# IuvenisSapiens/Qwen3-TTS-Rust

Hardware: AMD Instinct MI355X
Metric: audio-seconds generated per second (aggregate over GPUs) = concurrent real-time streams; RTF and first-chunk latency from the single-utterance leg (higher is better)
Workload: dtype i8

## Files before the change

### include/q3tts.h

```cpp
#ifndef Q3TTS_H
#define Q3TTS_H
#include <stdint.h>
#include <stddef.h>
#ifdef __cplusplus
extern "C" {
#endif

#define Q3TTS_OK 0
#define Q3TTS_ERR -1

const char* q3tts_last_error(void);
int q3tts_version(void);
int q3tts_device_count(void);

typedef struct q3tts_sampler_config {
    float temperature;
    int32_t top_k;
    float top_p;
    int32_t has_seed;
    uint64_t seed;
} q3tts_sampler_config;
void q3tts_sampler_config_default(q3tts_sampler_config* c);

typedef struct q3tts_gen_options {
// ... 112 lines not shown
int32_t q3tts_group_device_of(q3tts_group* g, int64_t req_id);
int q3tts_group_poll(q3tts_group* g, int64_t req_id, q3tts_req_status* out);
int q3tts_group_fetch(q3tts_group* g, int64_t req_id, int32_t* codes_out, int32_t frame_off, int32_t max_frames, float* pcm_out,
                      int64_t pcm_off, int64_t pcm_cap, int32_t* got_frames, int64_t* got_pcm);
int q3tts_group_wait(q3tts_group* g, int64_t req_id, double timeout_ms);
int q3tts_group_release(q3tts_group* g, int64_t req_id);
int q3tts_group_start(q3tts_group* g);
int q3tts_group_stop(q3tts_group* g);
typedef struct q3tts_comm q3tts_comm;
int q3tts_comm_available(void);
int q3tts_comm_unique_id(uint8_t out_id[128]);
int q3tts_comm_create(const uint8_t id[128], int32_t rank, int32_t world, int32_t device, q3tts_comm** out);
void q3tts_comm_destroy(q3tts_comm* c);
int q3tts_comm_voice_register(q3tts_comm* c, q3tts_engine* e, int32_t root, const float* spk_emb2048, const int32_t* ref_codes,
                              int32_t n_ref_codes, const int32_t* ref_text_ids, int32_t n_ref_text, int32_t* voice_id);
int32_t q3tts_engine_device(q3tts_engine* e);

typedef struct q3tts_assets q3tts_assets;
int q3tts_assets_open(const char* gguf_path, q3tts_assets** out);
void q3tts_assets_close(q3tts_assets* a);
const q3tts_assets* q3tts_engine_assets(q3tts_engine* e);
int q3tts_assets_codec_embedding(const q3tts_assets* a, int32_t q, int32_t code, float* out2048);
int q3tts_assets_text_embedding(const q3tts_assets* a, int64_t token, float* out2048);
int q3tts_assets_tts_pad(const q3tts_assets* a, float* out2048);
int q3tts_prompt_build_core(const q3tts_assets* a, const int32_t* text_ids, int32_t n_text, int32_t lang_id, int32_t spk_id,
                            const float* spk_emb2048, const int32_t* instr_ids, int32_t n_instr, const float* mid_rows,
                            int32_t n_mid, float* out, int32_t max_rows);
int q3tts_prompt_build_clone(const q3tts_assets* a, const int32_t* text_ids, int32_t n_text, const int32_t* ref_codes,
                             int32_t n_ref_codes, const int32_t* ref_text_ids, int32_t n_ref_text, const float* spk_emb2048,
                             int32_t lang_id, const int32_t* instr_ids, int32_t n_instr, float* out, int32_t max_rows);
int q3tts_prompt_build_streaming(const q3tts_assets* a, const int32_t* text_ids, int32_t n_text, int32_t lang_id, int32_t spk_id,
                                 const float* spk_emb2048, const int32_t* instr_ids, int32_t n_instr, const int32_t* ref_codes,
                                 int32_t n_ref_codes, const int32_t* ref_text_ids, int32_t n_ref_text, float* out, int32_t max_rows,
                                 int32_t* trail_ids, int32_t trail_cap, int32_t* n_trail);

typedef struct q3tts_sampler q3tts_sampler;
q3tts_sampler* q3tts_sampler_new(float temperature, int32_t top_k, float top_p, uint64_t seed);
void q3tts_sampler_free(q3tts_sampler* s);
int32_t q3tts_sampler_sample(q3tts_sampler* s, const float* logits, int32_t n_vocab, int32_t start, int32_t end);

typedef void (*q3tts_decode_cb)(void* user, const int64_t* codes, int32_t n_codes, int32_t is_final);
typedef struct q3tts_chunker q3tts_chunker;
q3tts_chunker* q3tts_chunker_new(q3tts_decode_cb cb, void* user);
void q3tts_chunker_free(q3tts_chunker* c);
int q3tts_chunker_push(q3tts_chunker* c, const int64_t* codes, int32_t n, int32_t is_final);

typedef struct q3tts_decoder q3tts_decoder;
int q3tts_decoder_create(const char* codec_gguf, int32_t n_streams, q3tts_decoder** out);
void q3tts_decoder_destroy(q3tts_decoder* d);
int q3tts_decoder_create_ex(const char* codec_gguf, int32_t n_streams, int32_t max_frames_per_call, int32_t max_group, q3tts_decoder** out);
int q3tts_decoder_decode_group(q3tts_decoder* d, int32_t G, const int32_t* streams, const int64_t* codes, int32_t n_frames, float* wav_out);
int q3tts_decoder_samples_per_frame(q3tts_decoder* d);
int q3tts_decoder_reset(q3tts_decoder* d, int32_t stream);
int q3tts_decoder_decode(q3tts_decoder* d, int32_t stream, const int64_t* codes, int32_t n_frames, int32_t is_last,
                         float* final_wav, int64_t* valid_samples);

int64_t q3tts_decoder_state_floats(q3tts_decoder* d);
int q3tts_decoder_state_export(q3tts_decoder* d, int32_t stream, float* out, int64_t n_floats);
int q3tts_decoder_state_import(q3tts_decoder* d, int32_t stream, const float* in, int64_t n_floats);
int32_t q3tts_decoder_state_entry(q3tts_decoder* d, int32_t i, const char** name, int64_t* offset, int32_t* rows, int32_t* cols);

int q3tts_mel_frames(int32_t n_samples);
int q3tts_mel(const float* audio, int32_t n_samples, float* mel_out );

typedef struct q3tts_tf q3tts_tf;
int q3tts_tf_open(const char* gguf_path, int32_t n_ctx, int32_t max_tok, q3tts_tf** out);
void q3tts_tf_close(q3tts_tf* t);
int q3tts_tf_dims(q3tts_tf* t, int32_t* n_embd, int32_t* n_layer, int32_t* n_head, int32_t* n_vocab);
void q3tts_tf_clear(q3tts_tf* t);
int q3tts_tf_eval(q3tts_tf* t, const float* x, const int32_t* pos4, int32_t ntok, float* hidden_out, float* logits_out,
                  int32_t row0, int32_t row1);

typedef struct q3tts_tokenizer q3tts_tokenizer;
int q3tts_tokenizer_open(const char* tokenizer_json, q3tts_tokenizer** out);
void q3tts_tokenizer_close(q3tts_tokenizer* t);
int32_t q3tts_tokenizer_encode(q3tts_tokenizer* t, const char* text_utf8, int32_t* ids, int32_t cap);
int64_t q3tts_tokenizer_decode(q3tts_tokenizer* t, const int32_t* ids, int32_t n, char* buf, int64_t cap);
int32_t q3tts_tokenizer_vocab_size(q3tts_tokenizer* t);
int64_t q3tts_text_nfc(const char* utf8, char* out, int64_t cap);

typedef struct q3tts_onnx q3tts_onnx;
int q3tts_onnx_open(const char* path, q3tts_onnx** out);
void q3tts_onnx_close(q3tts_onnx* m);
int q3tts_onnx_counts(q3tts_onnx* m, int32_t* n_nodes, int32_t* n_initializers, int32_t* n_inputs, int32_t* n_outputs);
int64_t q3tts_onnx_summary(q3tts_onnx* m, char* buf, int64_t cap);
int q3tts_onnx_node(q3tts_onnx* m, int32_t i, const char** op_type, const char** name, int32_t* n_in, int32_t* n_out, int32_t* n_attr);
const char* q3tts_onnx_node_input(q3tts_onnx* m, int32_t i, int32_t j);
const char* q3tts_onnx_node_output(q3tts_onnx* m, int32_t i, int32_t j);
int32_t q3tts_onnx_node_attr_ints(q3tts_onnx* m, int32_t i, const char* attr, int64_t* out, int32_t cap);
int32_t q3tts_onnx_node_attr_float(q3tts_onnx* m, int32_t i, const char* attr, float* out);
int q3tts_onnx_initializer(q3tts_onnx* m, int32_t i, const char** name, int32_t* dtype, int64_t* dims8, int32_t* ndims, const void** data,
                           int64_t* nbytes);
const char* q3tts_onnx_op_kernel(const char* op_type);
int q3tts_onnx_decoder_contract(q3tts_onnx* m, char* buf, int64_t cap);

typedef struct q3tts_onnx_session q3tts_onnx_session;
int q3tts_onnx_session_open(const char* path, int32_t device, q3tts_onnx_session** out);
void q3tts_onnx_session_close(q3tts_onnx_session* s);
int32_t q3tts_onnx_session_unsupported(q3tts_onnx_session* s, char* buf, int64_t cap);
int q3tts_onnx_session_set_input(q3tts_onnx_session* s, const char* name, int32_t dtype, const void* data, const int64_t* shape, int32_t rank);
int q3tts_onnx_session_run(q3tts_onnx_session* s);
int q3tts_onnx_session_output_info(q3tts_onnx_session* s, const char* name, int32_t* dtype, int32_t* rank, int64_t* shape8);
int q3tts_onnx_session_output(q3tts_onnx_session* s, const char* name, void* dst, int64_t cap_bytes);
int64_t q3tts_onnx_session_launches(q3tts_onnx_session* s);
int q3tts_onnx_op_executable(const char* op_type);
typedef struct q3tts_onnx_decoder q3tts_onnx_decoder;
int q3tts_onnx_decoder_open(const char* path, int32_t device, q3tts_onnx_decoder** out);
void q3tts_onnx_decoder_close(q3tts_onnx_decoder* d);
int q3tts_onnx_decoder_reset(q3tts_onnx_decoder* d);
int q3tts_onnx_decoder_decode(q3tts_onnx_decoder* d, const int64_t* codes, int32_t n_frames, int32_t is_final, float* pcm, int64_t cap, int64_t* n_out);
int q3tts_onnx_decoder_fetch(q3tts_onnx_decoder* d, float* pcm, int64_t cap, int64_t* n_out);

int q3tts_op_gemv_q8(const void* w_q8_0 , int32_t n, int32_t k, const int8_t* xq,
                     const uint16_t* xd, int32_t ntok, float* y , int32_t lpr);
int q3tts_op_gemv_kq(const void* const* raws, const int32_t* types, const int32_t* rows, int32_t nparts, int32_t k, const int8_t* xq, const uint16_t* xd,
                     int32_t ntok, float* y, int32_t lpr);
int q3tts_op_gateup_kq(const void* gate_raw, const void* up_raw, int32_t type, int32_t ff, int32_t k, const int8_t* xq, const uint16_t* xd, int32_t ntok,
                       int8_t* aq, uint16_t* ad);
int q3tts_op_gateup_q8(const void* w_q8_0, int32_t ff, int32_t k, const int8_t* xq, const uint16_t* xd, int32_t ntok, int8_t* aq,
                       uint16_t* ad);
int q3tts_op_matmul_float(const void* w , int32_t type, int32_t n, int32_t k, int32_t row0, int32_t nrows,
                          const float* x , int32_t ntok, float* y );
int q3tts_op_rmsnorm_quant(const float* x, const float* g, int32_t d, int32_t ntok, float eps, int8_t* xq, uint16_t* xd,
                           float* xn);
int q3tts_op_swiglu_quant(const float* gu, int32_t ff, int32_t ntok, int8_t* aq, uint16_t* ad);
int q3tts_op_argmax(const float* logits, int32_t n, int32_t start, int32_t end, int32_t mask_idx, int32_t* out);
int q3tts_op_sample(const float* logits, int32_t n, float temperature, int32_t top_k, float top_p, uint64_t seed, int32_t mask_idx,
                    int32_t n_draws, int32_t* out);
int q3tts_op_sample_rows(int32_t kernel, const float* logits, int32_t B, int32_t n, const float* temperature, const int32_t* top_k,
                         const float* top_p, const float* penalty, const uint64_t* seed, const int32_t* hist, const int32_t* hist_len,
                         int32_t hist_cap, int32_t n_draws, int32_t* out);
int q3tts_op_project(const float* x, const float* w , const float* b, int32_t n_in, int32_t n_out, float* y);
enum { Q3TTS_GEMM_AUTO = 0, Q3TTS_GEMM_SKINNY4 = 1, Q3TTS_GEMM_SKINNY8 = 2, Q3TTS_GEMM_SKINNY16 = 3,
       Q3TTS_GEMM_F32_1 = 4, Q3TTS_GEMM_F32_2 = 5,
       Q3TTS_GEMM_H1 = 6, Q3TTS_GEMM_H1_EPL = 7, Q3TTS_GEMM_H2 = 8, Q3TTS_GEMM_H2_EPL = 9,
       Q3TTS_GEMM_H3 = 10, Q3TTS_GEMM_H3_EPL = 11 };
enum { Q3TTS_EPI_NONE = 0, Q3TTS_EPI_GELU = 1, Q3TTS_EPI_RES_SCALE = 2 , Q3TTS_EPI_RES = 3 ,
       Q3TTS_EPI_SNAKE = 4  };
typedef struct q3tts_codec_gemm_desc {
    int32_t M, N, cin, taps, dil;
    const float* A; int64_t a_rows; int32_t lda, a_segT, a_skip;
    int32_t a_split, o_split;
    const float* W; const float* bias;
    int32_t epi; const float* res; int64_t res_floats; int32_t ldr, r_segT; int64_t r_skip;
    const float* scale; const float* snake_ea; const float* snake_ib;
    float* out; int64_t out_floats, out_off; int32_t ldo, o_segT; int64_t o_skip;
    int64_t ws_floats;
    int32_t form, ksplit, reducer;
    int32_t form_ran, ksplit_ran, reducer_ran;
} q3tts_codec_gemm_desc;
int q3tts_op_codec_gemm(q3tts_codec_gemm_desc* d);
int q3tts_codec_gemm_plan(q3tts_codec_gemm_desc* d);

#ifdef __cplusplus
}
#endif
#endif
```

### qwen3-tts-rust_amd/csrc/capi_ops.cpp

```cpp
#include "../../include/q3tts.h"
#include "transformer.h"
#include "host_logic.h"
#include "kdev.h"
#include "codec.h"

using namespace q3;
#define Q3_API_BEGIN try {
#define Q3_API_END(failval) } catch (const std::exception& ex) { set_last_error(ex.what()); return failval; } catch (...) { set_last_error("unknown error"); return failval; }
static void require_gpu() {
    int n = 0;
    if (hipGetDeviceCount(&n) != hipSuccess || n <= 0) throw Error("no HIP device available: the HIP path is the only compute path (no CPU fallback)");
}

extern "C" {

int q3tts_op_gemv_q8(const void* w, int32_t n, int32_t k, const int8_t* xq, const uint16_t* xd, int32_t ntok, float* y, int32_t lpr) {
    Q3_API_BEGIN
    require_gpu();
    DevBuf<uint8_t> storage;
    Q8Mat m = q8mat_from_host(w, n, k, storage);
    DevBuf<int8_t> dxq((size_t)ntok * k); dxq.upload(xq, dxq.n);
    DevBuf<uint16_t> dxd((size_t)ntok * (k / 32)); dxd.upload(xd, dxd.n);
    const int nsseg = ((k >> 8) + 7) / 8;
    DevBuf<float> parts((size_t)nsseg * ntok * n);
// ... 65 lines not shown
    DevBuf<uint8_t> storage;
    Q8Mat m = kqmat_from_host(parts, 2, k, storage);
    DevBuf<int8_t> dxq((size_t)ntok * k); dxq.upload(xq, dxq.n);
    DevBuf<uint16_t> dxd((size_t)ntok * (k / 32)); dxd.upload(xd, dxd.n);
    DevBuf<int8_t> daq((size_t)ntok * ff); DevBuf<uint16_t> dad((size_t)ntok * (ff / 32));
    if (!launch_gateup_mfma(0, m, ff, dxq.p, dxd.p, daq.p, dad.p, ntok)) throw Error("shape not served by the fused gate/up matrix-core kernel");
    Q3_LAUNCH_CHECK();
    Q3_HIP(hipDeviceSynchronize());
    daq.download(aq, daq.n); dad.download(ad, dad.n);
    return Q3TTS_OK;
    Q3_API_END(Q3TTS_ERR)
}

int q3tts_op_matmul_float(const void* w, int32_t type, int32_t n, int32_t k, int32_t row0, int32_t nrows, const float* x, int32_t ntok, float* y) {
    Q3_API_BEGIN
    require_gpu();
    Q3_CHECK(type == Q3_T_F32 || type == Q3_T_F16 || type == Q3_T_BF16, "float type expected");
    Q3_CHECK(n > 0 && k > 0 && k % 256 == 0 && ntok > 0 && row0 >= 0 && nrows > 0 && row0 + nrows <= n, "bad matmul shape");
    const size_t esz = type == Q3_T_F32 ? 4 : 2;
    DevBuf<uint8_t> dw((size_t)n * k * esz); dw.upload((const uint8_t*)w, dw.n);
    DevBuf<uint8_t> dwt((size_t)((n + 63) / 64) * 64 * k * esz);
    launch_tile_float(0, dw.p, dwt.p, type, n, k);
    FMat m; m.w = dw.p; m.wt = dwt.p; m.type = type; m.N = n; m.K = k;
    DevBuf<float> dx((size_t)ntok * k); dx.upload(x, dx.n);
    DevBuf<float> dy((size_t)ntok * nrows);
    launch_gemv_float(0, m, row0, nrows, dx.p, k, dy.p, nrows, ntok);
    Q3_HIP(hipDeviceSynchronize());
    dy.download(y, dy.n);
    return Q3TTS_OK;
    Q3_API_END(Q3TTS_ERR)
}

int q3tts_op_rmsnorm_quant(const float* x, const float* g, int32_t d, int32_t ntok, float eps, int8_t* xq, uint16_t* xd, float* xn) {
    Q3_API_BEGIN
    require_gpu();
    Q3_CHECK(d % 256 == 0 && d <= 2048, "d must be a multiple of 256 and <= 2048");
    DevBuf<float> dx((size_t)ntok * d), dg(d), dxn((size_t)ntok * d);
    dx.upload(x, dx.n); dg.upload(g, d);
    DevBuf<int8_t> dq((size_t)ntok * d); DevBuf<uint16_t> dd((size_t)ntok * d / 32);
    NormArgs a{};
    a.h_in = dx.p; a.h_stride = d; a.g = dg.p; a.eps = eps; a.d = d; a.xq = dq.p; a.xd = dd.p; a.xn_out = dxn.p;
    launch_rmsnorm_quant(0, a, ntok);
    Q3_HIP(hipDeviceSynchronize());
    if (xq) dq.download(xq, dq.n);
    if (xd) dd.download(xd, dd.n);
    if (xn) dxn.download(xn, dxn.n);
    return Q3TTS_OK;
    Q3_API_END(Q3TTS_ERR)
}

int q3tts_op_swiglu_quant(const float* gu, int32_t ff, int32_t ntok, int8_t* aq, uint16_t* ad) {
    Q3_API_BEGIN
    require_gpu();
    DevBuf<float> dgu((size_t)ntok * 2 * ff); dgu.upload(gu, dgu.n);
    DevBuf<int8_t> dq((size_t)ntok * ff); DevBuf<uint16_t> dd((size_t)ntok * ff / 32);
    launch_swiglu_quant(0, dgu.p, ff, dq.p, dd.p, ntok);
    Q3_HIP(hipDeviceSynchronize());
    dq.download(aq, dq.n); dd.download(ad, dd.n);
    return Q3TTS_OK;
    Q3_API_END(Q3TTS_ERR)
}

int q3tts_op_argmax(const float* logits, int32_t n, int32_t start, int32_t end, int32_t mask_idx, int32_t* out) {
    Q3_API_BEGIN
    require_gpu();
    DevBuf<float> dl(n); dl.upload(logits, n);
    DevBuf<int32_t> dm(1), dout(1);
    dm.upload(&mask_idx, 1);
    launch_argmax(0, dl.p, n, start, end, dm.p, dout.p, 1, 0, 1);
    Q3_HIP(hipDeviceSynchronize());
    dout.download(out, 1);
    return Q3TTS_OK;
    Q3_API_END(Q3TTS_ERR)
}

int q3tts_op_sample(const float* logits, int32_t n, float temperature, int32_t top_k, float top_p, uint64_t seed, int32_t mask_idx,
                    int32_t n_draws, int32_t* out) {
    Q3_API_BEGIN
    require_gpu();
    Q3_CHECK(logits && out && n >= 1 && n_draws >= 1, "bad arguments");
    StdRng rng(seed);
    DevBuf<float> dl(n), dt(1), dp(1); DevBuf<int32_t> dk(1), dm(1); DevBuf<uint32_t> dkey(8), ddraw(1); DevBuf<q3_u64> dout(n_draws);
    const uint32_t zero = 0;
    dl.upload(logits, n); dt.upload(&temperature, 1); dp.upload(&top_p, 1); dk.upload(&top_k, 1); dm.upload(&mask_idx, 1);
    dkey.upload(rng.key(), 8); ddraw.upload(&zero, 1);
    for (int i = 0; i < n_draws; i++) {
        SampleArgs a{dl.p, n, n, dt.p, dk.p, dp.p, dm.p, dkey.p, ddraw.p, dout.p + i, 1};
        launch_sample(0, a, 1);
    }
    Q3_HIP(hipDeviceSynchronize());
    std::vector<q3_u64> keys(n_draws);
    dout.download(keys.data(), n_draws);
    for (int i = 0; i < n_draws; i++) out[i] = (int32_t)(~(uint32_t)(keys[i] & 0xFFFFFFFFull));
    return Q3TTS_OK;
    Q3_API_END(Q3TTS_ERR)
}

int q3tts_op_sample_rows(int32_t kernel, const float* logits, int32_t B, int32_t n, const float* temperature, const int32_t* top_k,
                         const float* top_p, const float* penalty, const uint64_t* seed, const int32_t* hist, const int32_t* hist_len,
                         int32_t hist_cap, int32_t n_draws, int32_t* out) {
    Q3_API_BEGIN
    require_gpu();
    Q3_CHECK(logits && temperature && top_k && top_p && seed && out && B >= 1 && n >= 1 && n_draws >= 1, "bad arguments");
    Q3_CHECK(kernel == 0 || kernel == 1, "kernel must be 0 (k_sample) or 1 (k_sample_pred)");
    Q3_CHECK(kernel == 0 || !penalty, "the predictor sampler takes no penalty");
    Q3_CHECK(!penalty || (hist && hist_len && hist_cap >= 1), "a penalty needs a history");
    DevBuf<float> dl((size_t)B * n), dt(B), dp(B), dpen(B); DevBuf<int32_t> dk(B); DevBuf<uint32_t> dkey((size_t)8 * B), ddraw(B);
    DevBuf<q3_u64> dout((size_t)n_draws * B);
    dl.upload(logits, dl.n); dt.upload(temperature, B); dp.upload(top_p, B); dk.upload(top_k, B);
    std::vector<uint32_t> keys((size_t)8 * B), zero(B, 0u);
    for (int b = 0; b < B; b++) { StdRng rng(seed[b]); std::copy(rng.key(), rng.key() + 8, keys.begin() + (size_t)b * 8); }
    dkey.upload(keys.data(), keys.size()); ddraw.upload(zero.data(), B);
    DevBuf<int32_t> dh, dlen; DevBuf<q3_u64> dcur;
    if (penalty) {
        const int stride = hist_cap * 16;
        std::vector<int32_t> hh((size_t)B * stride, -1), len(B);
        std::vector<q3_u64> cur(B, 0ull);
        for (int b = 0; b < B; b++) {
            Q3_CHECK(hist_len[b] >= 0 && hist_len[b] <= hist_cap, "hist_len out of range");
            const int nh = hist_len[b];
            for (int f = 0; f + 1 < nh; f++) hh[(size_t)b * stride + (size_t)f * 16] = hist[(size_t)b * hist_cap + f];
            len[b] = nh > 0 ? nh - 1 : 0;
            if (nh > 0) cur[b] = pack_key(0.0f, hist[(size_t)b * hist_cap + nh - 1]);
        }
        dh.alloc(hh.size()); dh.upload(hh.data(), hh.size()); dlen.alloc(B); dlen.upload(len.data(), B); dcur.alloc((size_t)16 * B);
        std::vector<q3_u64> cur16((size_t)16 * B, 0ull);
        for (int b = 0; b < B; b++) cur16[(size_t)b * 16] = cur[b];
        dcur.upload(cur16.data(), cur16.size());
        dpen.upload(penalty, B);
    }
    for (int i = 0; i < n_draws; i++) {
        SampleArgs a{dl.p, n, n, dt.p, dk.p, dp.p, nullptr, dkey.p, ddraw.p, dout.p + (size_t)i * B, 1};
        if (penalty) { a.penalty = dpen.p; a.hist = dh.p; a.hist_stride = hist_cap * 16; a.hist_len = dlen.p; a.cur_key = dcur.p; a.cur_stride = 16; }
        if (kernel == 0) launch_sample(0, a, B);
        else launch_sample_pred(0, a, B);
        Q3_LAUNCH_CHECK();
    }
    Q3_HIP(hipDeviceSynchronize());
    std::vector<q3_u64> res(dout.n);
    dout.download(res.data(), res.size());
    for (size_t i = 0; i < res.size(); i++) out[i] = key_code(res[i]);
    return Q3TTS_OK;
    Q3_API_END(Q3TTS_ERR)
}

int q3tts_op_codec_gemm(q3tts_codec_gemm_desc* d) {
    Q3_API_BEGIN
    require_gpu();
    codec_gemm_run(d);
    return Q3TTS_OK;
    Q3_API_END(Q3TTS_ERR)
}

int q3tts_codec_gemm_plan(q3tts_codec_gemm_desc* d) {
    Q3_API_BEGIN
    codec_gemm_plan_only(d);
    return Q3TTS_OK;
    Q3_API_END(Q3TTS_ERR)
}

int q3tts_op_project(const float* x, const float* w, const float* b, int32_t n_in, int32_t n_out, float* y) {
    Q3_API_BEGIN
    require_gpu();
    std::vector<float> wt((size_t)n_in * n_out);
    for (int o = 0; o < n_out; o++) for (int i = 0; i < n_in; i++) wt[(size_t)i * n_out + o] = w[(size_t)o * n_in + i];
    DevBuf<float> dx(n_in), dw(wt.size()), db(n_out), dy(n_out);
    dx.upload(x, n_in); dw.upload(wt.data(), wt.size()); db.upload(b, n_out);
    launch_project(0, dx.p, n_in, dw.p, db.p, n_in, n_out, dy.p, n_out, 1);
    Q3_HIP(hipDeviceSynchronize());
    dy.download(y, n_out);
    return Q3TTS_OK;
    Q3_API_END(Q3TTS_ERR)
}

int q3tts_mel_frames(int32_t n) { const int plen = n + 768; return (plen > 1024 ? plen - 1024 : 0) / 256 + 1; }

}

#include "onnx_reader.h"
#include "onnx_exec.h"
struct q3tts_onnx { std::unique_ptr<OnnxModel> m; std::string text; };
extern "C" {
int q3tts_onnx_open(const char* path, q3tts_onnx** out) {
    Q3_API_BEGIN
    Q3_CHECK(path && out, "null argument");
    auto* h = new q3tts_onnx();
    try { h->m.reset(new OnnxModel(path)); } catch (...) { delete h; throw; }
    *out = h;
    return Q3TTS_OK;
    Q3_API_END(Q3TTS_ERR)
}
void q3tts_onnx_close(q3tts_onnx* m) { delete m; }
int q3tts_onnx_counts(q3tts_onnx* m, int32_t* n_nodes, int32_t* n_init, int32_t* n_in, int32_t* n_out) {
    if (!m) return Q3TTS_ERR;
    if (n_nodes) *n_nodes = (int32_t)m->m->nodes.size();
    if (n_init) *n_init = (int32_t)m->m->initializers.size();
    if (n_in) *n_in = (int32_t)m->m->inputs.size();
    if (n_out) *n_out = (int32_t)m->m->outputs.size();
    return Q3TTS_OK;
}
int64_t q3tts_onnx_summary(q3tts_onnx* m, char* buf, int64_t cap) {
    if (!m) return -1;
    m->text = m->m->summary();
    if (buf && cap > 0) { const size_t n = std::min((size_t)cap - 1, m->text.size()); std::memcpy(buf, m->text.data(), n); buf[n] = 0; }
    return (int64_t)m->text.size() + 1;
}
int q3tts_onnx_node(q3tts_onnx* m, int32_t i, const char** op_type, const char** name, int32_t* n_in, int32_t* n_out, int32_t* n_attr) {
    Q3_API_BEGIN
    Q3_CHECK(m && i >= 0 && i < (int)m->m->nodes.size(), "node index out of range");
    const OnnxNode& n = m->m->nodes[i];
    if (op_type) *op_type = n.op_type.c_str();
    if (name) *name = n.name.c_str();
    if (n_in) *n_in = (int32_t)n.inputs.size();
    if (n_out) *n_out = (int32_t)n.outputs.size();
    if (n_attr) *n_attr = (int32_t)n.attrs.size();
    return Q3TTS_OK;
    Q3_API_END(Q3TTS_ERR)
}
const char* q3tts_onnx_node_input(q3tts_onnx* m, int32_t i, int32_t j) {
    return (m && i >= 0 && i < (int)m->m->nodes.size() && j >= 0 && j < (int)m->m->nodes[i].inputs.size()) ? m->m->nodes[i].inputs[j].c_str() : nullptr;
}
const char* q3tts_onnx_node_output(q3tts_onnx* m, int32_t i, int32_t j) {
    return (m && i >= 0 && i < (int)m->m->nodes.size() && j >= 0 && j < (int)m->m->nodes[i].outputs.size()) ? m->m->nodes[i].outputs[j].c_str() : nullptr;
}
int32_t q3tts_onnx_node_attr_ints(q3tts_onnx* m, int32_t i, const char* attr, int64_t* out, int32_t cap) {
    if (!m || i < 0 || i >= (int)m->m->nodes.size() || !attr) return -1;
    const OnnxAttr* a = m->m->nodes[i].attr(attr);
    if (!a) return -1;
    if (a->type == 2 || (a->ints.empty() && a->type == 0)) { if (out && cap > 0) out[0] = a->i; return 1; }
    for (int k = 0; k < (int)a->ints.size() && k < cap; k++) out[k] = a->ints[k];
    return (int32_t)a->ints.size();
}
int32_t q3tts_onnx_node_attr_float(q3tts_onnx* m, int32_t i, const char* attr, float* out) {
    if (!m || i < 0 || i >= (int)m->m->nodes.size() || !attr || !out) return -1;
    const OnnxAttr* a = m->m->nodes[i].attr(attr);
    if (!a) return -1;
    *out = a->f;
    return 1;
}
int q3tts_onnx_initializer(q3tts_onnx* m, int32_t i, const char** name, int32_t* dtype, int64_t* dims8, int32_t* ndims, const void** data, int64_t* nbytes) {
    Q3_API_BEGIN
    Q3_CHECK(m && i >= 0 && i < (int)m->m->initializers.size(), "initializer index out of range");
    const OnnxTensor& t = m->m->initializers[i];
    Q3_CHECK(t.dims.size() <= 8, "more than 8 dimensions");
    if (name) *name = t.name.c_str();
    if (dtype) *dtype = t.data_type;
    if (ndims) *ndims = (int32_t)t.dims.size();
    if (dims8) for (size_t d = 0; d < t.dims.size(); d++) dims8[d] = t.dims[d];
    const void* p = t.raw; int64_t nb = (int64_t)t.raw_bytes;
    if (!p && !t.float_data.empty()) { p = t.float_data.data(); nb = (int64_t)t.float_data.size() * 4; }
    else if (!p && !t.int64_data.empty()) { p = t.int64_data.data(); nb = (int64_t)t.int64_data.size() * 8; }
    else if (!p && !t.int32_data.empty()) { p = t.int32_data.data(); nb = (int64_t)t.int32_data.size() * 4; }
    if (data) *data = p;
    if (nbytes) *nbytes = nb;
    return Q3TTS_OK;
    Q3_API_END(Q3TTS_ERR)
}
const char* q3tts_onnx_op_kernel(const char* op_type) { return op_type ? onnx_op_kernel(op_type) : nullptr; }
int q3tts_onnx_decoder_contract(q3tts_onnx* m, char* buf, int64_t cap) {
    if (!m) return Q3TTS_ERR;
    const std::string miss = m->m->check_decoder_contract();
    if (buf && cap > 0) { const size_t n = std::min((size_t)cap - 1, miss.size()); std::memcpy(buf, miss.data(), n); buf[n] = 0; }
    return miss.empty() ? 0 : 1;
}
}

#include "tokenizer.h"
struct q3tts_tokenizer { std::unique_ptr<Tokenizer> t; std::string text; };
extern "C" {
int q3tts_tokenizer_open(const char* tokenizer_json, q3tts_tokenizer** out) {
    Q3_API_BEGIN
    Q3_CHECK(tokenizer_json && out, "null argument");
    auto* h = new q3tts_tokenizer();
    try { h->t.reset(new Tokenizer(tokenizer_json)); } catch (...) { delete h; throw; }
    *out = h;
    return Q3TTS_OK;
    Q3_API_END(Q3TTS_ERR)
}
void q3tts_tokenizer_close(q3tts_tokenizer* t) { delete t; }
int32_t q3tts_tokenizer_encode(q3tts_tokenizer* t, const char* text_utf8, int32_t* ids, int32_t cap) {
    Q3_API_BEGIN
    Q3_CHECK(t && text_utf8, "null argument");
    const std::vector<int32_t> v = t->t->encode(text_utf8);
    for (size_t i = 0; i < v.size() && (int32_t)i < cap; i++) ids[i] = v[i];
    return (int32_t)v.size();
    Q3_API_END(-1)
}
int64_t q3tts_tokenizer_decode(q3tts_tokenizer* t, const int32_t* ids, int32_t n, char* buf, int64_t cap) {
    Q3_API_BEGIN
    Q3_CHECK(t && (ids || n == 0) && n >= 0, "bad arguments");
    t->text = t->t->decode(std::vector<int32_t>(ids, ids + n));
    if (buf && cap > 0) { const size_t k = std::min((size_t)cap - 1, t->text.size()); std::memcpy(buf, t->text.data(), k); buf[k] = 0; }
    return (int64_t)t->text.size();
    Q3_API_END(-1)
}
int64_t q3tts_text_nfc(const char* utf8, char* out, int64_t cap) {
    try {
        if (!utf8) return 0;
        const std::string r = q3::nfc_utf8(utf8);
        if (out && cap > 0) { const size_t n = std::min<size_t>((size_t)cap - 1, r.size()); memcpy(out, r.data(), n); out[n] = 0; }
        return (int64_t)r.size() + 1;
    } catch (const std::exception& e) { q3::set_last_error(e.what()); return -1; }
}
int32_t q3tts_tokenizer_vocab_size(q3tts_tokenizer* t) { return t ? t->t->vocab_size() : 0; }
}

// ... 93 lines not shown
```

### qwen3-tts-rust_amd/csrc/kernels.h

```cpp
#pragma once
#include <hip/hip_runtime.h>
#include <cstdint>

namespace q3 {

struct Q8Mat {
    const uint8_t* qs = nullptr;
    const uint16_t* sc = nullptr;
    int N = 0;
    int Npad = 0;
    int K = 0;
    const uint8_t* rg_type = nullptr;
    const uint32_t* rg_off = nullptr;
    const uint8_t* meta = nullptr;
    size_t qbytes = 0;
    int nparts = 0; int p1_rg0 = 0x7fffffff, p2_rg0 = 0x7fffffff; int p0_type = 0, p1_type = 0, p2_type = 0; uint32_t p0_off = 0, p1_off = 0, p2_off = 0;
    size_t bytes() const { return (qbytes ? qbytes : (size_t)Npad * K) + (size_t)Npad * (K / 32) * 2 + (meta ? (size_t)Npad * (K / 256) * 16 : 0); }
};
inline size_t q3_rowgroup_bytes(int type, int K) { return type == 13 ? (size_t)(K / 256) * 5120 : type == 14 ? (size_t)(K / 256) * 6144 : (size_t)(K / 32) * 1024; }

struct TokMeta {
    const int32_t* seq;
    const int32_t* slot;
    const int32_t* pos;
    int uniform_pos = -1;
    __device__ __forceinline__ int seq_of(int tok) const { return uniform_pos >= 0 ? tok : seq[tok]; }
    __device__ __forceinline__ int slot_of(int tok) const { return uniform_pos >= 0 ? uniform_pos : slot[tok]; }
    __device__ __forceinline__ int pos_of(int tok, int stream) const { return uniform_pos >= 0 ? uniform_pos : pos[(size_t)tok * 4 + stream]; }
};

struct KvCache {
    uint16_t* k;
    uint16_t* v;
    const int32_t* page_table;
    int max_pages;
    int n_layer, n_kv;
    __host__ __device__ size_t page_stride() const { return (size_t)n_layer * n_kv * 8192; }
    __host__ __device__ size_t layer_stride() const { return (size_t)n_kv * 8192; }
    __device__ __forceinline__ int page_of(int seq, int logical) const { return page_table ? page_table[(size_t)seq * max_pages + logical] : seq; }
};

bool launch_gateup_mfma(hipStream_t st, const Q8Mat& wgu, int ff, const int8_t* xq, const uint16_t* xd, int8_t* aq, uint16_t* ad, int ntok);
void launch_gemv_q8(hipStream_t st, const Q8Mat& w, int row0, int nrows, const int8_t* xq, const uint16_t* xd,
                    float* out, int out_stride, int ntok, int lpr_hint = 0);

struct NormArgs {
    const float* h_in; int h_stride;
    const int32_t* idx; int idx_stride;
    const unsigned long long* idx_keys;
    const float* parts; int nparts; int parts_stride;
    float* h_out;
    const float* g; float eps; int d;
    int8_t* xq; uint16_t* xd;
    float* xn_out;
};
void launch_rmsnorm_quant(hipStream_t st, const NormArgs& a, int ntok);

void launch_qk_rope_append(hipStream_t st, const float* qkv, int qkv_stride, const float* parts_unused, int n_head, int n_kv,
                           const float* q_norm_w, const float* k_norm_w, float eps, const float* rope_cos,
                           const float* rope_sin, int n_ctx, const int32_t* mrope_sec , const TokMeta& tm,
                           const KvCache& kv, int layer, float* qrot, int ntok);

void launch_attention(hipStream_t st, const float* qrot, int n_head, int n_kv, const TokMeta& tm, const KvCache& kv,
                      int layer, float* att , int8_t* aq, uint16_t* ad, int ntok);

void launch_swiglu_quant(hipStream_t st, const float* gu, int ff, int8_t* aq, uint16_t* ad, int ntok);

void launch_argmax(hipStream_t st, const float* logits, int stride, int start, int end, const int32_t* mask_per_tok,
                   int32_t* out, int out_stride, int add, int ntok);

void launch_project(hipStream_t st, const float* x, int x_stride, const float* Wt, const float* b, int n_in, int n_out,
                    float* out, int out_stride, int ntok);
void launch_project_table(hipStream_t st, const float* table, int64_t rows, const float* Wt, const float* b, int n_in,
                          int n_out, float* out);

void launch_argmax_keys(hipStream_t st, const float* logits, int stride, int n, const int32_t* mask_per_tok, unsigned long long* keys,
                        int key_stride, int ntok);


void launch_copy_f32(hipStream_t st, const float* src, float* dst, size_t n);
void init_kernel_attributes();

struct FMat { const void* w = nullptr; const void* wt = nullptr; int type = 0; int N = 0, K = 0; size_t bytes() const { return (size_t)N * K * (type == 0 ? 4 : 2); } };
void launch_gemv_float(hipStream_t st, const FMat& w, int row0, int nrows, const float* x, int x_stride, float* out, int out_stride, int ntok);
bool launch_gateup_float(hipStream_t st, const FMat& wgu, int ff, const float* x, int x_stride, float* act, int ntok);
void launch_tile_float(hipStream_t st, const void* w, void* wt, int type, int N, int K);
void launch_swiglu_f32(hipStream_t st, const float* gu, int ff, float* out, int ntok);

typedef unsigned long long q3_u64;
struct NormPro {
    const float* h_in; int h_stride;
    const q3_u64* idx_keys; int idx_stride;
    const float* parts; int nparts; int parts_stride; size_t parts_slab;
    float* h_out;
    const float* g; float eps;
    float* xn_out;
};
struct ArgmaxEpi {
    q3_u64* keys; int key_stride;
    const int32_t* mask_per_tok;
    int idx_add;
};
void launch_gemv_q8_norm(hipStream_t st, const Q8Mat& w, int row0, int nrows, const NormPro& a, float* out, int out_stride,
                         int ntok, const ArgmaxEpi* am);
void launch_rmsnorm_quant_wg(hipStream_t st, const NormPro& a, int d, int8_t* xq, uint16_t* xd, int ntok);
void launch_gateup_swiglu(hipStream_t st, const Q8Mat& wgu, int ff, const NormPro& a, int8_t* aq, uint16_t* ad, int ntok);
void launch_attention_fused(hipStream_t st, const float* qkv, int qkv_stride, int n_head, int n_kv, const float* q_norm_w,
                            const float* k_norm_w, float eps, const float* rope_cos, const float* rope_sin, int n_ctx,
                            const int32_t* mrope_sec, const TokMeta& tm, const KvCache& kv, int layer, int8_t* aq, uint16_t* ad,
                            int ntok);
void launch_attention_short(hipStream_t st, const float* qkv, int qkv_stride, int n_head, int n_kv, const float* q_norm_w,
                            const float* k_norm_w, float eps, const float* rope_cos, const float* rope_sin, int n_ctx,
                            const int32_t* mrope_sec, const TokMeta& tm, const KvCache& kv, int layer, int8_t* aq, uint16_t* ad, int ntok,
                            float* att = nullptr );
void launch_project_blk(hipStream_t st, const float* x, int x_stride, const float* Wblk , const float* b,
                        int n_in, int n_out, float* out, int out_stride, int ntok);
struct TextTrail {
    const int32_t* n_frames = nullptr; const int32_t* n_trail = nullptr; const int32_t* ids = nullptr; int ids_stride = 0;
    const float* table = nullptr; int64_t rows = 0;
};
void launch_feedback_keys(hipStream_t st, const float* const* tables, const int64_t* table_rows, const q3_u64* keys, int key_stride,
                          const float* tts_pad, float* out, int ntok, const TextTrail* trail = nullptr);
void launch_gather_rows_keys(hipStream_t st, const float* table, int64_t rows, const q3_u64* keys, int key_stride, int row_len,
                             float* dst, int ntok);
struct AdvanceKeysArgs {
    int B; int32_t *finished, *n_frames; const int32_t* max_frames; q3_u64* keys; q3_u64* next_key0; int32_t* hist; int hist_stride;
    int32_t *t_slot, *t_pos;
};
void launch_advance_keys(hipStream_t st, const AdvanceKeysArgs& a);

struct SampleArgs {
    const float* logits; int stride; int n;
    const float* temperature; const int32_t* top_k; const float* top_p;
    const int32_t* mask_idx;
    const uint32_t* rng_key; uint32_t* draws;
    q3_u64* out_key; int out_stride;
    const float* penalty = nullptr;
    const int32_t* hist = nullptr; int hist_stride = 0; const int32_t* hist_len = nullptr;
    const q3_u64* cur_key = nullptr; int cur_stride = 0;
};
void launch_sample(hipStream_t st, const SampleArgs& a, int B);
void launch_sample_pred(hipStream_t st, const SampleArgs& a, int B);

}
```

### qwen3-tts-rust_amd/csrc/kernels_fused.hip

```cpp
#include "kernels.h"
#include "kdev.h"
#include "wslice.h"
#include <cstdlib>
#include "q3_common.h"

namespace q3 {
Q3_STAMP_SETTER(set_stamp_buffer_fused)

__device__ __forceinline__ void norm_quant_token(const NormPro& a, int d, int tok, int ntok, int lane, int8_t* xq_dst,
                                                 uint16_t* xd_dst, bool write_global) {
    const int nch = d >> 8;
    const float* hin = a.h_in;
    if (a.idx_keys) hin += (size_t)key_code(a.idx_keys[(size_t)tok * a.idx_stride]) * a.h_stride;
    else hin += (size_t)tok * a.h_stride;
    float4 x[8];
    float p = 0.0f;
#pragma unroll
    for (int c = 0; c < 8; c++) {
        if (c < nch) {
            float4 v = *reinterpret_cast<const float4*>(hin + 256 * c + 4 * lane);
            if (a.nparts > 0) {
                const float* pp = a.parts + (size_t)tok * a.parts_stride + 256 * c + 4 * lane;
                float4 y = *reinterpret_cast<const float4*>(pp);
                for (int s = 1; s < a.nparts; s++) {
// ... 136 lines not shown
            acc[m] = ws.chain(0.0f, &xq_s[mm][seg * 256], dxv, r, half, bil);
        }
        if (q == 0) {
#pragma unroll
            for (int m = 0; m < MT; m++) red[wave][m * R + r] = acc[m];
        }
    });
    wg_barrier_lds();
    for (int t = threadIdx.x; t < R * MT; t += blockDim.x) {
        const int m = t / R, rr = t % R;
        float v[8];
#pragma unroll
        for (int s = 0; s < 8; s++) v[s] = red[s][t];
        float S = v[0];
#pragma unroll
        for (int s = 1; s < 8; s++) S = (s < nseg) ? S + v[s] : S;
        const int orow = blockIdx.x * R + rr, tok = tok0 + m;
        const bool ok = orow < nrows && tok < ntok;
        if (EPI == 0) {
            if (ok) out[(size_t)tok * out_stride + orow] = S;
        } else {
            const int gi = orow + am.idx_add;
            const int mk = (ok && am.mask_per_tok) ? am.mask_per_tok[tok] : -1;
            u64 key = (ok && gi != mk && S > -INFINITY) ? pack_key(S, gi) : 0ull;
#pragma unroll
            for (int sft = R / 2; sft >= 1; sft >>= 1) {
                const u64 o = __shfl_xor(key, sft);
                key = o > key ? o : key;
            }
            if (rr == 0 && key != 0ull && tok < ntok) atomicMax(am.keys + (size_t)tok * am.key_stride, key);
        }
    }
}

template <int LPR, int MT, int EPI>
static void gemv_norm_launch(hipStream_t st, const Q8Mat& w, int row0, int nrows, const NormPro& a, float* out, int out_stride,
                             int ntok, const ArgmaxEpi& am) {
    constexpr int R = 64 / LPR;
    const int nseg = w.K >> 8;
    dim3 grid((nrows + R - 1) / R, 1, (ntok + MT - 1) / MT);
    Q3_TS_SWITCH(w, hipLaunchKernelGGL((k_gemv_q8_norm<LPR, MT, EPI, TS>), grid, dim3(64 * nseg), 0, st, w, row0, nrows, a, out, out_stride, ntok, am));
}
template <int LPR, int EPI>
static void gemv_norm_mt(hipStream_t st, const Q8Mat& w, int row0, int nrows, const NormPro& a, float* out, int out_stride, int ntok,
                         const ArgmaxEpi& am) {
    if (ntok == 1) gemv_norm_launch<LPR, 1, EPI>(st, w, row0, nrows, a, out, out_stride, ntok, am);
    else if (ntok == 2) gemv_norm_launch<LPR, 2, EPI>(st, w, row0, nrows, a, out, out_stride, ntok, am);
    else if (ntok <= 4) gemv_norm_launch<LPR, 4, EPI>(st, w, row0, nrows, a, out, out_stride, ntok, am);
    else gemv_norm_launch<LPR, 8, EPI>(st, w, row0, nrows, a, out, out_stride, ntok, am);
}
void launch_gemv_q8_norm(hipStream_t st, const Q8Mat& w, int row0, int nrows, const NormPro& a, float* out, int out_stride, int ntok,
                         const ArgmaxEpi* am) {
    ArgmaxEpi none{};
    if (am) { gemv_norm_mt<2, 1>(st, w, row0, nrows, a, out, out_stride, ntok, *am); return; }
    if (nrows / 32 >= 512) gemv_norm_mt<2, 0>(st, w, row0, nrows, a, out, out_stride, ntok, none);
    else if (nrows / 16 >= 256) gemv_norm_mt<4, 0>(st, w, row0, nrows, a, out, out_stride, ntok, none);
    else gemv_norm_mt<8, 0>(st, w, row0, nrows, a, out, out_stride, ntok, none);
}

template <int MT, int NSEG, int TS>
__global__ void __launch_bounds__(64 * NSEG) k_gateup_swiglu(Q8Mat w, int ff, NormPro a, int8_t* __restrict__ aq,
                                                             uint16_t* __restrict__ ad, int ntok) {
    __shared__ float red[8][2][32 * MT];
    __shared__ __attribute__((aligned(16))) int8_t xq_s[MT][2048];
    __shared__ __attribute__((aligned(16))) uint16_t xd_s[MT][64];
    __shared__ __attribute__((aligned(16))) float vbuf_s[2048];
    __shared__ float scal_s[1];
    const int lane = threadIdx.x & 63, wave = threadIdx.x >> 6;
    const int r = lane & 31, half = lane >> 5;
    const int nseg = w.K >> 8;
    const int seg = wave;
    const int tok0 = blockIdx.z * MT;
    const int rgG = blockIdx.x, rgU = (ff >> 5) + blockIdx.x;
    wslice_dispatch<TS>(w, rgG, [&](auto tag) {
        constexpr int WT = decltype(tag)::value;
        WSlice<2, WT> wsg, wsu;
        if (WT == 0) {
            const int nb = w.K >> 5;
            const uint8_t* baseG = w.qs + ((size_t)rgG * nb + (size_t)seg * 8) * 1024 + half * 512 + r * 16;
            const uint8_t* baseU = w.qs + ((size_t)rgU * nb + (size_t)seg * 8) * 1024 + half * 512 + r * 16;
#pragma unroll
            for (int i = 0; i < 8; i++) { wsg.wv[i] = *reinterpret_cast<const uint4*>(baseG + (size_t)i * 1024); wsu.wv[i] = *reinterpret_cast<const uint4*>(baseU + (size_t)i * 1024); }
            wsg.dwv = *reinterpret_cast<const uint4*>(w.sc + (((size_t)rgG * nseg + seg) * 32 + r) * 8);
            wsu.dwv = *reinterpret_cast<const uint4*>(w.sc + (((size_t)rgU * nseg + seg) * 32 + r) * 8);
        } else {
            wsg.load(w, rgG, r, seg, half, 0);
            wsu.load(w, rgU, r, seg, half, 0);
        }
        for (int m = 0; m < MT; m++) {
            const int tok = tok0 + m;
            norm_quant_wg(a, w.K, tok, tok < ntok, lane, wave, xq_s[m], xd_s[m], vbuf_s, scal_s, blockIdx.x == 0);
            if (m + 1 < MT) wg_barrier_lds();
        }
        wg_barrier_lds();
        wsg.finish(half); wsu.finish(half);
#pragma unroll
        for (int m = 0; m < MT; m++) {
            const int mm = (tok0 + m < ntok) ? m : 0;
            const uint4 dxv = *reinterpret_cast<const uint4*>(&xd_s[mm][seg * 8]);
            float ag = 0.0f, au = 0.0f;
            if (WT == 0) {
#pragma unroll
                for (int i = 0; i < 8; i++) {
                    const uint4 xv = *reinterpret_cast<const uint4*>(&xq_s[mm][seg * 256 + i * 32 + half * 16]);
                    int ig = dot16(wsg.wv[i], xv), iu = dot16(wsu.wv[i], xv);
                    ig += xor_lane<32>(ig); iu += xor_lane<32>(iu);
                    const float dx = h2f(half_of(dxv, i));
                    ag = q3_fmaf((float)ig, h2f(half_of(wsg.dwv, i)) * dx, ag);
                    au = q3_fmaf((float)iu, h2f(half_of(wsu.dwv, i)) * dx, au);
                }
            } else {
                ag = wsg.chain(0.0f, &xq_s[mm][seg * 256], dxv, r, half, 0);
                au = wsu.chain(0.0f, &xq_s[mm][seg * 256], dxv, r, half, 0);
            }
            if (half == 0) { red[wave][0][m * 32 + r] = ag; red[wave][1][m * 32 + r] = au; }
        }
    });
    wg_barrier_lds();
    for (int t = threadIdx.x; t < 32 * MT; t += blockDim.x) {
        const int m = t >> 5, rr = t & 31, tok = tok0 + m;
        float vg[8], vu[8];
#pragma unroll
        for (int s = 0; s < 8; s++) { vg[s] = red[s][0][t]; vu[s] = red[s][1][t]; }
        float G = vg[0], U = vu[0];
#pragma unroll
        for (int s = 1; s < 8; s++) { G = (s < nseg) ? G + vg[s] : G; U = (s < nseg) ? U + vu[s] : U; }
        const float y = q3_swiglu(G, U);
        float amax = q3_fabsf(y);
        amax = fmaxf(amax, xor_lane<16>(amax)); amax = fmaxf(amax, xor_lane<8>(amax)); amax = fmaxf(amax, xor_lane<4>(amax));
        amax = fmaxf(amax, xor_lane<2>(amax)); amax = fmaxf(amax, xor_lane<1>(amax));
        const float dd = amax / 127.0f;
        const float id = (dd != 0.0f) ? (1.0f / dd) : 0.0f;
        if (tok < ntok) {
            aq[(size_t)tok * ff + blockIdx.x * 32 + rr] = (int8_t)(int)q3_rintf(y * id);
            if (rr == 0) ad[(size_t)tok * (ff >> 5) + blockIdx.x] = f2h(dd);
        }
    }
}
void launch_gateup_swiglu(hipStream_t st, const Q8Mat& w, int ff, const NormPro& a, int8_t* aq, uint16_t* ad, int ntok) {
    const int nseg = w.K >> 8;
    const int mt = ntok == 1 ? 1 : ntok == 2 ? 2 : 4;
    dim3 grid(ff / 32, 1, (ntok + mt - 1) / mt);
#define Q3_GU(MTV, NS) Q3_TS_SWITCH(w, hipLaunchKernelGGL((k_gateup_swiglu<MTV, NS, TS>), grid, dim3(64 * NS), 0, st, w, ff, a, aq, ad, ntok))
#define Q3_GU_NS(NS) do { if (mt == 1) Q3_GU(1, NS); else if (mt == 2) Q3_GU(2, NS); else Q3_GU(4, NS); } while (0)
    switch (nseg) {
        case 1: Q3_GU_NS(1); break; case 2: Q3_GU_NS(2); break; case 3: Q3_GU_NS(3); break; case 4: Q3_GU_NS(4); break;
        case 5: Q3_GU_NS(5); break; case 6: Q3_GU_NS(6); break; case 7: Q3_GU_NS(7); break; case 8: Q3_GU_NS(8); break;
        default: throw Error("k_gateup_swiglu: K must be at most 2048");
    }
#undef Q3_GU_NS
#undef Q3_GU
}

__global__ void __launch_bounds__(256) k_attention_fused(const float* __restrict__ qkv, int qkv_stride, int n_head, int n_kv,
                                                         const float* __restrict__ q_norm_w, const float* __restrict__ k_norm_w,
                                                         float eps, const float* __restrict__ rope_cos,
                                                         const float* __restrict__ rope_sin, int n_ctx,
                                                         const int32_t* __restrict__ mrope_sec, TokMeta tm, KvCache kv, int layer,
                                                         int8_t* __restrict__ aq, uint16_t* __restrict__ ad) {
    __shared__ __attribute__((aligned(16))) float q_s[128];
    __shared__ __attribute__((aligned(16))) uint16_t kcur_s[128];
    __shared__ __attribute__((aligned(16))) uint16_t vcur_s[128];
    __shared__ float p_s[256];
    __shared__ float red_s[4][128];
    __shared__ float wmax_s[4];
    const int h = blockIdx.x, tok = blockIdx.y, tid = threadIdx.x, lane = tid & 63, wave = tid >> 6;
    const int seq = tm.seq_of(tok), slot = tm.slot_of(tok), n = slot + 1;
    const int grp = n_head / n_kv, kvh = h / grp;
    const size_t head_off = (size_t)layer * kv.layer_stride() + (size_t)kvh * 8192;
    const int jj = lane >> 4, dc = lane & 15;
    uint4 kreg[16], vreg[16];
    {
        const int jbase = wave * 64;
        if (jbase < n) {
            const int page = kv.page_of(seq, jbase >> 6);
            const uint16_t* Kb = kv.k + (size_t)page * kv.page_stride() + head_off;
#pragma unroll
            for (int d8 = 0; d8 < 16; d8++) kreg[d8] = *reinterpret_cast<const uint4*>(Kb + (d8 * 64 + lane) * 8);
        }
#pragma unroll
        for (int u = 0; u < 16; u++) {
            const int jg = 16 * u + 4 * wave + jj;
            vreg[u] = make_uint4(0, 0, 0, 0);
            if (jg < n && jg != slot) {
                const int page = kv.page_of(seq, jg >> 6);
                vreg[u] = *reinterpret_cast<const uint4*>(kv.v + (size_t)page * kv.page_stride() + head_off + (jg & 63) * 128 + dc * 8);
            }
        }
    }
    if (wave < 3) {
        const float* vec = qkv + (size_t)tok * qkv_stride + (wave == 0 ? (size_t)h * 128 : wave == 1 ? (size_t)(n_head + kvh) * 128 : (size_t)(n_head + n_kv + kvh) * 128);
        const float x1 = vec[lane], x2 = vec[lane + 64];
        const int page = kv.page_of(seq, slot >> 6), ps = slot & 63;
        if (wave < 2) {
            const float* wn = wave == 0 ? q_norm_w : k_norm_w;
            const float w1 = wn[lane], w2 = wn[lane + 64];
            int32_t sec[4] = { mrope_sec[0], mrope_sec[1], mrope_sec[2], mrope_sec[3] };
            int pp = tm.pos_of(tok, q3_mrope_stream(lane, sec));
            if (pp < 0) pp = 0;
            if (pp > n_ctx - 1) pp = n_ctx - 1;
            const float cs = rope_cos[(size_t)pp * 64 + lane], sn = rope_sin[(size_t)pp * 64 + lane];
            float p = x1 * x1;
            p = q3_fmaf(x2, x2, p);
            const float ss = wave_sum_bfly(p);
            const float mean = ss / 128.0f;
            const float scale = 1.0f / q3_sqrtf(mean + eps);
            const float y1 = (x1 * scale) * w1, y2 = (x2 * scale) * w2;
            float o1, o2;
            q3_rope_pair(y1, y2, cs, sn, &o1, &o2);
            if (wave == 0) { q_s[lane] = o1; q_s[lane + 64] = o2; }
            else {
                const uint16_t k1 = f2h(o1), k2 = f2h(o2);
                kcur_s[lane] = k1; kcur_s[lane + 64] = k2;
                if (h % grp == 0) {
                    uint16_t* Kb = kv.k + (size_t)page * kv.page_stride() + head_off;
                    Kb[((lane >> 3) * 64 + ps) * 8 + (lane & 7)] = k1;
                    Kb[(((lane + 64) >> 3) * 64 + ps) * 8 + (lane & 7)] = k2;
                }
            }
        } else {
            const uint16_t v1 = f2h(x1), v2 = f2h(x2);
            vcur_s[lane] = v1; vcur_s[lane + 64] = v2;
            if (h % grp == 0) {
                uint16_t* Vb = kv.v + (size_t)page * kv.page_stride() + head_off;
                Vb[ps * 128 + lane] = v1; Vb[ps * 128 + lane + 64] = v2;
            }
        }
    }
    wg_barrier_lds();
    const float scale = 0.08838834764831845f;
    float M = 0.0f, L = 0.0f, O[8];
#pragma unroll
    for (int i = 0; i < 8; i++) O[i] = 0.0f;
    for (int c0 = 0; c0 < n; c0 += 256) {
        const int jbase = c0 + wave * 64;
        const int jme = jbase + lane;
        const bool valid = jme < n;
        if (c0 > 0) {
            if (jbase < n) {
                const int page = kv.page_of(seq, jbase >> 6);
                const uint16_t* Kb = kv.k + (size_t)page * kv.page_stride() + head_off;
#pragma unroll
                for (int d8 = 0; d8 < 16; d8++) kreg[d8] = *reinterpret_cast<const uint4*>(Kb + (d8 * 64 + lane) * 8);
            }
#pragma unroll
            for (int u = 0; u < 16; u++) {
                const int jg = c0 + 16 * u + 4 * wave + jj;
                vreg[u] = make_uint4(0, 0, 0, 0);
                if (jg < n && jg != slot) {
                    const int page = kv.page_of(seq, jg >> 6);
                    vreg[u] = *reinterpret_cast<const uint4*>(kv.v + (size_t)page * kv.page_stride() + head_off + (jg & 63) * 128 + dc * 8);
                }
            }
        }
        float s = -INFINITY;
        if (jbase < n) {
            const bool cur = (jme == slot);
            float acc = 0.0f;
#pragma unroll
            for (int d8 = 0; d8 < 16; d8++) {
                uint4 kk = kreg[d8];
                if (cur) kk = *reinterpret_cast<const uint4*>(&kcur_s[8 * d8]);
                const float4 qa = *reinterpret_cast<const float4*>(&q_s[8 * d8]);
                const float4 qb = *reinterpret_cast<const float4*>(&q_s[8 * d8 + 4]);
                acc = q3_fmaf(qa.x, h2f(kk.x & 0xFFFFu), acc); acc = q3_fmaf(qa.y, h2f(kk.x >> 16), acc);
                acc = q3_fmaf(qa.z, h2f(kk.y & 0xFFFFu), acc); acc = q3_fmaf(qa.w, h2f(kk.y >> 16), acc);
                acc = q3_fmaf(qb.x, h2f(kk.z & 0xFFFFu), acc); acc = q3_fmaf(qb.y, h2f(kk.z >> 16), acc);
                acc = q3_fmaf(qb.z, h2f(kk.w & 0xFFFFu), acc); acc = q3_fmaf(qb.w, h2f(kk.w >> 16), acc);
            }
            if (valid) s = acc * scale;
        }
        const float wm = wave_max_bfly(s);
        if (lane == 0) wmax_s[wave] = wm;
        wg_barrier_lds();
        const float mc = fmaxf(fmaxf(wmax_s[0], wmax_s[1]), fmaxf(wmax_s[2], wmax_s[3]));
        const float p = valid ? q3_expf(s - mc) : 0.0f;
        p_s[wave * 64 + lane] = p;
        wg_barrier_lds();
        float S[8];
#pragma unroll
        for (int i = 0; i < 8; i++) S[i] = 0.0f;
        const int cn = (n - c0) < 256 ? (n - c0) : 256;
#pragma unroll
        for (int u = 0; u < 16; u++) {
            if (16 * u < cn) {
                const int jl = 16 * u + 4 * wave + jj;
                const int jg = c0 + jl;
                const float pj = p_s[jl];
                uint4 vv = vreg[u];
                if (jg == slot) vv = *reinterpret_cast<const uint4*>(&vcur_s[dc * 8]);
                S[0] = q3_fmaf(pj, h2f(vv.x & 0xFFFFu), S[0]); S[1] = q3_fmaf(pj, h2f(vv.x >> 16), S[1]);
                S[2] = q3_fmaf(pj, h2f(vv.y & 0xFFFFu), S[2]); S[3] = q3_fmaf(pj, h2f(vv.y >> 16), S[3]);
                S[4] = q3_fmaf(pj, h2f(vv.z & 0xFFFFu), S[4]); S[5] = q3_fmaf(pj, h2f(vv.z >> 16), S[5]);
                S[6] = q3_fmaf(pj, h2f(vv.w & 0xFFFFu), S[6]); S[7] = q3_fmaf(pj, h2f(vv.w >> 16), S[7]);
            }
        }
#pragma unroll
        for (int i = 0; i < 8; i++) {
            const float a2 = S[i] + xor_lane<16>(S[i]);
            const float T = a2 + xor_lane<32>(a2);
            if (jj == 0) red_s[wave][dc * 8 + i] = T;
        }
        wg_barrier_lds();
        if (wave == 0) {
            float a2 = p_s[lane];
            a2 = a2 + p_s[lane + 64]; a2 = a2 + p_s[lane + 128]; a2 = a2 + p_s[lane + 192];
            const float lc = wave_sum_bfly(a2);
            float oc[8];
#pragma unroll
            for (int i = 0; i < 8; i++) oc[i] = (red_s[0][dc * 8 + i] + red_s[1][dc * 8 + i]) + (red_s[2][dc * 8 + i] + red_s[3][dc * 8 + i]);
            if (c0 == 0) {
                M = mc; L = lc;
#pragma unroll
                for (int i = 0; i < 8; i++) O[i] = oc[i];
            } else {
                const float mn = fmaxf(M, mc);
                const float ea = q3_expf(M - mn), eb = q3_expf(mc - mn);
                const float t2 = lc * eb;
                L = q3_fmaf(L, ea, t2);
#pragma unroll
                for (int i = 0; i < 8; i++) { const float u2 = oc[i] * eb; O[i] = q3_fmaf(O[i], ea, u2); }
                M = mn;
            }
        }
        wg_barrier_lds();
    }
    if (wave == 0) {
        float y[8];
        float amax = 0.0f;
#pragma unroll
        for (int i = 0; i < 8; i++) { y[i] = O[i] / L; amax = fmaxf(amax, q3_fabsf(y[i])); }
        amax = fmaxf(amax, xor_lane<1>(amax));
        amax = fmaxf(amax, xor_lane<2>(amax));
        const float dd = amax / 127.0f;
        const float id = (dd != 0.0f) ? (1.0f / dd) : 0.0f;
        if (jj == 0) {
            const size_t o = ((size_t)tok * n_head + h) * 128 + dc * 8;
            uint32_t lo = 0, hi = 0;
#pragma unroll
            for (int i = 0; i < 4; i++) {
                lo |= (uint32_t)((int)q3_rintf(y[i] * id) & 0xFF) << (8 * i);
                hi |= (uint32_t)((int)q3_rintf(y[i + 4] * id) & 0xFF) << (8 * i);
            }
            *reinterpret_cast<uint2*>(aq + o) = make_uint2(lo, hi);
            if ((dc & 3) == 0) ad[o >> 5] = f2h(dd);
        }
    }
}
void launch_attention_fused(hipStream_t st, const float* qkv, int qkv_stride, int n_head, int n_kv, const float* q_norm_w,
                            const float* k_norm_w, float eps, const float* rope_cos, const float* rope_sin, int n_ctx,
                            const int32_t* mrope_sec, const TokMeta& tm, const KvCache& kv, int layer, int8_t* aq, uint16_t* ad,
                            int ntok) {
    hipLaunchKernelGGL(k_attention_fused, dim3(n_head, ntok), dim3(256), 0, st, qkv, qkv_stride, n_head, n_kv, q_norm_w, k_norm_w,
                       eps, rope_cos, rope_sin, n_ctx, mrope_sec, tm, kv, layer, aq, ad);
}

template <int HPW>
__global__ void __launch_bounds__(64) k_attention_short(const float* __restrict__ qkv, int qkv_stride, int n_head, int n_kv,
                                                        const float* __restrict__ q_norm_w, const float* __restrict__ k_norm_w, float eps,
                                                        const float* __restrict__ rope_cos, const float* __restrict__ rope_sin, int n_ctx,
                                                        const int32_t* __restrict__ mrope_sec, TokMeta tm, KvCache kv, int layer,
                                                        int8_t* __restrict__ aq, uint16_t* __restrict__ ad, float* __restrict__ att) {
    __shared__ __attribute__((aligned(16))) float q_s[HPW][128];
    __shared__ __attribute__((aligned(16))) uint16_t kcur_s[128];
    __shared__ __attribute__((aligned(16))) uint16_t vcur_s[128];
    __shared__ float p_s[HPW][64];
    const int kvh = HPW == 2 ? blockIdx.x : blockIdx.x >> 1, h0 = HPW == 2 ? 2 * blockIdx.x : blockIdx.x;
    Q3_STAMP_DECL;
    Q3_STAMP(0);
    const bool writer = HPW == 2 || (blockIdx.x & 1) == 0;
    const int tok = blockIdx.y, lane = threadIdx.x;
    const float scale = 0.08838834764831845f;
    const int jj = lane >> 4, dc = lane & 15;
    const int seq = tm.seq_of(tok), slot = tm.slot_of(tok), n = slot + 1;
    const size_t head_off = (size_t)layer * kv.layer_stride() + (size_t)kvh * 8192;
    const int page = kv.page_of(seq, 0);
    const uint16_t* Kb = kv.k + (size_t)page * kv.page_stride() + head_off;
    const uint16_t* Vb = kv.v + (size_t)page * kv.page_stride() + head_off;
    uint4 kreg[16], vreg[4][4];
#pragma unroll
    for (int d8 = 0; d8 < 16; d8++) kreg[d8] = (lane < slot) ? *reinterpret_cast<const uint4*>(Kb + (d8 * 64 + lane) * 8) : make_uint4(0, 0, 0, 0);
#pragma unroll
    for (int ww = 0; ww < 4; ww++)
#pragma unroll
        for (int u = 0; u < 4; u++) {
            const int jl = 16 * u + 4 * ww + jj;
            vreg[ww][u] = (jl < slot) ? *reinterpret_cast<const uint4*>(Vb + jl * 128 + dc * 8) : make_uint4(0, 0, 0, 0);
        }
    int32_t sec[4] = { mrope_sec[0], mrope_sec[1], mrope_sec[2], mrope_sec[3] };
    int pp = tm.pos_of(tok, q3_mrope_stream(lane, sec));
    if (pp < 0) pp = 0;
    if (pp > n_ctx - 1) pp = n_ctx - 1;
    const float cs = rope_cos[(size_t)pp * 64 + lane], sn = rope_sin[(size_t)pp * 64 + lane];
    const float* tv = qkv + (size_t)tok * qkv_stride;
#pragma unroll
    for (int which = 0; which < HPW + 1; which++) {
        const float* vec = tv + (which < HPW ? (size_t)(h0 + which) * 128 : (size_t)(n_head + kvh) * 128);
        const float* wn = which < HPW ? q_norm_w : k_norm_w;
        const float x1 = vec[lane], x2 = vec[lane + 64];
        float p = x1 * x1;
        p = q3_fmaf(x2, x2, p);
        const float ss = wave_sum_bfly(p);
        const float mean = ss / 128.0f;
        const float sc2 = 1.0f / q3_sqrtf(mean + eps);
        const float y1 = (x1 * sc2) * wn[lane], y2 = (x2 * sc2) * wn[lane + 64];
        float o1, o2;
        q3_rope_pair(y1, y2, cs, sn, &o1, &o2);
        if (which < HPW) { q_s[which][lane] = o1; q_s[which][lane + 64] = o2; }
        else {
            const uint16_t k1 = f2h(o1), k2 = f2h(o2);
            kcur_s[lane] = k1; kcur_s[lane + 64] = k2;
            if (writer) {
                uint16_t* Kw = kv.k + (size_t)page * kv.page_stride() + head_off;
                Kw[((lane >> 3) * 64 + slot) * 8 + (lane & 7)] = k1;
                Kw[(((lane + 64) >> 3) * 64 + slot) * 8 + (lane & 7)] = k2;
            }
        }
    }
    {
        const float* vec = tv + (size_t)(n_head + n_kv + kvh) * 128;
        const uint16_t v1 = f2h(vec[lane]), v2 = f2h(vec[lane + 64]);
        vcur_s[lane] = v1; vcur_s[lane + 64] = v2;
        if (writer) {
            uint16_t* Vw = kv.v + (size_t)page * kv.page_stride() + head_off;
            Vw[slot * 128 + lane] = v1; Vw[slot * 128 + lane + 64] = v2;
        }
    }
    wg_barrier_lds();
    Q3_STAMP(1);
    const bool valid = lane < n, cur = lane == slot;
    float a[HPW];
#pragma unroll
    for (int hh = 0; hh < HPW; hh++) a[hh] = 0.0f;
#pragma unroll
    for (int d8 = 0; d8 < 16; d8++) {
        uint4 kk = kreg[d8];
        if (cur) kk = *reinterpret_cast<const uint4*>(&kcur_s[8 * d8]);
        const float kf[8] = { h2f(kk.x & 0xFFFFu), h2f(kk.x >> 16), h2f(kk.y & 0xFFFFu), h2f(kk.y >> 16),
                              h2f(kk.z & 0xFFFFu), h2f(kk.z >> 16), h2f(kk.w & 0xFFFFu), h2f(kk.w >> 16) };
#pragma unroll
        for (int e = 0; e < 8; e++)
#pragma unroll
            for (int hh = 0; hh < HPW; hh++) a[hh] = q3_fmaf(q_s[hh][8 * d8 + e], kf[e], a[hh]);
    }
    Q3_STAMP_AFTER(2, a[0]);
    float L[HPW];
#pragma unroll
    for (int hh = 0; hh < HPW; hh++) {
        const float sc = valid ? a[hh] * scale : -INFINITY;
        const float m = wave_max_bfly(sc);
        const float pv = valid ? q3_expf(sc - m) : 0.0f;
        p_s[hh][lane] = pv;
        L[hh] = wave_sum_bfly(pv);
    }
    wg_barrier_lds();
    Q3_STAMP(3);
    const int dq = n_head * 128;
#pragma unroll
    for (int hh = 0; hh < HPW; hh++) {
        float s01[8], s23[8], y[8];
#pragma unroll
        for (int ww = 0; ww < 4; ww++) {
            float S[8];
#pragma unroll
            for (int i = 0; i < 8; i++) S[i] = 0.0f;
#pragma unroll
            for (int u = 0; u < 4; u++) {
                if (16 * u < n) {
                    const int jl = 16 * u + 4 * ww + jj;
                    const float pj = p_s[hh][jl];
                    uint4 vv = vreg[ww][u];
                    if (jl == slot) vv = *reinterpret_cast<const uint4*>(&vcur_s[dc * 8]);
                    S[0] = q3_fmaf(pj, h2f(vv.x & 0xFFFFu), S[0]); S[1] = q3_fmaf(pj, h2f(vv.x >> 16), S[1]);
                    S[2] = q3_fmaf(pj, h2f(vv.y & 0xFFFFu), S[2]); S[3] = q3_fmaf(pj, h2f(vv.y >> 16), S[3]);
                    S[4] = q3_fmaf(pj, h2f(vv.z & 0xFFFFu), S[4]); S[5] = q3_fmaf(pj, h2f(vv.z >> 16), S[5]);
                    S[6] = q3_fmaf(pj, h2f(vv.w & 0xFFFFu), S[6]); S[7] = q3_fmaf(pj, h2f(vv.w >> 16), S[7]);
                }
            }
#pragma unroll
            for (int i = 0; i < 8; i++) {
                const float a2 = S[i] + xor_lane<16>(S[i]);
                const float T = a2 + xor_lane<32>(a2);
                if (ww == 0) s01[i] = T; else if (ww == 1) s01[i] = s01[i] + T; else if (ww == 2) s23[i] = T; else s23[i] = s23[i] + T;
            }
        }
#pragma unroll
        for (int i = 0; i < 8; i++) y[i] = (s01[i] + s23[i]) / L[hh];
        const int hq = h0 + hh;
        if (att && jj == 0) {
            float* o = att + (size_t)tok * dq + (size_t)hq * 128 + dc * 8;
            *reinterpret_cast<float4*>(o) = make_float4(y[0], y[1], y[2], y[3]);
            *reinterpret_cast<float4*>(o + 4) = make_float4(y[4], y[5], y[6], y[7]);
        }
        float amax = 0.0f;
#pragma unroll
        for (int i = 0; i < 8; i++) amax = fmaxf(amax, q3_fabsf(y[i]));
        amax = fmaxf(amax, xor_lane<1>(amax));
        amax = fmaxf(amax, xor_lane<2>(amax));
        const float dd = amax / 127.0f;
        const float id = (dd != 0.0f) ? (1.0f / dd) : 0.0f;
        if (jj == 0) {
            uint32_t lo = 0, hi = 0;
#pragma unroll
            for (int i = 0; i < 4; i++) {
                lo |= (uint32_t)((int)q3_rintf(y[i] * id) & 0xFF) << (8 * i);
                hi |= (uint32_t)((int)q3_rintf(y[i + 4] * id) & 0xFF) << (8 * i);
            }
            *reinterpret_cast<uint2*>(aq + (size_t)tok * dq + (size_t)hq * 128 + dc * 8) = make_uint2(lo, hi);
            if ((dc & 3) == 0) ad[(size_t)tok * (dq >> 5) + hq * 4 + (dc >> 2)] = f2h(dd);
        }
    }
    Q3_STAMP(6);
    Q3_STAMP_FLUSH();
}
void launch_attention_short(hipStream_t st, const float* qkv, int qkv_stride, int n_head, int n_kv, const float* q_norm_w,
                            const float* k_norm_w, float eps, const float* rope_cos, const float* rope_sin, int n_ctx,
                            const int32_t* mrope_sec, const TokMeta& tm, const KvCache& kv, int layer, int8_t* aq, uint16_t* ad, int ntok, float* att) {
    static const int hpw1_max = [] { const char* e = std::getenv("Q3_SHORT_ATTN_HPW1_MAX"); return e ? atoi(e) : 128; }();
    if (ntok <= hpw1_max)
        hipLaunchKernelGGL(k_attention_short<1>, dim3(n_head, ntok), dim3(64), 0, st, qkv, qkv_stride, n_head, n_kv, q_norm_w, k_norm_w, eps, rope_cos,
                           rope_sin, n_ctx, mrope_sec, tm, kv, layer, aq, ad, att);
    else
        hipLaunchKernelGGL(k_attention_short<2>, dim3(n_kv, ntok), dim3(64), 0, st, qkv, qkv_stride, n_head, n_kv, q_norm_w, k_norm_w, eps, rope_cos,
                           rope_sin, n_ctx, mrope_sec, tm, kv, layer, aq, ad, att);
}

__global__ void __launch_bounds__(256) k_project_mt(const float* __restrict__ x, int x_stride, const float* __restrict__ Wblk,
                                                    const float* __restrict__ b, int n_in, int n_out, float* __restrict__ out,
                                                    int out_stride, int ntok) {
    constexpr int KC = 512, LDP = KC + 4;
    __shared__ __attribute__((aligned(16))) float xs[16][LDP];
    __shared__ __attribute__((aligned(16))) float ws[16][LDP];
    const int ob = blockIdx.x, t0 = blockIdx.y * 16, tid = threadIdx.x;
    const int o16 = tid & 15, tl = tid >> 4;
    const float* wslab = Wblk + (size_t)ob * n_in * 16;
    float4 rx[8], rw[8];
    auto fetch = [&](int k0) {
#pragma unroll
        for (int j = 0; j < 8; j++) {
            const int e = tid + 256 * j;
            const int t = e >> 7, i4 = e & 127;
            rx[j] = (t0 + t < ntok) ? *reinterpret_cast<const float4*>(x + (size_t)(t0 + t) * x_stride + k0 + 4 * i4) : make_float4(0.f, 0.f, 0.f, 0.f);
            rw[j] = *reinterpret_cast<const float4*>(wslab + (size_t)k0 * 16 + 4 * (size_t)e);
        }
    };
    auto stash = [&]() {
#pragma unroll
        for (int j = 0; j < 8; j++) {
            const int e = tid + 256 * j;
            *reinterpret_cast<float4*>(&xs[e >> 7][4 * (e & 127)]) = rx[j];
            const int i = e >> 2, q = (e & 3) * 4;
            ws[q + 0][i] = rw[j].x; ws[q + 1][i] = rw[j].y; ws[q + 2][i] = rw[j].z; ws[q + 3][i] = rw[j].w;
        }
    };
    const int o = ob * 16 + o16;
    float sum = b[o];
    fetch(0);
    for (int k0 = 0; k0 < n_in; k0 += KC) {
        stash();
        __syncthreads();
        if (k0 + KC < n_in) fetch(k0 + KC);
#pragma unroll 8
        for (int i = 0; i < KC; i += 4) {
            const float4 xv = *reinterpret_cast<const float4*>(&xs[tl][i]), wv = *reinterpret_cast<const float4*>(&ws[o16][i]);
            float t = xv.x * wv.x; sum = sum + t;
            t = xv.y * wv.y; sum = sum + t;
            t = xv.z * wv.z; sum = sum + t;
            t = xv.w * wv.w; sum = sum + t;
        }
        __syncthreads();
    }
    if (t0 + tl < ntok) out[(size_t)(t0 + tl) * out_stride + o] = sum;
}
void init_fused_kernel_attributes() {}
void launch_project_blk(hipStream_t st, const float* x, int x_stride, const float* Wblk, const float* b, int n_in, int n_out,
                        float* out, int out_stride, int ntok) {
    if (n_in % 512 != 0 || x_stride % 4 != 0 || (reinterpret_cast<uintptr_t>(x) & 15) != 0) throw Error("k_project_mt: n_in must be a multiple of 512 and the rows 16-byte aligned");
    hipLaunchKernelGGL(k_project_mt, dim3(n_out / 16, (ntok + 15) / 16), dim3(256), 0, st, x, x_stride, Wblk, b, n_in, n_out, out, out_stride, ntok);
}

template <bool TRAIL>
__global__ void __launch_bounds__(256) k_feedback_keys(const float* const* __restrict__ tables, const int64_t* __restrict__ table_rows,
                                                       const u64* __restrict__ keys, int key_stride,
                                                       const float* __restrict__ tts_pad, float* __restrict__ out, TextTrail tt) {
    const int tok = blockIdx.y, i = blockIdx.x * 256 + threadIdx.x;
    float acc = 0.0f;
#pragma unroll
    for (int q = 0; q < 16; q++) {
        int c = key_code(keys[(size_t)tok * key_stride + q]);
        if (c < 0) c = 0;
        const float v = ((int64_t)c < table_rows[q]) ? tables[q][(size_t)c * 2048 + i] : 0.0f;
        acc = acc + v;
    }
    float last;
    if constexpr (TRAIL) {
        const int f = tt.n_frames[tok];
        if (f < tt.n_trail[tok]) {
            const int32_t id = tt.ids[(size_t)tok * tt.ids_stride + f];
            if (id >= 0 && (int64_t)id < tt.rows) last = tt.table[(size_t)id * 2048 + i];
            else {
                const float x = (float)((unsigned long long)(long long)id * 17ull + (unsigned long long)i);
                last = (x < 16777216.0f ? (float)((uint32_t)x & 1u) : 0.0f) - 1.0f;
            }
        } else {
            last = tts_pad[i];
        }
    } else {
        last = tts_pad[i];
    }
    acc = acc + last;
    out[(size_t)tok * 2048 + i] = acc;
}
void launch_feedback_keys(hipStream_t st, const float* const* tables, const int64_t* table_rows, const u64* keys, int key_stride,
                          const float* tts_pad, float* out, int ntok, const TextTrail* trail) {
    if (trail) hipLaunchKernelGGL(k_feedback_keys<true>, dim3(8, ntok), dim3(256), 0, st, tables, table_rows, keys, key_stride, tts_pad, out, *trail);
    else hipLaunchKernelGGL(k_feedback_keys<false>, dim3(8, ntok), dim3(256), 0, st, tables, table_rows, keys, key_stride, tts_pad, out, TextTrail());
}

__global__ void __launch_bounds__(256) k_gather_rows_keys(const float* __restrict__ table, int64_t rows, const u64* __restrict__ keys,
                                                          int key_stride, int row_len, float* __restrict__ dst) {
    const int tok = blockIdx.y, i = blockIdx.x * 256 + threadIdx.x;
    if (i >= row_len) return;
    int c = key_code(keys[(size_t)tok * key_stride]);
    if (c < 0) c = 0;
    dst[(size_t)tok * row_len + i] = ((int64_t)c < rows) ? table[(size_t)c * row_len + i] : 0.0f;
}
void launch_gather_rows_keys(hipStream_t st, const float* table, int64_t rows, const u64* keys, int key_stride, int row_len,
                             float* dst, int ntok) {
    hipLaunchKernelGGL(k_gather_rows_keys, dim3((row_len + 255) / 256, ntok), dim3(256), 0, st, table, rows, keys, key_stride, row_len, dst);
}

__global__ void k_advance_keys(AdvanceKeysArgs a) {
    const int b = blockIdx.x * 64 + threadIdx.x;
    if (b >= a.B) return;
    u64* k = a.keys + (size_t)b * 16;
    const bool live = !a.finished[b] && a.n_frames[b] < a.max_frames[b];
    if (live) {
        const int c0 = key_code(k[0]);
        if (c0 == Q3_CODEC_EOS || c0 == Q3_TEXT_EOS) a.finished[b] = 1;
        else {
            int32_t* dst = a.hist + (size_t)b * a.hist_stride + (size_t)a.n_frames[b] * 16;
            for (int q = 0; q < 16; q++) dst[q] = key_code(k[q]);
            a.n_frames[b] = a.n_frames[b] + 1;
            a.t_slot[b] = a.t_slot[b] + 1;
            a.t_pos[b * 4 + 0] += 1; a.t_pos[b * 4 + 1] += 1; a.t_pos[b * 4 + 2] += 1;
        }
    }
    k[0] = a.next_key0[b];
    a.next_key0[b] = pack_key(-INFINITY, 0);
    for (int q = 1; q < 16; q++) k[q] = pack_key(-INFINITY, 0);
}
void launch_advance_keys(hipStream_t st, const AdvanceKeysArgs& a) {
    hipLaunchKernelGGL(k_advance_keys, dim3((a.B + 63) / 64), dim3(64), 0, st, a);
}

}
```

### qwen3-tts-rust_amd/csrc/transformer.cpp

```cpp
#include "transformer.h"
#include <cstdlib>
#include <cmath>

namespace q3 {

__global__ void k_repack_q8(const uint8_t* __restrict__ raw, int n, int K, int row_off, uint8_t* __restrict__ qs,
                            uint16_t* __restrict__ sc, int sc_row_extra) {
    const int nb = K >> 5, nseg = K >> 8;
    const size_t id = (size_t)blockIdx.x * 256 + threadIdx.x;
    if (id >= (size_t)n * nb) return;
    const int r = (int)(id / nb), b = (int)(id % nb);
    const uint8_t* src = raw + id * 34;
    const int row = row_off + r, rg = row >> 5, r32 = row & 31;
    uint16_t d;
    memcpy(&d, src, 2);
    const int srow = row + sc_row_extra;
    sc[(((size_t)(srow >> 5) * nseg + (b >> 3)) * 32 + (srow & 31)) * 8 + (b & 7)] = d;
    uint8_t* dst = qs + ((size_t)rg * nb + b) * 1024 + r32 * 16;
    for (int i = 0; i < 16; i++) { dst[i] = src[2 + i]; dst[512 + i] = src[18 + i]; }
}

__global__ void k_repack_q5k(const uint8_t* __restrict__ raw, int n, int K, int row_off, uint8_t* __restrict__ qs, const uint32_t* __restrict__ rg_off,
                             uint16_t* __restrict__ sc, uint8_t* __restrict__ meta) {
    const int nseg = K >> 8;
// ... 95 lines not shown
    std::vector<uint8_t> types((size_t)nrg);
    std::vector<uint32_t> off((size_t)nrg);
    size_t qs_bytes = 0;
    { int rg = 0; for (int i = 0; i < nparts; i++) for (int j = 0; j < parts[i].rows / 32; j++, rg++) { types[(size_t)rg] = (uint8_t)parts[i].type; off[(size_t)rg] = (uint32_t)(qs_bytes / 16); qs_bytes += q3_rowgroup_bytes(parts[i].type, k); } }
    const size_t sc_bytes = (size_t)n * (k / 32) * 2, meta_bytes = (size_t)n * (k / 256) * 16, ty_bytes = (size_t)((nrg + 15) & ~15), off_bytes = (size_t)((nrg * 4 + 15) & ~15);
    storage.alloc(qs_bytes + sc_bytes + meta_bytes + ty_bytes + off_bytes);
    storage.zero();
    uint8_t* base = storage.p;
    uint16_t* sc = reinterpret_cast<uint16_t*>(base + qs_bytes);
    uint8_t* meta = base + qs_bytes + sc_bytes;
    uint8_t* ty = meta + meta_bytes;
    uint32_t* offd = reinterpret_cast<uint32_t*>(ty + ty_bytes);
    Q3_HIP(hipMemcpy(ty, types.data(), types.size(), hipMemcpyHostToDevice));
    Q3_HIP(hipMemcpy(offd, off.data(), off.size() * 4, hipMemcpyHostToDevice));
    m.qs = base; m.sc = sc; m.meta = meta; m.rg_type = ty; m.rg_off = offd; m.qbytes = qs_bytes;
    int last = -1, row_off = 0;
    for (int i = 0; i < nparts; i++) {
        const int t = parts[i].type, rows = parts[i].rows;
        Q3_CHECK(t == Q3_T_Q8_0 || t == Q3_T_Q5_K || t == Q3_T_Q6_K, "unsupported weight type");
        if (t != last) {
            const int rg0 = row_off / 32;
            if (m.nparts == 0) { m.p0_type = t; m.p0_off = off[(size_t)rg0]; }
            else if (m.nparts == 1) { m.p1_rg0 = rg0; m.p1_type = t; m.p1_off = off[(size_t)rg0]; }
            else { m.p2_rg0 = rg0; m.p2_type = t; m.p2_off = off[(size_t)rg0]; }
            m.nparts++; last = t;
        }
        const size_t raw_bytes = t == Q3_T_Q8_0 ? (size_t)rows * (k / 32) * 34 : (size_t)rows * (k / 256) * (t == Q3_T_Q5_K ? 176 : 210);
        DevBuf<uint8_t> raw(raw_bytes);
        raw.upload((const uint8_t*)parts[i].raw, raw_bytes);
        if (t == Q3_T_Q8_0) {
            const size_t nblk = (size_t)rows * (k / 32);
            hipLaunchKernelGGL(k_repack_q8, dim3((unsigned)((nblk + 255) / 256)), dim3(256), 0, 0, raw.p, rows, k, 0, base + (size_t)off[(size_t)(row_off / 32)] * 16, sc, row_off);
        } else {
            const size_t nsb = (size_t)rows * (k / 256);
            if (t == Q3_T_Q5_K) hipLaunchKernelGGL(k_repack_q5k, dim3((unsigned)((nsb + 255) / 256)), dim3(256), 0, 0, raw.p, rows, k, row_off, base, offd, sc, meta);
            else hipLaunchKernelGGL(k_repack_q6k, dim3((unsigned)((nsb + 255) / 256)), dim3(256), 0, 0, raw.p, rows, k, row_off, base, offd, sc, meta);
        }
        Q3_HIP(hipDeviceSynchronize());
        row_off += rows;
    }
    return m;
}

Q8Mat Transformer::make_mat(const Gguf& g, const std::vector<std::pair<std::string, int>>& rows, int N, int K) {
    Q3_CHECK(K % 256 == 0, "K must be a multiple of 256");
    Q8Mat m;
    m.N = N; m.Npad = (N + 31) & ~31; m.K = K;
    const int nrg = m.Npad / 32;
    std::vector<uint8_t> types((size_t)nrg, (uint8_t)Q3_T_Q8_0);
    bool kq = false;
    for (auto& r : rows) {
        const GgufTensor& t = g.need(r.first);
        if (t.type != Q3_T_Q8_0 && t.type != Q3_T_Q5_K && t.type != Q3_T_Q6_K)
            throw Error("tensor " + r.first + ": ggml type " + std::to_string(t.type) + " is not supported by the HIP path (Q8_0, Q5_K, Q6_K)");
        Q3_CHECK(r.second % 32 == 0 && t.ne[1] % 32 == 0 && r.second + t.ne[1] <= m.Npad, "bad row range for " + r.first);
        for (int64_t i = 0; i < t.ne[1] / 32; i++) types[(size_t)(r.second / 32 + i)] = (uint8_t)t.type;
        kq = kq || t.type != Q3_T_Q8_0;
    }
    std::vector<uint32_t> off((size_t)nrg);
    size_t qs_bytes = 0;
    for (int i = 0; i < nrg; i++) { off[(size_t)i] = (uint32_t)(qs_bytes / 16); qs_bytes += q3_rowgroup_bytes(kq ? types[(size_t)i] : Q3_T_Q8_0, K); }
    Q3_CHECK(qs_bytes / 16 < (1ull << 32), "matrix too large for 32-bit row-group offsets");
    const size_t sc_bytes = (size_t)m.Npad * (K / 32) * 2;
    const size_t meta_bytes = kq ? (size_t)m.Npad * (K / 256) * 16 : 0, ty_bytes = (size_t)((nrg + 15) & ~15), off_bytes = kq ? (size_t)((nrg * 4 + 15) & ~15) : 0;
    blobs_.emplace_back(qs_bytes + sc_bytes + meta_bytes + ty_bytes + off_bytes);
    blobs_.back().zero();
    uint8_t* base = blobs_.back().p;
    m.qs = base;
    m.sc = reinterpret_cast<const uint16_t*>(base + qs_bytes);
    mat_meta_[m.qs] = base + qs_bytes + sc_bytes;
    mat_types_[m.qs] = base + qs_bytes + sc_bytes + meta_bytes;
    mat_off_[m.qs] = reinterpret_cast<uint32_t*>(base + qs_bytes + sc_bytes + meta_bytes + ty_bytes);
    if (kq) {
        Q3_HIP(hipMemcpy(mat_types_[m.qs], types.data(), types.size(), hipMemcpyHostToDevice));
        Q3_HIP(hipMemcpy(mat_off_[m.qs], off.data(), off.size() * 4, hipMemcpyHostToDevice));
        m.meta = mat_meta_[m.qs]; m.rg_type = mat_types_[m.qs]; m.rg_off = mat_off_[m.qs]; m.qbytes = qs_bytes;
        all_q8_ = false;
        int last = -1;
        for (int i = 0; i < nrg; i++) {
            if (last == types[(size_t)i]) continue;
            last = types[(size_t)i];
            Q3_CHECK(m.nparts < 3, "more than 3 runs of weight types in one fused matrix");
            if (m.nparts == 0) { m.p0_type = last; m.p0_off = off[(size_t)i]; }
            else if (m.nparts == 1) { m.p1_rg0 = i; m.p1_type = last; m.p1_off = off[(size_t)i]; }
            else { m.p2_rg0 = i; m.p2_type = last; m.p2_off = off[(size_t)i]; }
            m.nparts++;
        }
    }
    for (auto& r : rows) load_into(g, r.first, m, r.second, K);
    return m;
}

void Transformer::load_into(const Gguf& g, const std::string& name, Q8Mat& dst, int row_off, int K_expect) {
    const GgufTensor& t = g.need(name);
    Q3_CHECK(t.ne[0] == K_expect, "unexpected K for " + name);
    DevBuf<uint8_t> raw(t.nbytes);
    raw.upload(t.data, t.nbytes);
    uint8_t* qs = const_cast<uint8_t*>(dst.qs);
    uint16_t* sc = const_cast<uint16_t*>(dst.sc);
    if (t.type == Q3_T_Q8_0) {
        const size_t nblk = (size_t)t.ne[1] * (t.ne[0] / 32);
        uint8_t* q0 = qs;
        int ro = row_off;
        if (dst.rg_off) {
            uint32_t o = 0;
            Q3_HIP(hipMemcpy(&o, dst.rg_off + row_off / 32, 4, hipMemcpyDeviceToHost));
            q0 = qs + (size_t)o * 16; ro = 0;
        }
        hipLaunchKernelGGL(k_repack_q8, dim3((unsigned)((nblk + 255) / 256)), dim3(256), 0, 0, raw.p, (int)t.ne[1], (int)t.ne[0], ro, q0, sc, row_off - ro);
    } else {
        const size_t nsb = (size_t)t.ne[1] * (t.ne[0] / 256);
        uint8_t* meta = mat_meta_.at(dst.qs);
        if (t.type == Q3_T_Q5_K) hipLaunchKernelGGL(k_repack_q5k, dim3((unsigned)((nsb + 255) / 256)), dim3(256), 0, 0, raw.p, (int)t.ne[1], (int)t.ne[0], row_off, qs, dst.rg_off, sc, meta);
        else hipLaunchKernelGGL(k_repack_q6k, dim3((unsigned)((nsb + 255) / 256)), dim3(256), 0, 0, raw.p, (int)t.ne[1], (int)t.ne[0], row_off, qs, dst.rg_off, sc, meta);
    }
    Q3_HIP(hipDeviceSynchronize());
}

FMat Transformer::make_fmat(const Gguf& g, const std::vector<std::string>& names, int K_expect) {
    FMat m;
    size_t total = 0;
    for (auto& n : names) {
        const GgufTensor& t = g.need(n);
        Q3_CHECK(t.ne[0] == K_expect && (t.type == Q3_T_F32 || t.type == Q3_T_F16 || t.type == Q3_T_BF16), "bad float tensor " + n);
        if (m.N == 0) m.type = t.type;
        Q3_CHECK(t.type == m.type, "mixed float types in one fused matrix: " + n);
        m.N += (int)t.ne[1]; total += t.nbytes;
    }
    m.K = K_expect;
    blobs_.emplace_back(total);
    size_t off = 0;
    for (auto& n : names) { const GgufTensor& t = g.need(n); Q3_HIP(hipMemcpy(blobs_.back().p + off, t.data, t.nbytes, hipMemcpyHostToDevice)); off += t.nbytes; }
    m.w = blobs_.back().p;
    if (K_expect % 256 == 0) {
        const size_t esz = m.type == Q3_T_F32 ? 4 : 2;
        blobs_.emplace_back((size_t)((m.N + 63) / 64) * 64 * K_expect * esz);
        launch_tile_float(nullptr, m.w, blobs_.back().p, m.type, m.N, K_expect);
        Q3_HIP(hipDeviceSynchronize());
        m.wt = blobs_.back().p;
    }
    return m;
}

float* Transformer::load_f32(const Gguf& g, const std::string& name, int64_t n_expect) {
    const GgufTensor& t = g.need(name);
    Q3_CHECK(t.type == Q3_T_F32 && t.ne[0] * t.rows() == n_expect, "bad f32 tensor " + name);
    blobs_.emplace_back((size_t)n_expect * 4);
    blobs_.back().upload(t.data, (size_t)n_expect * 4);
    return reinterpret_cast<float*>(blobs_.back().p);
}

Transformer::Transformer(const std::string& path, int n_ctx, int max_tok) : n_ctx_(n_ctx), max_tok_(max_tok) {
    init_kernel_attributes();
    if (const char* e = std::getenv("Q3_UNFUSED")) fused = !(e[0] == '1');
    Gguf g(path);
    hp_.arch = g.kv_str("general.architecture", "qwen3");
    auto K = [&](const char* s) { return hp_.arch + "." + s; };
    hp_.n_embd = (int)g.kv_int(K("embedding_length"), 0);
    hp_.n_layer = (int)g.kv_int(K("block_count"), 0);
    hp_.n_head = (int)g.kv_int(K("attention.head_count"), 0);
    hp_.n_kv = (int)g.kv_int(K("attention.head_count_kv"), hp_.n_head);
    const int head_dim = (int)g.kv_int(K("attention.key_length"), hp_.n_head ? hp_.n_embd / hp_.n_head : 0);
    hp_.n_ff = (int)g.kv_int(K("feed_forward_length"), 0);
    hp_.eps = (float)g.kv_float(K("attention.layer_norm_rms_epsilon"), 1e-6);
    hp_.rope_base = (float)g.kv_float(K("rope.freq_base"), 1e6);
    if (auto* s = g.kv(K("rope.dimension_sections")))
        for (size_t i = 0; i < s->arr_i.size() && i < 4; i++) hp_.mrope_sec[i] = (int32_t)s->arr_i[i];
    Q3_CHECK(hp_.n_embd > 0 && hp_.n_layer > 0 && hp_.n_head > 0 && head_dim == Q3_HEAD_DIM, "unsupported hparams");
    Q3_CHECK(hp_.n_embd % 256 == 0 && hp_.n_embd <= 2048 && hp_.n_ff % 256 == 0 && hp_.n_head % hp_.n_kv == 0, "unsupported dims");
    Q3_CHECK(hp_.n_head * 128 <= 2048, "n_head*128 must be <= 2048 (single super-segment o-proj)");
    const int d = hp_.n_embd, dq = hp_.n_head * 128, dkv = hp_.n_kv * 128, ff = hp_.n_ff;
    layers_.resize(hp_.n_layer);
    {
        const int t0 = g.need("blk.0.attn_q.weight").type;
        float_mode_ = (t0 == Q3_T_F32 || t0 == Q3_T_F16 || t0 == Q3_T_BF16);
    }
    for (int l = 0; l < hp_.n_layer; l++) {
        Layer& L = layers_[l];
        const std::string p = "blk." + std::to_string(l) + ".";
        if (float_mode_) {
            L.fqkv = make_fmat(g, {p + "attn_q.weight", p + "attn_k.weight", p + "attn_v.weight"}, d);
            L.fo = make_fmat(g, {p + "attn_output.weight"}, dq);
            L.fgu = make_fmat(g, {p + "ffn_gate.weight", p + "ffn_up.weight"}, d);
            L.fdown = make_fmat(g, {p + "ffn_down.weight"}, ff);
            L.attn_norm = load_f32(g, p + "attn_norm.weight", d);
            L.q_norm = load_f32(g, p + "attn_q_norm.weight", 128);
            L.k_norm = load_f32(g, p + "attn_k_norm.weight", 128);
            L.ffn_norm = load_f32(g, p + "ffn_norm.weight", d);
            const size_t lb = L.fqkv.bytes() + L.fo.bytes() + L.fgu.bytes() + L.fdown.bytes();
            if (l == 0) layer_weight_bytes_ = lb;
            weight_bytes_ += lb;
            continue;
        }
        L.wqkv = make_mat(g, {{p + "attn_q.weight", 0}, {p + "attn_k.weight", dq}, {p + "attn_v.weight", dq + dkv}}, dq + 2 * dkv, d);
        L.wo = make_mat(g, {{p + "attn_output.weight", 0}}, d, dq);
        L.wgu = make_mat(g, {{p + "ffn_gate.weight", 0}, {p + "ffn_up.weight", ff}}, 2 * ff, d);
        L.wdown = make_mat(g, {{p + "ffn_down.weight", 0}}, d, ff);
        if (L.wgu.nparts > 1) fused = false;
        L.attn_norm = load_f32(g, p + "attn_norm.weight", d);
        L.q_norm = load_f32(g, p + "attn_q_norm.weight", 128);
        L.k_norm = load_f32(g, p + "attn_k_norm.weight", 128);
        L.ffn_norm = load_f32(g, p + "ffn_norm.weight", d);
        if (l == 0) layer_weight_bytes_ = L.wqkv.bytes() + L.wo.bytes() + L.wgu.bytes() + L.wdown.bytes();
        weight_bytes_ += L.wqkv.bytes() + L.wo.bytes() + L.wgu.bytes() + L.wdown.bytes();
    }
    if (const char* e = std::getenv("Q3_SPEC")) ggml_mode_ = std::string(e) == "ggml";
    if (ggml_mode_) {
        Q3_CHECK(!float_mode_, "Q3_SPEC=ggml serves Q8_0 / Q5_K_M files (float-weight files have no ggml-mode kernels)");
        gg_layers_.resize(hp_.n_layer);
        for (int l = 0; l < hp_.n_layer; l++) {
            const std::string p = "blk." + std::to_string(l) + ".";
            GgLayer& G = gg_layers_[l];
            G.wq = gg_load(g, p + "attn_q.weight", dq, d); G.wk = gg_load(g, p + "attn_k.weight", dkv, d); G.wv = gg_load(g, p + "attn_v.weight", dkv, d);
            G.wo = gg_load(g, p + "attn_output.weight", d, dq);
            G.gate = gg_load(g, p + "ffn_gate.weight", ff, d); G.up = gg_load(g, p + "ffn_up.weight", ff, d); G.down = gg_load(g, p + "ffn_down.weight", d, ff);
        }
    }
    output_norm_ = load_f32(g, "output_norm.weight", d);
    const GgufTensor& ot = g.need("output.weight");
    hp_.n_vocab = (int)ot.ne[1];
    if (float_mode_) { foutput_ = make_fmat(g, {"output.weight"}, d); fused = false; }
    else output_ = make_mat(g, {{"output.weight", 0}}, hp_.n_vocab, d);
    if (ggml_mode_) gg_output_ = gg_load(g, "output.weight", hp_.n_vocab, d);
    std::vector<float> c((size_t)n_ctx * 64), s((size_t)n_ctx * 64);
    for (int p = 0; p < n_ctx; p++)
        for (int i = 0; i < 64; i++) {
            const double inv = std::pow((double)hp_.rope_base, -(double)i / 64.0);
            const double ang = (double)p * inv;
            c[(size_t)p * 64 + i] = (float)std::cos(ang);
            s[(size_t)p * 64 + i] = (float)std::sin(ang);
        }
    rope_cos_.alloc(c.size()); rope_cos_.upload(c.data(), c.size());
    rope_sin_.alloc(s.size()); rope_sin_.upload(s.data(), s.size());
    d_mrope_.alloc(4); d_mrope_.upload(hp_.mrope_sec, 4);
    alloc_workspace();
}

Transformer::Transformer(const Transformer& o, int max_tok)
    : fused(o.fused), float_mode_(o.float_mode_), foutput_(o.foutput_), hp_(o.hp_), n_ctx_(o.n_ctx_), max_tok_(max_tok), layers_(o.layers_), output_(o.output_),
      output_norm_(o.output_norm_), ws_(o.ws_), weight_bytes_(o.weight_bytes_), layer_weight_bytes_(o.layer_weight_bytes_), all_q8_(o.all_q8_),
      ggml_mode_(o.ggml_mode_), gg_layers_(o.gg_layers_), gg_output_(o.gg_output_) {
    alloc_workspace();
}

void Transformer::alloc_workspace() {
    const int d = hp_.n_embd, dq = hp_.n_head * 128, dkv = hp_.n_kv * 128, ff = hp_.n_ff;
    nparts_d_ = ((ff >> 8) + 7) / 8;
    const size_t T = (size_t)max_tok_;
    scratch_.alloc(T * 32); hid_.alloc(T * d); big_logits_.alloc(T * 2176);
    if (float_mode_) { xnf_.alloc(T * d); attf_.alloc(T * dq); actf_.alloc(T * ff); }
    h_.alloc(T * d); h2_.alloc(T * d); parts_o_.alloc(T * d); parts_d_.alloc((size_t)nparts_d_ * T * d);
    qkv_.alloc(T * (dq + 2 * dkv)); qrot_.alloc(T * dq); gu_.alloc(T * 2 * ff);
    const size_t mx = (size_t)(d > dq ? d : dq);
    xq_.alloc(T * mx); xd_.alloc(T * mx / 32); aq_.alloc(T * dq); ad_.alloc(T * dq / 32); fq_.alloc(T * ff); fd_.alloc(T * ff / 32);
    if (ggml_mode_) {
        const size_t kmax = (size_t)std::max(std::max(d, dq), ff);
        gg_q8_.alloc(T * kmax); gg_qk_.alloc(T * kmax); gg_d8_.alloc(T * kmax / 32); gg_dk_.alloc(T * kmax / 256); gg_bs_.alloc(T * kmax / 16);
        gg_xn_.alloc(T * kmax); gg_att_.alloc(T * dq); gg_act_f_.alloc(T * ff); gg_scores_.alloc(T * hp_.n_head * (size_t)n_ctx_);
        gg_act_ = GgAct{gg_q8_.p, gg_d8_.p, gg_qk_.p, gg_dk_.p, gg_bs_.p};
    }
}

GgMat Transformer::gg_load(const Gguf& g, const std::string& name, int n_expect, int k_expect) {
    const GgufTensor& t = g.need(name);
    Q3_CHECK((int)t.ne[0] == k_expect && (int)t.ne[1] == n_expect, "ggml mode: shape of " + name);
    Q3_CHECK(t.type == Q3_T_Q8_0 || t.type == Q3_T_Q5_K || t.type == Q3_T_Q6_K, "ggml mode: type of " + name);
    GgMat m; m.type = t.type; m.n = n_expect; m.k = k_expect;
    m.row_bytes = t.type == Q3_T_Q8_0 ? (size_t)(k_expect / 32) * 34 : t.type == Q3_T_Q5_K ? (size_t)(k_expect / 256) * 176 : (size_t)(k_expect / 256) * 210;
    blobs_.emplace_back(m.row_bytes * (size_t)n_expect);
    blobs_.back().upload(reinterpret_cast<const uint8_t*>(t.data), m.row_bytes * (size_t)n_expect);
    m.p = blobs_.back().p;
    return m;
}
void Transformer::gg_linear(hipStream_t st, const GgMat& w, int row0, int nrows, const float* x, float* out, int out_stride, int ntok) {
    gg_quant(st, x, w.k, gg_act_, ntok);
    gg_matvec(st, w, row0, nrows, gg_act_, out, out_stride, ntok);
}
void Transformer::forward_ggml(hipStream_t st, const Input& in, int ntok, const TokMeta& tm, const KvCache& kv, float* hidden_out) {
    const int d = hp_.n_embd, dq = hp_.n_head * 128, dkv = hp_.n_kv * 128, ff = hp_.n_ff, qs = dq + 2 * dkv;
    gg_load_rows(st, in.x, in.x_stride, in.idx, in.idx_stride, in.idx_keys, d, h_.p, ntok);
    for (int l = 0; l < hp_.n_layer; l++) {
        const Layer& L = layers_[l];
        const GgLayer& G = gg_layers_[l];
        gg_rmsnorm(st, h_.p, L.attn_norm, d, hp_.eps, gg_xn_.p, ntok);
        gg_quant(st, gg_xn_.p, d, gg_act_, ntok);
        gg_matvec(st, G.wq, 0, dq, gg_act_, qkv_.p, qs, ntok);
        gg_matvec(st, G.wk, 0, dkv, gg_act_, qkv_.p + dq, qs, ntok);
        gg_matvec(st, G.wv, 0, dkv, gg_act_, qkv_.p + dq + dkv, qs, ntok);
        gg_qk_rope_append(st, qkv_.p, qs, hp_.n_head, hp_.n_kv, L.q_norm, L.k_norm, hp_.eps, rope_cos_.p, rope_sin_.p, n_ctx_, d_mrope_.p, tm, kv, l, ntok);
        gg_attention(st, qkv_.p, qs, hp_.n_head, hp_.n_kv, tm, kv, l, gg_att_.p, gg_scores_.p, n_ctx_, ntok);
        gg_linear(st, G.wo, 0, d, gg_att_.p, parts_o_.p, d, ntok);
        gg_add(st, h_.p, parts_o_.p, (size_t)ntok * d);
        gg_rmsnorm(st, h_.p, L.ffn_norm, d, hp_.eps, gg_xn_.p, ntok);
        gg_quant(st, gg_xn_.p, d, gg_act_, ntok);
        gg_matvec(st, G.gate, 0, ff, gg_act_, gu_.p, ff, ntok);
        gg_matvec(st, G.up, 0, ff, gg_act_, gu_.p + (size_t)ntok * ff, ff, ntok);
        gg_swiglu(st, gu_.p, gu_.p + (size_t)ntok * ff, gg_act_f_.p, (size_t)ntok * ff);
        gg_linear(st, G.down, 0, d, gg_act_f_.p, parts_o_.p, d, ntok);
        gg_add(st, h_.p, parts_o_.p, (size_t)ntok * d);
    }
    gg_rmsnorm(st, h_.p, output_norm_, d, hp_.eps, hid_.p, ntok);
    if (hidden_out) launch_copy_f32(st, hid_.p, hidden_out, (size_t)ntok * d);
    Q3_LAUNCH_CHECK();
}


void Transformer::gemv(hipStream_t st, const Q8Mat& w, int row0, int nrows, const int8_t* xq, const uint16_t* xd, float* out,
                       int out_stride, int ntok) {
    if (timer) timer->begin(st);
    launch_gemv_q8(st, w, row0, nrows, xq, xd, out, out_stride, ntok);
    if (timer) timer->end(st, (double)nrows * ((double)w.K + (double)(w.K / 32) * 2.0));
}

void Transformer::forward(hipStream_t st, const Input& in, int ntok, const TokMeta& tm, const KvCache& kv, float* hidden_out) {
    Q3_CHECK(ntok >= 1 && ntok <= max_tok_, "ntok out of range");
    const int d = hp_.n_embd, dq = hp_.n_head * 128, dkv = hp_.n_kv * 128, ff = hp_.n_ff;
    if (ggml_mode_) { last_fused_ = false; last_ntok_ = ntok; forward_ggml(st, in, ntok, tm, kv, hidden_out); return; }
    if (float_mode_) { last_fused_ = false; last_ntok_ = ntok; forward_float(st, in, ntok, tm, kv, hidden_out); return; }
    const bool use_fused = fused && ntok <= fused_max_tok_;
    last_fused_ = use_fused; last_ntok_ = ntok;
    if (use_fused) {
        for (int l = 0; l < hp_.n_layer; l++) {
            const Layer& L = layers_[l];
            NormPro a{};
            if (l == 0) { a.h_in = in.x; a.h_stride = in.x_stride; a.idx_keys = in.idx_keys; a.idx_stride = in.idx_stride; a.nparts = 0; }
            else { a.h_in = h2_.p; a.h_stride = d; a.parts = parts_d_.p; a.nparts = nparts_d_; a.parts_stride = d; a.parts_slab = (size_t)ntok * d; }
            a.h_out = h_.p; a.g = L.attn_norm; a.eps = hp_.eps;
            if (timer) timer->begin(st);
            launch_gemv_q8_norm(st, L.wqkv, 0, dq + 2 * dkv, a, qkv_.p, dq + 2 * dkv, ntok, nullptr);
            if (timer) timer->end(st, (double)L.wqkv.bytes());
            if (same_seq_) {
                launch_qk_rope_append(st, qkv_.p, dq + 2 * dkv, nullptr, hp_.n_head, hp_.n_kv, L.q_norm, L.k_norm, hp_.eps, rope_cos_.p,
                                      rope_sin_.p, n_ctx_, d_mrope_.p, tm, kv, l, qrot_.p, ntok);
                launch_attention(st, qrot_.p, hp_.n_head, hp_.n_kv, tm, kv, l, nullptr, aq_.p, ad_.p, ntok);
            } else {
                if (short_attn_min_ > 0 && ntok >= short_attn_min_ && hp_.n_head == 2 * hp_.n_kv)
                    launch_attention_short(st, qkv_.p, dq + 2 * dkv, hp_.n_head, hp_.n_kv, L.q_norm, L.k_norm, hp_.eps, rope_cos_.p,
                                           rope_sin_.p, n_ctx_, d_mrope_.p, tm, kv, l, aq_.p, ad_.p, ntok);
                else
                launch_attention_fused(st, qkv_.p, dq + 2 * dkv, hp_.n_head, hp_.n_kv, L.q_norm, L.k_norm, hp_.eps, rope_cos_.p,
                                       rope_sin_.p, n_ctx_, d_mrope_.p, tm, kv, l, aq_.p, ad_.p, ntok);
            }
            gemv(st, L.wo, 0, d, aq_.p, ad_.p, parts_o_.p, d, ntok);
            NormPro b{};
            b.h_in = h_.p; b.h_stride = d; b.parts = parts_o_.p; b.nparts = 1; b.parts_stride = d; b.parts_slab = (size_t)ntok * d; b.h_out = h2_.p;
            b.g = L.ffn_norm; b.eps = hp_.eps;
            LaunchTimer* tg = timer_gu ? timer_gu : timer;
            if (tg) tg->begin(st);
            launch_gateup_swiglu(st, L.wgu, ff, b, fq_.p, fd_.p, ntok);
            if (tg) tg->end(st, (double)L.wgu.bytes());
            gemv(st, L.wdown, 0, d, fq_.p, fd_.p, parts_d_.p, d, ntok);
        }
        if (hidden_out) head(st, 0, ntok, 0, 0, nullptr, 0, nullptr, -1, hidden_out);
        Q3_LAUNCH_CHECK();
        return;
    }
    const bool wgnorm = ntok > 8;
    auto norm = [&](const NormArgs& a) {
        if (!wgnorm) { launch_rmsnorm_quant(st, a, ntok); return; }
        NormPro p{};
        p.h_in = a.h_in; p.h_stride = a.h_stride; p.idx_keys = a.idx_keys; p.idx_stride = a.idx_stride; p.parts = a.parts; p.nparts = a.nparts;
        p.parts_stride = a.parts_stride; p.parts_slab = (size_t)ntok * a.parts_stride; p.h_out = a.h_out; p.g = a.g; p.eps = a.eps; p.xn_out = a.xn_out;
        Q3_CHECK(a.idx == nullptr, "int32 row indices are not supported on the batched path");
        launch_rmsnorm_quant_wg(st, p, a.d, a.xq, a.xd, ntok);
    };
    for (int l = 0; l < hp_.n_layer; l++) {
        const Layer& L = layers_[l];
        NormArgs a{};
        if (l == 0) { a.h_in = in.x; a.h_stride = in.x_stride; a.idx = in.idx; a.idx_keys = in.idx_keys; a.idx_stride = in.idx_stride; a.nparts = 0; }
        else { a.h_in = h_.p; a.h_stride = d; a.parts = parts_d_.p; a.nparts = nparts_d_; a.parts_stride = d; }
        a.h_out = h_.p; a.g = L.attn_norm; a.eps = hp_.eps; a.d = d; a.xq = xq_.p; a.xd = xd_.p;
        norm(a);
        gemv(st, L.wqkv, 0, dq + 2 * dkv, xq_.p, xd_.p, qkv_.p, dq + 2 * dkv, ntok);
        if (short_attn_min_ > 0 && ntok >= short_attn_min_ && !same_seq_ && hp_.n_head == 2 * hp_.n_kv)
            launch_attention_short(st, qkv_.p, dq + 2 * dkv, hp_.n_head, hp_.n_kv, L.q_norm, L.k_norm, hp_.eps, rope_cos_.p, rope_sin_.p,
                                   n_ctx_, d_mrope_.p, tm, kv, l, aq_.p, ad_.p, ntok);
        else {
            launch_qk_rope_append(st, qkv_.p, dq + 2 * dkv, nullptr, hp_.n_head, hp_.n_kv, L.q_norm, L.k_norm, hp_.eps, rope_cos_.p,
                                  rope_sin_.p, n_ctx_, d_mrope_.p, tm, kv, l, qrot_.p, ntok);
            launch_attention(st, qrot_.p, hp_.n_head, hp_.n_kv, tm, kv, l, nullptr, aq_.p, ad_.p, ntok);
        }
        NormArgs b{};
        b.h_in = h_.p; b.h_stride = d; b.parts = parts_o_.p; b.nparts = 1; b.parts_stride = d; b.h_out = h_.p;
        b.g = L.ffn_norm; b.eps = hp_.eps; b.d = d; b.xq = xq_.p; b.xd = xd_.p;
        gemv(st, L.wo, 0, d, aq_.p, ad_.p, parts_o_.p, d, ntok);
        norm(b);
        bool gu_done = false;
        LaunchTimer* tg = timer_gu ? timer_gu : timer;
        if (fused) {
            if (tg) tg->begin(st);
            gu_done = launch_gateup_mfma(st, L.wgu, ff, xq_.p, xd_.p, fq_.p, fd_.p, ntok);
            if (tg && gu_done) tg->end(st, (double)L.wgu.bytes());
        }
        if (!gu_done) {
            if (tg) { tg->begin(st); launch_gemv_q8(st, L.wgu, 0, 2 * ff, xq_.p, xd_.p, gu_.p, 2 * ff, ntok); tg->end(st, (double)L.wgu.bytes()); }
            else
            gemv(st, L.wgu, 0, 2 * ff, xq_.p, xd_.p, gu_.p, 2 * ff, ntok);
            launch_swiglu_quant(st, gu_.p, ff, fq_.p, fd_.p, ntok);
        }
        gemv(st, L.wdown, 0, d, fq_.p, fd_.p, parts_d_.p, d, ntok);
        if (l + 1 == hp_.n_layer) {
            NormArgs nx{};
            nx.h_in = h_.p; nx.h_stride = d; nx.parts = parts_d_.p; nx.nparts = nparts_d_; nx.parts_stride = d; nx.eps = hp_.eps; nx.d = d; nx.xq = xq_.p; nx.xd = xd_.p;
            nx.h_out = nullptr; nx.g = output_norm_; nx.xn_out = hidden_out ? hidden_out : hid_.p;
            norm(nx);
        }
    }
    Q3_LAUNCH_CHECK();
}

void Transformer::forward_float(hipStream_t st, const Input& in, int ntok, const TokMeta& tm, const KvCache& kv, float* hidden_out) {
    const int d = hp_.n_embd, dq = hp_.n_head * 128, dkv = hp_.n_kv * 128, ff = hp_.n_ff;
    auto norm = [&](const float* h_in, int h_stride, const unsigned long long* idx_keys, int idx_stride, const float* parts, const float* g, float* xn) {
        NormArgs a{};
        a.h_in = h_in; a.h_stride = h_stride; a.idx_keys = idx_keys; a.idx_stride = idx_stride; a.parts = parts; a.nparts = parts ? 1 : 0; a.parts_stride = d;
        a.h_out = h_.p; a.g = g; a.eps = hp_.eps; a.d = d; a.xq = xq_.p; a.xd = xd_.p; a.xn_out = xn;
        if (ntok <= 8) { launch_rmsnorm_quant(st, a, ntok); return; }
        NormPro p{};
        p.h_in = a.h_in; p.h_stride = a.h_stride; p.idx_keys = a.idx_keys; p.idx_stride = a.idx_stride; p.parts = a.parts; p.nparts = a.nparts;
        p.parts_stride = a.parts_stride; p.parts_slab = (size_t)ntok * a.parts_stride; p.h_out = a.h_out; p.g = a.g; p.eps = a.eps; p.xn_out = a.xn_out;
        launch_rmsnorm_quant_wg(st, p, a.d, a.xq, a.xd, ntok);
    };
    auto fgemv = [&](const FMat& w, const float* x, int xs, float* out, int os) {
        if (timer) timer->begin(st);
        launch_gemv_float(st, w, 0, w.N, x, xs, out, os, ntok);
        if (timer) timer->end(st, (double)w.bytes());
    };
    for (int l = 0; l < hp_.n_layer; l++) {
        const Layer& L = layers_[l];
        if (l == 0) norm(in.x, in.x_stride, in.idx_keys, in.idx_stride, nullptr, L.attn_norm, xnf_.p);
        else norm(h_.p, d, nullptr, 0, parts_d_.p, L.attn_norm, xnf_.p);
        fgemv(L.fqkv, xnf_.p, d, qkv_.p, dq + 2 * dkv);
        if (short_attn_min_ > 0 && ntok >= short_attn_min_ && !same_seq_ && hp_.n_head == 2 * hp_.n_kv)
            launch_attention_short(st, qkv_.p, dq + 2 * dkv, hp_.n_head, hp_.n_kv, L.q_norm, L.k_norm, hp_.eps, rope_cos_.p, rope_sin_.p,
                                   n_ctx_, d_mrope_.p, tm, kv, l, aq_.p, ad_.p, ntok, attf_.p);
        else {
            launch_qk_rope_append(st, qkv_.p, dq + 2 * dkv, nullptr, hp_.n_head, hp_.n_kv, L.q_norm, L.k_norm, hp_.eps, rope_cos_.p, rope_sin_.p,
                                  n_ctx_, d_mrope_.p, tm, kv, l, qrot_.p, ntok);
            launch_attention(st, qrot_.p, hp_.n_head, hp_.n_kv, tm, kv, l, attf_.p, aq_.p, ad_.p, ntok);
        }
        fgemv(L.fo, attf_.p, dq, parts_o_.p, d);
        norm(h_.p, d, nullptr, 0, parts_o_.p, L.ffn_norm, xnf_.p);
        LaunchTimer* tg = timer_gu ? timer_gu : timer;
        if (tg) tg->begin(st);
        const bool gu_fused = launch_gateup_float(st, L.fgu, ff, xnf_.p, d, actf_.p, ntok);
        if (tg && gu_fused) tg->end(st, (double)L.fgu.bytes());
        if (!gu_fused) {
            if (tg) { tg->begin(st); launch_gemv_float(st, L.fgu, 0, L.fgu.N, xnf_.p, d, gu_.p, 2 * ff, ntok); tg->end(st, (double)L.fgu.bytes()); }
            else
            fgemv(L.fgu, xnf_.p, d, gu_.p, 2 * ff);
            launch_swiglu_f32(st, gu_.p, ff, actf_.p, ntok);
        }
        fgemv(L.fdown, actf_.p, ff, parts_d_.p, d);
    }
    norm(h_.p, d, nullptr, 0, parts_d_.p, output_norm_, hidden_out ? hidden_out : hid_.p);
    if (hidden_out) launch_copy_f32(st, hidden_out, hid_.p, (size_t)ntok * d);
    Q3_LAUNCH_CHECK();
}

void Transformer::head(hipStream_t st, int tok0, int tok_count, int row0, int nrows, float* logits, int logits_stride,
                       const ArgmaxEpi* am, int nrows_valid, float* hidden_out) {
    head_impl(st, tok0, tok_count, row0, nrows, logits, logits_stride, am, nrows_valid, hidden_out);
    Q3_LAUNCH_CHECK();
}
void Transformer::head_impl(hipStream_t st, int tok0, int tok_count, int row0, int nrows, float* logits, int logits_stride,
                            const ArgmaxEpi* am, int nrows_valid, float* hidden_out) {
    const int d = hp_.n_embd;
    Q3_CHECK(row0 % 32 == 0 && (float_mode_ || row0 + nrows <= output_.Npad), "head row range");
    if (ggml_mode_) {
        if (hidden_out) launch_copy_f32(st, hid_.p + (size_t)tok0 * d, hidden_out, (size_t)tok_count * d);
        if (nrows <= 0) return;
        int nr = nrows;
        if (row0 + nr > gg_output_.n) nr = gg_output_.n - row0;
        float* dst = am ? big_logits_.p : logits;
        const int ls = am ? nrows : logits_stride;
        if (am && big_logits_.n < (size_t)tok_count * nrows) throw Error("head scratch too small");
        gg_linear(st, gg_output_, row0, nr, hid_.p + (size_t)tok0 * d, dst, ls, tok_count);
        if (am) launch_argmax_keys(st, big_logits_.p, nrows, std::min(nrows_valid > 0 ? nrows_valid : nrows, nr), am->mask_per_tok, am->keys, am->key_stride, tok_count);
        return;
    }
    if (last_fused_) {
        NormPro f{};
        f.h_in = h2_.p + (size_t)tok0 * d; f.h_stride = d;
        f.parts = parts_d_.p + (size_t)tok0 * d; f.nparts = nparts_d_; f.parts_stride = d;
        f.parts_slab = (size_t)last_ntok_ * d;
        f.g = output_norm_; f.eps = hp_.eps; f.xn_out = hidden_out;
        if (nrows <= 0) {
            if (timer) timer->begin(st);
            launch_gemv_q8_norm(st, output_, 0, 32, f, scratch_logits(tok_count), 32, tok_count, nullptr);
            if (timer) timer->end(st, 32.0 * ((double)d * 1.0625));
            return;
        }
        if (timer) timer->begin(st);
        if (am) launch_gemv_q8_norm(st, output_, row0, nrows_valid > 0 ? nrows_valid : nrows, f, nullptr, 0, tok_count, am);
        else launch_gemv_q8_norm(st, output_, row0, nrows, f, logits, logits_stride, tok_count, nullptr);
        if (timer) timer->end(st, (double)nrows * ((double)d * 1.0625));
        return;
    }
    if (hidden_out) launch_copy_f32(st, hid_.p + (size_t)tok0 * d, hidden_out, (size_t)tok_count * d);
    if (nrows <= 0) return;
    if (float_mode_) {
        float* dst = am ? big_logits_.p : logits;
        const int ls = am ? nrows : logits_stride;
        if (timer) timer->begin(st);
        launch_gemv_float(st, foutput_, row0, nrows, hid_.p + (size_t)tok0 * d, d, dst, ls, tok_count);
        if (timer) timer->end(st, (double)nrows * d * (foutput_.type == Q3_T_F32 ? 4 : 2));
        if (am) launch_argmax_keys(st, big_logits_.p, nrows, nrows_valid > 0 ? nrows_valid : nrows, am->mask_per_tok, am->keys, am->key_stride, tok_count);
        return;
    }
    if (am) {
        const int nv = nrows_valid > 0 ? nrows_valid : nrows;
        if (big_logits_.n < (size_t)tok_count * nrows) throw Error("head scratch too small");
        gemv(st, output_, row0, nrows, xq_.p + (size_t)tok0 * d, xd_.p + (size_t)tok0 * (d / 32), big_logits_.p, nrows, tok_count);
        launch_argmax_keys(st, big_logits_.p, nrows, nv, am->mask_per_tok, am->keys, am->key_stride, tok_count);
        return;
    }
    gemv(st, output_, row0, nrows, xq_.p + (size_t)tok0 * d, xd_.p + (size_t)tok0 * (d / 32), logits, logits_stride, tok_count);
}

KvPool::KvPool(int n_layer, int n_kv, int n_pages, int n_seq, int max_pages_per_seq)
    : n_layer_(n_layer), n_kv_(n_kv), n_pages_(n_pages), n_seq_(n_seq), max_pages_(max_pages_per_seq) {
    const size_t per_page = (size_t)n_layer * n_kv * 8192;
    k_.alloc(per_page * n_pages); v_.alloc(per_page * n_pages);
    k_.zero(); v_.zero();
    const size_t nt = (size_t)n_seq * max_pages_per_seq;
    Q3_HIP(hipHostMalloc((void**)&table_, nt * sizeof(int32_t)));
    std::fill(table_, table_ + nt, 0);
    d_table_.alloc(nt);
    d_table_.upload(table_, nt);
    for (int p = n_pages - 1; p >= 0; p--) free_.push_back(p);
    used_pages_.assign(n_seq, 0);
}
KvCache KvPool::view() const {
    KvCache c;
    c.k = k_.p; c.v = v_.p; c.page_table = d_table_.p; c.max_pages = max_pages_; c.n_layer = n_layer_; c.n_kv = n_kv_;
    return c;
}
int KvPool::alloc_page() { Q3_CHECK(!free_.empty(), "KV pool exhausted"); int p = free_.back(); free_.pop_back(); return p; }
void KvPool::free_page(int p) { free_.push_back(p); }
void KvPool::assign(int seq, int lp, int pp) {
    table_[(size_t)seq * max_pages_ + lp] = pp;
    Q3_HIP(hipMemcpy(d_table_.p + (size_t)seq * max_pages_ + lp, &pp, 4, hipMemcpyHostToDevice));
}
void KvPool::ensure(int seq, int n_positions) {
    const int need = (n_positions + 63) / 64;
    Q3_CHECK(seq >= 0 && seq < n_seq_, "KV sequence index out of range");
    Q3_CHECK(need <= max_pages_ && need <= n_pages_, "sequence exceeds max pages");
    while (used_pages_[seq] < need) { assign(seq, used_pages_[seq], alloc_page()); used_pages_[seq]++; }
}
void KvPool::ensure(int seq, int n_positions, hipStream_t st) {
    const int need = (n_positions + 63) / 64;
    Q3_CHECK(seq >= 0 && seq < n_seq_, "KV sequence index out of range");
    Q3_CHECK(need <= max_pages_ && need <= n_pages_, "sequence exceeds max pages");
    const int first = used_pages_[seq];
    while (used_pages_[seq] < need) { table_[(size_t)seq * max_pages_ + used_pages_[seq]] = alloc_page(); used_pages_[seq]++; }
    if (need > first)
        Q3_HIP(hipMemcpyAsync(d_table_.p + (size_t)seq * max_pages_ + first, table_ + (size_t)seq * max_pages_ + first, (size_t)(need - first) * 4,
                              hipMemcpyHostToDevice, st));
}
KvPool::~KvPool() { if (table_) (void)hipHostFree(table_); }
void KvPool::release(int seq) {
    Q3_CHECK(seq >= 0 && seq < n_seq_, "KV sequence index out of range");
    for (int i = 0; i < used_pages_[seq]; i++) free_page(table_[(size_t)seq * max_pages_ + i]);
    used_pages_[seq] = 0;
}

}
```

### qwen3-tts-rust_amd/csrc/transformer.h

```cpp
#pragma once
#include "q3_common.h"
#include "gguf.h"
#include "kernels.h"
#include "ggml_mode.h"
#include <map>
#include <memory>

namespace q3 {

struct TfHparams {
    std::string arch;
    int n_embd = 0, n_layer = 0, n_head = 0, n_kv = 0, n_ff = 0, n_vocab = 0;
    float eps = 1e-6f, rope_base = 1e6f;
    int32_t mrope_sec[4] = {0, 0, 0, 0};
};

class Transformer {
public:
    Transformer(const std::string& gguf_path, int n_ctx, int max_tok);
    Transformer(const Transformer& weights_of, int max_tok);
    const TfHparams& hp() const { return hp_; }
    int n_ctx() const { return n_ctx_; }
    int max_tok() const { return max_tok_; }
    size_t weight_bytes() const { return weight_bytes_; }
    size_t layer_weight_bytes() const { return layer_weight_bytes_; }
    size_t head_bytes_per_row() const { return (size_t)hp_.n_embd + (size_t)(hp_.n_embd / 32) * 2; }

    struct Input {
        const float* x = nullptr; int x_stride = 0;
        const int32_t* idx = nullptr; int idx_stride = 0;
        const q3_u64* idx_keys = nullptr;
    };
    bool fused = true;
    void forward(hipStream_t st, const Input& in, int ntok, const TokMeta& tm, const KvCache& kv, float* hidden_out);
    void head(hipStream_t st, int tok0, int tok_count, int row0, int nrows, float* logits, int logits_stride,
              const ArgmaxEpi* am = nullptr, int nrows_valid = -1, float* hidden_out = nullptr);
    void set_same_seq_tokens(bool v) { same_seq_ = v; }
    void set_short_attention(int min_tok) { short_attn_min_ = min_tok; }
    void set_fused_max_tokens(int n) { fused_max_tok_ = n; }

    bool ggml_mode() const { return ggml_mode_; }

    LaunchTimer* timer = nullptr;
    LaunchTimer* timer_gu = nullptr;
    const Q8Mat& mat_qkv(int l) const { return layers_[l].wqkv; }
    const Q8Mat& mat_out() const { return output_; }

private:
    void head_impl(hipStream_t st, int tok0, int tok_count, int row0, int nrows, float* logits, int logits_stride, const ArgmaxEpi* am,
                   int nrows_valid, float* hidden_out);
    struct Layer { Q8Mat wqkv, wo, wgu, wdown; FMat fqkv, fo, fgu, fdown; float *attn_norm, *q_norm, *k_norm, *ffn_norm; };
    FMat make_fmat(const Gguf& g, const std::vector<std::string>& names, int K_expect);
    void forward_float(hipStream_t st, const Input& in, int ntok, const TokMeta& tm, const KvCache& kv, float* hidden_out);
    bool float_mode_ = false; FMat foutput_; DevBuf<float> xnf_, attf_, actf_;
    float* scratch_logits(int) { return scratch_.p; }
    DevBuf<float> scratch_, hid_, big_logits_;
    void gemv(hipStream_t st, const Q8Mat& w, int row0, int nrows, const int8_t* xq, const uint16_t* xd, float* out,
              int out_stride, int ntok);
    Q8Mat make_mat(const Gguf& g, const std::vector<std::pair<std::string, int>>& rows , int N, int K);
    void load_into(const Gguf& g, const std::string& name, Q8Mat& dst, int row_off, int K_expect);
    float* load_f32(const Gguf& g, const std::string& name, int64_t n_expect);
    TfHparams hp_;
    int n_ctx_ = 0, max_tok_ = 0;
    std::vector<Layer> layers_;
    Q8Mat output_;
    float* output_norm_ = nullptr;
    struct WeightStore {
        std::vector<DevBuf<uint8_t>> blobs; DevBuf<float> rope_cos, rope_sin; DevBuf<int32_t> d_mrope;
        std::map<const uint8_t*, uint8_t*> mat_meta, mat_types; std::map<const uint8_t*, uint32_t*> mat_off;
    };
    std::shared_ptr<WeightStore> ws_;
    std::vector<DevBuf<uint8_t>>& blobs_ = ws_init()->blobs;
    size_t weight_bytes_ = 0, layer_weight_bytes_ = 0;
    DevBuf<float>& rope_cos_ = ws_->rope_cos; DevBuf<float>& rope_sin_ = ws_->rope_sin;
    DevBuf<int32_t>& d_mrope_ = ws_->d_mrope;
    WeightStore* ws_init() { if (!ws_) ws_ = std::make_shared<WeightStore>(); return ws_.get(); }
    void alloc_workspace();
    DevBuf<float> h_, h2_, parts_o_, parts_d_, qkv_, qrot_, gu_;
    bool same_seq_ = false; int short_attn_min_ = 0; int fused_max_tok_ = 8; bool last_fused_ = false; int last_ntok_ = 0; bool all_q8_ = true;
    std::map<const uint8_t*, uint8_t*>& mat_meta_ = ws_->mat_meta; std::map<const uint8_t*, uint8_t*>& mat_types_ = ws_->mat_types; std::map<const uint8_t*, uint32_t*>& mat_off_ = ws_->mat_off;
    DevBuf<int8_t> xq_, aq_, fq_;
    DevBuf<uint16_t> xd_, ad_, fd_;
    int nparts_d_ = 1;
    struct GgLayer { GgMat wq, wk, wv, wo, gate, up, down; };
    bool ggml_mode_ = false;
    std::vector<GgLayer> gg_layers_;
    GgMat gg_output_;
    GgMat gg_load(const Gguf& g, const std::string& name, int n_expect, int k_expect);
    void forward_ggml(hipStream_t st, const Input& in, int ntok, const TokMeta& tm, const KvCache& kv, float* hidden_out);
    void gg_linear(hipStream_t st, const GgMat& w, int row0, int nrows, const float* x, float* out, int out_stride, int ntok);
    GgAct gg_act_{};
    DevBuf<int8_t> gg_q8_, gg_qk_; DevBuf<uint16_t> gg_d8_; DevBuf<float> gg_dk_, gg_xn_, gg_att_, gg_scores_, gg_act_f_; DevBuf<int16_t> gg_bs_;
};

Q8Mat q8mat_from_host(const void* raw_q8_0, int n, int k, DevBuf<uint8_t>& storage);
struct KqPart { const void* raw; int type; int rows; };
Q8Mat kqmat_from_host(const KqPart* parts, int nparts, int k, DevBuf<uint8_t>& storage);

class KvPool {
public:
    KvPool(int n_layer, int n_kv, int n_pages, int n_seq, int max_pages_per_seq);
    ~KvPool();
    KvPool(const KvPool&) = delete; KvPool& operator=(const KvPool&) = delete;
    KvCache view() const;
    int alloc_page();
    void free_page(int p);
    void assign(int seq, int logical_page, int physical_page);
    void ensure(int seq, int n_positions);
    void ensure(int seq, int n_positions, hipStream_t st);
    void release(int seq);
    int pages_free() const { return (int)free_.size(); }
    int page(int seq, int logical_page) const { return table_[(size_t)seq * max_pages_ + logical_page]; }
    size_t bytes() const { return (k_.n + v_.n) * 2; }
private:
    int n_layer_, n_kv_, n_pages_, n_seq_, max_pages_;
    DevBuf<uint16_t> k_, v_;
    DevBuf<int32_t> d_table_;
    int32_t* table_ = nullptr;
    std::vector<int> free_;
    std::vector<int> used_pages_;
};

}
```

### qwen3-tts-rust_amd/python/q3tts/__init__.py

```python
import ctypes as C
import os
import numpy as np

_HERE = os.path.dirname(os.path.abspath(__file__))
PKG_ROOT = os.path.dirname(os.path.dirname(_HERE))
LIB_PATH = os.path.join(PKG_ROOT, "libq3tts.so")
_lib = None


class Q3Error(RuntimeError):
    pass


class SamplerConfig(C.Structure):
    _fields_ = [("temperature", C.c_float), ("top_k", C.c_int32), ("top_p", C.c_float), ("has_seed", C.c_int32),
                ("seed", C.c_uint64)]


class GenOptions(C.Structure):
    _fields_ = [("repetition_penalty", C.c_float), ("predictor_temperature", C.c_float), ("predictor_top_k", C.c_int32),
                ("predictor_top_p", C.c_float)]


GEN_DEFAULTS = {"repetition_penalty": 1.0, "predictor_temperature": 0.0, "predictor_top_k": 0, "predictor_top_p": 1.0}


class EngineParams(C.Structure):
    _fields_ = [("model_dir", C.c_char_p), ("quant", C.c_char_p), ("device", C.c_int32), ("max_batch", C.c_int32),
                ("max_prompt", C.c_int32), ("max_steps", C.c_int32), ("load_codec", C.c_int32), ("use_graph", C.c_int32)]


class Request(C.Structure):
    _fields_ = [("prompt", C.c_void_p), ("n_prompt", C.c_int32), ("sampler", SamplerConfig), ("max_steps", C.c_int32),
                ("mask_eos", C.c_int32), ("codes_out", C.c_void_p), ("pcm_out", C.c_void_p), ("pcm_capacity", C.c_int64),
                ("n_frames", C.c_int32), ("n_pcm", C.c_int64), ("prefill_ms", C.c_double), ("first_chunk_ms", C.c_double),
                ("total_ms", C.c_double)]


class Stats(C.Structure):
    _fields_ = [("frame_loop_ms", C.c_double), ("frames", C.c_int64), ("prefill_ms", C.c_double), ("gemv_ms", C.c_double),
                ("gemv_launches", C.c_int64), ("gemv_bytes", C.c_double), ("codec_ms", C.c_double), ("codec_calls", C.c_int64),
                ("talker_weight_bytes", C.c_double), ("predictor_weight_bytes", C.c_double), ("kv_bytes_per_token", C.c_double),
                ("gu_ms", C.c_double), ("gu_launches", C.c_int64), ("gu_bytes", C.c_double),
                ("sched_steps", C.c_int64), ("slot_frames", C.c_double), ("graph_frames", C.c_int64)]


class ReqStatus(C.Structure):
    _fields_ = [("state", C.c_int32), ("n_frames", C.c_int32), ("n_pcm", C.c_int64), ("queue_ms", C.c_double),
                ("prefill_ms", C.c_double), ("first_chunk_ms", C.c_double), ("total_ms", C.c_double)]


REQ_QUEUED, REQ_RUNNING, REQ_DRAINING, REQ_DONE, REQ_FAILED = 0, 1, 2, 3, -1


DECODE_CB = C.CFUNCTYPE(None, C.c_void_p, C.POINTER(C.c_int64), C.c_int32, C.c_int32)

SYMBOLS = [
    "q3tts_last_error", "q3tts_version", "q3tts_device_count", "q3tts_sampler_config_default", "q3tts_engine_params_default",
    "q3tts_engine_create", "q3tts_engine_destroy", "q3tts_generate_batch", "q3tts_engine_stats", "q3tts_engine_reset_stats",
    "q3tts_engine_set_instrument", "q3tts_engine_bytes_per_step", "q3tts_assets_open", "q3tts_assets_close", "q3tts_engine_assets",
    "q3tts_assets_codec_embedding", "q3tts_assets_text_embedding", "q3tts_assets_tts_pad", "q3tts_prompt_build_core",
    "q3tts_prompt_build_clone", "q3tts_sampler_new", "q3tts_sampler_free", "q3tts_sampler_sample", "q3tts_chunker_new",
    "q3tts_chunker_free", "q3tts_chunker_push", "q3tts_decoder_create", "q3tts_decoder_destroy", "q3tts_decoder_samples_per_frame",
    "q3tts_decoder_reset", "q3tts_decoder_decode", "q3tts_mel_frames", "q3tts_mel", "q3tts_tf_open", "q3tts_tf_close",
    "q3tts_tf_dims", "q3tts_tf_clear", "q3tts_tf_eval", "q3tts_op_gemv_q8", "q3tts_op_gateup_q8", "q3tts_op_matmul_float", "q3tts_op_rmsnorm_quant", "q3tts_op_swiglu_quant",
    "q3tts_op_argmax", "q3tts_op_project", "q3tts_op_sample", "q3tts_submit", "q3tts_poll", "q3tts_fetch", "q3tts_wait",
    "q3tts_release", "q3tts_decoder_create_ex", "q3tts_decoder_decode_group", "q3tts_sched_start", "q3tts_sched_stop", "q3tts_sched_step", "q3tts_voice_register", "q3tts_submit_text",
    "q3tts_group_create", "q3tts_group_destroy", "q3tts_group_size", "q3tts_group_engine", "q3tts_group_uses_rccl", "q3tts_group_voice_register",
    "q3tts_group_submit", "q3tts_group_submit_text", "q3tts_group_device_of", "q3tts_group_poll", "q3tts_group_fetch", "q3tts_group_wait",
    "q3tts_group_release", "q3tts_group_start", "q3tts_group_stop", "q3tts_comm_available", "q3tts_comm_unique_id", "q3tts_comm_create",
    "q3tts_comm_destroy", "q3tts_comm_voice_register", "q3tts_engine_device",
    "q3tts_onnx_open", "q3tts_onnx_close", "q3tts_onnx_counts", "q3tts_onnx_summary", "q3tts_onnx_node", "q3tts_onnx_node_input", "q3tts_onnx_node_output",
    "q3tts_onnx_node_attr_ints", "q3tts_onnx_node_attr_float", "q3tts_onnx_initializer", "q3tts_onnx_op_kernel", "q3tts_onnx_decoder_contract",
    "q3tts_onnx_session_open", "q3tts_onnx_session_close", "q3tts_onnx_session_unsupported", "q3tts_onnx_session_set_input", "q3tts_onnx_session_run",
    "q3tts_onnx_session_output_info", "q3tts_onnx_session_output", "q3tts_onnx_session_launches", "q3tts_onnx_op_executable",
    "q3tts_text_nfc", "q3tts_op_gemv_kq", "q3tts_op_gateup_kq", "q3tts_onnx_decoder_open", "q3tts_onnx_decoder_close", "q3tts_onnx_decoder_reset", "q3tts_onnx_decoder_fetch", "q3tts_group_info", "q3tts_onnx_decoder_decode",
    "q3tts_decoder_state_floats", "q3tts_decoder_state_export", "q3tts_decoder_state_import", "q3tts_decoder_state_entry",
    "q3tts_tokenizer_open", "q3tts_tokenizer_close", "q3tts_tokenizer_encode", "q3tts_tokenizer_decode", "q3tts_tokenizer_vocab_size",
    "q3tts_gen_options_default", "q3tts_submit_ex", "q3tts_submit_text_ex", "q3tts_generate_batch_ex", "q3tts_group_submit_ex",
    "q3tts_group_submit_text_ex", "q3tts_op_sample_rows",
    "q3tts_prompt_build_streaming", "q3tts_submit_trailing", "q3tts_submit_text_streaming", "q3tts_generate_batch_trailing",
    "q3tts_group_submit_text_streaming", "q3tts_op_codec_gemm", "q3tts_codec_gemm_plan",
]


def lib():
    global _lib
    if _lib is None:
        if not os.path.exists(LIB_PATH):
            raise Q3Error("libq3tts.so not built (run qwen3-tts-rust_amd/build.sh); there is no CPU fallback")
        L = C.CDLL(LIB_PATH)
        L.q3tts_last_error.restype = C.c_char_p
        L.q3tts_engine_create.argtypes = [C.POINTER(EngineParams), C.POINTER(C.c_void_p)]
        L.q3tts_engine_destroy.argtypes = [C.c_void_p]
        L.q3tts_generate_batch.argtypes = [C.c_void_p, C.POINTER(Request), C.c_int32, C.c_int32]
        L.q3tts_engine_stats.argtypes = [C.c_void_p, C.POINTER(Stats)]
        L.q3tts_submit.argtypes = [C.c_void_p, C.POINTER(Request), C.c_int32, C.POINTER(C.c_int64)]
        L.q3tts_poll.argtypes = [C.c_void_p, C.c_int64, C.POINTER(ReqStatus)]
        L.q3tts_fetch.argtypes = [C.c_void_p, C.c_int64, C.c_void_p, C.c_int32, C.c_int32, C.c_void_p, C.c_int64, C.c_int64,
                                  C.POINTER(C.c_int32), C.POINTER(C.c_int64)]
        L.q3tts_wait.argtypes = [C.c_void_p, C.c_int64, C.c_double]
        L.q3tts_release.argtypes = [C.c_void_p, C.c_int64]
        L.q3tts_sched_start.argtypes = [C.c_void_p]
        L.q3tts_sched_stop.argtypes = [C.c_void_p]
        L.q3tts_sched_step.argtypes = [C.c_void_p, C.POINTER(C.c_int32)]
        L.q3tts_voice_register.argtypes = [C.c_void_p, C.c_void_p, C.c_void_p, C.c_int32, C.c_void_p, C.c_int32, C.POINTER(C.c_int32)]
        L.q3tts_submit_text.argtypes = [C.c_void_p, C.c_int32, C.c_void_p, C.c_int32, C.c_int32, C.c_void_p, C.c_int32,
                                        C.POINTER(SamplerConfig), C.c_int32, C.c_int32, C.c_int32, C.POINTER(C.c_int64)]
        L.q3tts_engine_reset_stats.argtypes = [C.c_void_p]
        L.q3tts_engine_set_instrument.argtypes = [C.c_void_p, C.c_int32]
        L.q3tts_engine_bytes_per_step.restype = C.c_double
        L.q3tts_engine_bytes_per_step.argtypes = [C.c_void_p, C.c_int32, C.c_double]
        L.q3tts_assets_open.argtypes = [C.c_char_p, C.POINTER(C.c_void_p)]
        L.q3tts_assets_close.argtypes = [C.c_void_p]
        L.q3tts_engine_assets.restype = C.c_void_p
        L.q3tts_engine_assets.argtypes = [C.c_void_p]
        L.q3tts_assets_codec_embedding.argtypes = [C.c_void_p, C.c_int32, C.c_int32, C.c_void_p]
        L.q3tts_assets_text_embedding.argtypes = [C.c_void_p, C.c_int64, C.c_void_p]
        L.q3tts_assets_tts_pad.argtypes = [C.c_void_p, C.c_void_p]
        L.q3tts_prompt_build_core.argtypes = [C.c_void_p, C.c_void_p, C.c_int32, C.c_int32, C.c_int32, C.c_void_p, C.c_void_p,
                                              C.c_int32, C.c_void_p, C.c_int32, C.c_void_p, C.c_int32]
        L.q3tts_prompt_build_clone.argtypes = [C.c_void_p, C.c_void_p, C.c_int32, C.c_void_p, C.c_int32, C.c_void_p, C.c_int32,
                                               C.c_void_p, C.c_int32, C.c_void_p, C.c_int32, C.c_void_p, C.c_int32]
        L.q3tts_sampler_new.restype = C.c_void_p
        L.q3tts_sampler_new.argtypes = [C.c_float, C.c_int32, C.c_float, C.c_uint64]
        L.q3tts_sampler_free.argtypes = [C.c_void_p]
        L.q3tts_sampler_sample.restype = C.c_int32
        L.q3tts_sampler_sample.argtypes = [C.c_void_p, C.c_void_p, C.c_int32, C.c_int32, C.c_int32]
        L.q3tts_chunker_new.restype = C.c_void_p
        L.q3tts_chunker_new.argtypes = [DECODE_CB, C.c_void_p]
        L.q3tts_chunker_free.argtypes = [C.c_void_p]
        L.q3tts_chunker_push.argtypes = [C.c_void_p, C.c_void_p, C.c_int32, C.c_int32]
        L.q3tts_decoder_create.argtypes = [C.c_char_p, C.c_int32, C.POINTER(C.c_void_p)]
        L.q3tts_decoder_destroy.argtypes = [C.c_void_p]
        L.q3tts_decoder_create_ex.argtypes = [C.c_char_p, C.c_int32, C.c_int32, C.c_int32, C.POINTER(C.c_void_p)]
        L.q3tts_decoder_decode_group.argtypes = [C.c_void_p, C.c_int32, C.c_void_p, C.c_void_p, C.c_int32, C.c_void_p]
        L.q3tts_decoder_samples_per_frame.argtypes = [C.c_void_p]
        L.q3tts_decoder_reset.argtypes = [C.c_void_p, C.c_int32]
        L.q3tts_decoder_decode.argtypes = [C.c_void_p, C.c_int32, C.c_void_p, C.c_int32, C.c_int32, C.c_void_p, C.POINTER(C.c_int64)]
        L.q3tts_mel_frames.argtypes = [C.c_int32]
        L.q3tts_mel.argtypes = [C.c_void_p, C.c_int32, C.c_void_p]
        L.q3tts_tf_open.argtypes = [C.c_char_p, C.c_int32, C.c_int32, C.POINTER(C.c_void_p)]
        L.q3tts_tf_close.argtypes = [C.c_void_p]
        L.q3tts_tf_dims.argtypes = [C.c_void_p] + [C.POINTER(C.c_int32)] * 4
        L.q3tts_tf_clear.argtypes = [C.c_void_p]
        L.q3tts_tf_eval.argtypes = [C.c_void_p, C.c_void_p, C.c_void_p, C.c_int32, C.c_void_p, C.c_void_p, C.c_int32, C.c_int32]
        L.q3tts_op_gemv_q8.argtypes = [C.c_void_p, C.c_int32, C.c_int32, C.c_void_p, C.c_void_p, C.c_int32, C.c_void_p, C.c_int32]
        L.q3tts_op_gateup_q8.argtypes = [C.c_void_p, C.c_int32, C.c_int32, C.c_void_p, C.c_void_p, C.c_int32, C.c_void_p, C.c_void_p]
        L.q3tts_op_matmul_float.argtypes = [C.c_void_p, C.c_int32, C.c_int32, C.c_int32, C.c_int32, C.c_int32, C.c_void_p, C.c_int32, C.c_void_p]
        L.q3tts_op_rmsnorm_quant.argtypes = [C.c_void_p, C.c_void_p, C.c_int32, C.c_int32, C.c_float, C.c_void_p, C.c_void_p, C.c_void_p]
        L.q3tts_op_swiglu_quant.argtypes = [C.c_void_p, C.c_int32, C.c_int32, C.c_void_p, C.c_void_p]
        L.q3tts_op_argmax.argtypes = [C.c_void_p, C.c_int32, C.c_int32, C.c_int32, C.c_int32, C.c_void_p]
        L.q3tts_op_sample.argtypes = [C.c_void_p, C.c_int32, C.c_float, C.c_int32, C.c_float, C.c_uint64, C.c_int32, C.c_int32, C.c_void_p]
        L.q3tts_op_project.argtypes = [C.c_void_p, C.c_void_p, C.c_void_p, C.c_int32, C.c_int32, C.c_void_p]
        L.q3tts_gen_options_default.argtypes = [C.POINTER(GenOptions)]
        L.q3tts_submit_ex.argtypes = [C.c_void_p, C.POINTER(Request), C.c_int32, C.POINTER(GenOptions), C.POINTER(C.c_int64)]
        L.q3tts_submit_text_ex.argtypes = [C.c_void_p, C.c_int32, C.c_void_p, C.c_int32, C.c_int32, C.c_void_p, C.c_int32,
                                           C.POINTER(SamplerConfig), C.c_int32, C.c_int32, C.c_int32, C.POINTER(GenOptions),
                                           C.POINTER(C.c_int64)]
        L.q3tts_generate_batch_ex.argtypes = [C.c_void_p, C.POINTER(Request), C.c_int32, C.c_int32, C.POINTER(GenOptions)]
        L.q3tts_group_submit_ex.argtypes = [C.c_void_p, C.POINTER(Request), C.c_int32, C.POINTER(GenOptions), C.POINTER(C.c_int64)]
        L.q3tts_group_submit_text_ex.argtypes = [C.c_void_p, C.c_int32, C.c_void_p, C.c_int32, C.c_int32, C.c_void_p, C.c_int32,
                                                 C.POINTER(SamplerConfig), C.c_int32, C.c_int32, C.c_int32, C.POINTER(GenOptions),
                                                 C.POINTER(C.c_int64)]
        L.q3tts_op_sample_rows.argtypes = [C.c_int32, C.c_void_p, C.c_int32, C.c_int32, C.c_void_p, C.c_void_p, C.c_void_p, C.c_void_p,
                                           C.c_void_p, C.c_void_p, C.c_void_p, C.c_int32, C.c_int32, C.c_void_p]
        L.q3tts_prompt_build_streaming.argtypes = [C.c_void_p, C.c_void_p, C.c_int32, C.c_int32, C.c_int32, C.c_void_p, C.c_void_p, C.c_int32,
                                                   C.c_void_p, C.c_int32, C.c_void_p, C.c_int32, C.c_void_p, C.c_int32, C.c_void_p, C.c_int32,
                                                   C.POINTER(C.c_int32)]
        L.q3tts_submit_trailing.argtypes = [C.c_void_p, C.POINTER(Request), C.c_int32, C.POINTER(GenOptions), C.c_void_p, C.c_int32,
                                            C.POINTER(C.c_int64)]
        L.q3tts_submit_text_streaming.argtypes = L.q3tts_submit_text_ex.argtypes
        L.q3tts_generate_batch_trailing.argtypes = [C.c_void_p, C.POINTER(Request), C.c_int32, C.c_int32, C.POINTER(GenOptions),
                                                    C.POINTER(C.c_void_p), C.c_void_p]
        L.q3tts_group_submit_text_streaming.argtypes = L.q3tts_group_submit_text_ex.argtypes
        _lib = L
    return _lib


def _p(a):
    return a.ctypes.data_as(C.c_void_p) if a is not None else None


def _chk(rc):
    if rc != 0:
        raise Q3Error(lib().q3tts_last_error().decode())


def device_count():
    return lib().q3tts_device_count()


class Assets:
    def __init__(self, path=None, handle=None):
        self._own = handle is None
        if handle is None:
            h = C.c_void_p()
            _chk(lib().q3tts_assets_open(path.encode(), C.byref(h)))
            handle = h.value
        self.h = handle

    def close(self):
        if self._own and self.h:
            lib().q3tts_assets_close(self.h)
        self.h = None

    def codec_embedding(self, q, code):
        out = np.zeros(2048, np.float32)
        _chk(lib().q3tts_assets_codec_embedding(self.h, q, code, _p(out)))
        return out

    def text_embedding(self, tok):
        out = np.zeros(2048, np.float32)
        _chk(lib().q3tts_assets_text_embedding(self.h, tok, _p(out)))
        return out

    def tts_pad(self):
        out = np.zeros(2048, np.float32)
        _chk(lib().q3tts_assets_tts_pad(self.h, _p(out)))
        return out

    def build_core(self, text_ids, lang_id=2055, spk_id=None, spk_emb=None, instr_ids=None, mid=None, max_rows=4096):
        t = np.ascontiguousarray(text_ids, np.int32)
        ins = np.ascontiguousarray(instr_ids, np.int32) if instr_ids is not None else None
        se = np.ascontiguousarray(spk_emb, np.float32) if spk_emb is not None else None
        md = np.ascontiguousarray(mid, np.float32) if mid is not None else None
        out = np.zeros((max_rows, 2048), np.float32)
        n = lib().q3tts_prompt_build_core(self.h, _p(t), t.size, -1 if lang_id is None else lang_id,
                                          -1 if spk_id is None else spk_id, _p(se), _p(ins), ins.size if ins is not None else 0,
                                          _p(md), md.shape[0] if md is not None else 0, _p(out), max_rows)
        if n < 0:
            raise Q3Error(lib().q3tts_last_error().decode())
        return out[:n].copy()

    def build_clone(self, text_ids, ref_codes, ref_text_ids, spk_emb, lang_id=2055, instr_ids=None, max_rows=4096):
# ... 327 lines not shown
        return wav


def op_gemv_q8(w_raw, n, k, xq, xd, lpr=0):
    xq = np.ascontiguousarray(xq, np.int8).reshape(-1, k)
    xd = np.ascontiguousarray(xd, np.uint16).reshape(-1, k // 32)
    w_raw = np.ascontiguousarray(w_raw, np.uint8)
    y = np.zeros((xq.shape[0], n), np.float32)
    _chk(lib().q3tts_op_gemv_q8(_p(w_raw), n, k, _p(xq), _p(xd), xq.shape[0], _p(y), lpr))
    return y


def op_gateup_q8(w_raw, ff, k, xq, xd):
    xq = np.ascontiguousarray(xq, np.int8).reshape(-1, k)
    xd = np.ascontiguousarray(xd, np.uint16).reshape(-1, k // 32)
    w_raw = np.ascontiguousarray(w_raw, np.uint8)
    aq = np.zeros((xq.shape[0], ff), np.int8)
    ad = np.zeros((xq.shape[0], ff // 32), np.uint16)
    _chk(lib().q3tts_op_gateup_q8(_p(w_raw), ff, k, _p(xq), _p(xd), xq.shape[0], _p(aq), _p(ad)))
    return aq, ad


def op_matmul_float(w_raw, ggml_type, n, k, x, row0=0, nrows=None):
    nrows = n - row0 if nrows is None else nrows
    w_raw = np.ascontiguousarray(w_raw)
    x = np.ascontiguousarray(x, np.float32)
    y = np.zeros((x.shape[0], nrows), np.float32)
    _chk(lib().q3tts_op_matmul_float(_p(w_raw), ggml_type, n, k, row0, nrows, _p(x), x.shape[0], _p(y)))
    return y


def op_rmsnorm_quant(x, g, eps=1e-6):
    x = np.ascontiguousarray(x, np.float32)
    x2 = x.reshape(-1, x.shape[-1])
    d = x2.shape[1]
    g = np.ascontiguousarray(g, np.float32)
    xq = np.zeros(x2.shape, np.int8)
    xd = np.zeros((x2.shape[0], d // 32), np.uint16)
    xn = np.zeros(x2.shape, np.float32)
    _chk(lib().q3tts_op_rmsnorm_quant(_p(x2), _p(g), d, x2.shape[0], eps, _p(xq), _p(xd), _p(xn)))
    return xq, xd, xn


def op_swiglu_quant(gu, ff):
    gu = np.ascontiguousarray(gu, np.float32).reshape(-1, 2 * ff)
    aq = np.zeros((gu.shape[0], ff), np.int8)
    ad = np.zeros((gu.shape[0], ff // 32), np.uint16)
    _chk(lib().q3tts_op_swiglu_quant(_p(gu), ff, gu.shape[0], _p(aq), _p(ad)))
    return aq, ad


def op_argmax(logits, start, end, mask_idx=-1):
    logits = np.ascontiguousarray(logits, np.float32)
    out = np.zeros(1, np.int32)
    _chk(lib().q3tts_op_argmax(_p(logits), logits.size, start, end, mask_idx, _p(out)))
    return int(out[0])


def op_sample(logits, temperature, top_k, top_p, seed, n_draws=1, mask_idx=-1):
    logits = np.ascontiguousarray(logits, dtype=np.float32)
    out = np.zeros(n_draws, dtype=np.int32)
    _chk(lib().q3tts_op_sample(_p(logits), logits.size, temperature, top_k, top_p, seed, mask_idx, n_draws, _p(out)))
    return out


def op_sample_rows(logits, temperature, top_k, top_p, seed, n_draws=1, kernel=0, penalty=None, history=None):
    lg = np.ascontiguousarray(logits, np.float32)
    B, n = lg.shape
    t = np.ascontiguousarray(np.broadcast_to(np.asarray(temperature, np.float32), (B,)))
    k = np.ascontiguousarray(np.broadcast_to(np.asarray(top_k, np.int32), (B,)))
    p = np.ascontiguousarray(np.broadcast_to(np.asarray(top_p, np.float32), (B,)))
    s = np.ascontiguousarray(np.broadcast_to(np.asarray(seed, np.uint64), (B,)))
    pen = hist = hlen = None
    cap = 1
    if penalty is not None:
        pen = np.ascontiguousarray(np.broadcast_to(np.asarray(penalty, np.float32), (B,)))
        history = history if history is not None else [[] for _ in range(B)]
        cap = max(1, max(len(h) for h in history))
        hist = np.full((B, cap), -1, np.int32)
        hlen = np.array([len(h) for h in history], np.int32)
        for b, h in enumerate(history):
            hist[b, : len(h)] = h
    out = np.zeros((n_draws, B), np.int32)
    _chk(lib().q3tts_op_sample_rows(kernel, _p(lg), B, n, _p(t), _p(k), _p(p), _p(pen), _p(s), _p(hist), _p(hlen), cap, n_draws, _p(out)))
    return out


def op_project(x, w, b):
    x = np.ascontiguousarray(x, np.float32)
    w = np.ascontiguousarray(w, np.float32)
    b = np.ascontiguousarray(b, np.float32)
    y = np.zeros(b.size, np.float32)
    _chk(lib().q3tts_op_project(_p(x), _p(w), _p(b), x.size, b.size, _p(y)))
    return y


GEMM_FORMS = {"AUTO": 0, "SKINNY4": 1, "SKINNY8": 2, "SKINNY16": 3, "F32_1": 4, "F32_2": 5, "H1": 6, "H1_EPL": 7, "H2": 8, "H2_EPL": 9,
              "H3": 10, "H3_EPL": 11}
GEMM_FORM_NAMES = {v: k for k, v in GEMM_FORMS.items()}
EPI_NONE, EPI_GELU, EPI_RES_SCALE, EPI_RES, EPI_SNAKE = range(5)


class CodecGemmDesc(C.Structure):
    _fields_ = [("M", C.c_int32), ("N", C.c_int32), ("cin", C.c_int32), ("taps", C.c_int32), ("dil", C.c_int32),
                ("A", C.c_void_p), ("a_rows", C.c_int64), ("lda", C.c_int32), ("a_segT", C.c_int32), ("a_skip", C.c_int32),
                ("a_split", C.c_int32), ("o_split", C.c_int32),
                ("W", C.c_void_p), ("bias", C.c_void_p),
                ("epi", C.c_int32), ("res", C.c_void_p), ("res_floats", C.c_int64), ("ldr", C.c_int32), ("r_segT", C.c_int32), ("r_skip", C.c_int64),
                ("scale", C.c_void_p), ("snake_ea", C.c_void_p), ("snake_ib", C.c_void_p),
                ("out", C.c_void_p), ("out_floats", C.c_int64), ("out_off", C.c_int64), ("ldo", C.c_int32), ("o_segT", C.c_int32), ("o_skip", C.c_int64),
                ("ws_floats", C.c_int64),
                ("form", C.c_int32), ("ksplit", C.c_int32), ("reducer", C.c_int32),
                ("form_ran", C.c_int32), ("ksplit_ran", C.c_int32), ("reducer_ran", C.c_int32)]


def _codec_gemm_desc(M, N, cin, taps, dil, lda, a_rows, a_segT, a_skip, epi, ldr, res_floats, r_segT, r_skip, ldo, out_floats, out_off,
                     o_segT, o_skip, a_split, o_split, ws_floats, form, ksplit, reducer):
    d = CodecGemmDesc()
    d.M, d.N, d.cin, d.taps, d.dil = M, N, cin, taps, dil
    d.lda, d.a_rows, d.a_segT, d.a_skip = lda, a_rows, a_segT, a_skip
    d.epi, d.ldr, d.res_floats, d.r_segT, d.r_skip = epi, ldr, res_floats, r_segT, r_skip
    d.ldo, d.out_floats, d.out_off, d.o_segT, d.o_skip = ldo, out_floats, out_off, o_segT, o_skip
    d.a_split, d.o_split, d.ws_floats = int(bool(a_split)), int(bool(o_split)), ws_floats
    d.form = GEMM_FORMS[form] if isinstance(form, str) else form
    d.ksplit, d.reducer = ksplit, reducer
    return d


def op_codec_gemm(A, W, M, cin, taps=1, dil=1, out=None, ldo=None, out_off=0, o_segT=0, o_skip=0, a_segT=0, a_skip=0, bias=None,
                  epi=EPI_NONE, res=None, ldr=0, r_segT=0, r_skip=0, scale=None, ea=None, ib=None, a_split=False, o_split=False,
                  ws_floats=1 << 22, form="AUTO", ksplit=1, reducer=-1):
    A = np.ascontiguousarray(A)
    assert A.ndim == 2 and A.dtype.itemsize == 4
    W = np.ascontiguousarray(W, np.float32)
    N = W.shape[0]
    ldo = N if ldo is None else ldo
    if out is None:
        out = np.zeros(out_off + M * ldo, np.float32)
    out = np.array(out, copy=True).reshape(-1)
    assert out.dtype.itemsize == 4
    vecs = [None if v is None else np.ascontiguousarray(v, np.float32) for v in (bias, scale, ea, ib)]
    for v in vecs:
        assert v is None or v.size == N
    res = None if res is None else np.ascontiguousarray(res, np.float32).reshape(-1)
    d = _codec_gemm_desc(M, N, cin, taps, dil, A.shape[1], A.shape[0], a_segT, a_skip, epi, ldr, 0 if res is None else res.size, r_segT, r_skip,
                         ldo, out.size, out_off, o_segT, o_skip, a_split, o_split, ws_floats, form, ksplit, reducer)
    d.A, d.W, d.out, d.res = _p(A), _p(W), _p(out), _p(res)
    d.bias, d.scale, d.snake_ea, d.snake_ib = (_p(v) for v in vecs)
    lib().q3tts_op_codec_gemm.argtypes = [C.POINTER(CodecGemmDesc)]
    _chk(lib().q3tts_op_codec_gemm(C.byref(d)))
    return out, (GEMM_FORM_NAMES[d.form_ran], d.ksplit_ran, d.reducer_ran)


def codec_gemm_plan(M, N, cin, taps=1, dil=1, lda=None, ldo=None, out_off=0, o_segT=0, o_skip=0, a_segT=0, a_skip=0, epi=EPI_NONE, ldr=0,
                    r_segT=0, r_skip=0, a_split=False, o_split=False, ws_floats=1 << 22):
    d = _codec_gemm_desc(M, N, cin, taps, dil, cin if lda is None else lda, 0, a_segT, a_skip, epi, ldr, 0, r_segT, r_skip,
                         N if ldo is None else ldo, 0, out_off, o_segT, o_skip, a_split, o_split, ws_floats, 0, 1, -1)
    lib().q3tts_codec_gemm_plan.argtypes = [C.POINTER(CodecGemmDesc)]
    _chk(lib().q3tts_codec_gemm_plan(C.byref(d)))
    return GEMM_FORM_NAMES[d.form_ran], d.ksplit_ran, d.reducer_ran


def mel(audio):
    audio = np.ascontiguousarray(audio, np.float32)
    n = lib().q3tts_mel_frames(audio.size)
    out = np.zeros((n, 128), np.float32)
    _chk(lib().q3tts_mel(_p(audio), audio.size, _p(out)))
    return out


class OnnxSession:

    def __init__(self, path, device=0):
        L = lib()
        L.q3tts_onnx_session_open.argtypes = [C.c_char_p, C.c_int32, C.POINTER(C.c_void_p)]
        L.q3tts_onnx_session_close.argtypes = [C.c_void_p]
        L.q3tts_onnx_session_unsupported.argtypes = [C.c_void_p, C.c_char_p, C.c_int64]
        L.q3tts_onnx_session_set_input.argtypes = [C.c_void_p, C.c_char_p, C.c_int32, C.c_void_p, C.c_void_p, C.c_int32]
        L.q3tts_onnx_session_run.argtypes = [C.c_void_p]
        L.q3tts_onnx_session_output_info.argtypes = [C.c_void_p, C.c_char_p, C.POINTER(C.c_int32), C.POINTER(C.c_int32), C.c_void_p]
        L.q3tts_onnx_session_output.argtypes = [C.c_void_p, C.c_char_p, C.c_void_p, C.c_int64]
        L.q3tts_onnx_session_launches.restype = C.c_int64
        L.q3tts_onnx_session_launches.argtypes = [C.c_void_p]
        h = C.c_void_p()
        _chk(L.q3tts_onnx_session_open(path.encode(), device, C.byref(h)))
        self.h = h.value

    def close(self):
        if self.h:
            lib().q3tts_onnx_session_close(self.h)
        self.h = None

    def unsupported(self):
        buf = C.create_string_buffer(4096)
        n = lib().q3tts_onnx_session_unsupported(self.h, buf, 4096)
        return [x for x in buf.value.decode().split(",") if x] if n else []

    def run(self, feeds, outputs):
        keep = []
        for name, arr in feeds.items():
            a = np.ascontiguousarray(arr, dtype=np.int64 if np.issubdtype(np.asarray(arr).dtype, np.integer) else np.float32)
            keep.append(a)
            shape = (C.c_int64 * max(a.ndim, 1))(*a.shape)
            _chk(lib().q3tts_onnx_session_set_input(self.h, name.encode(), 7 if a.dtype == np.int64 else 1, a.ctypes.data, shape, a.ndim))
        _chk(lib().q3tts_onnx_session_run(self.h))
        res = {}
        for name in outputs:
            dt, rk = C.c_int32(), C.c_int32()
            shape = (C.c_int64 * 8)()
            _chk(lib().q3tts_onnx_session_output_info(self.h, name.encode(), C.byref(dt), C.byref(rk), shape))
            shp = tuple(shape[i] for i in range(rk.value))
            out = np.empty(shp, dtype=np.int64 if dt.value == 7 else np.float32)
            _chk(lib().q3tts_onnx_session_output(self.h, name.encode(), out.ctypes.data, out.nbytes))
            res[name] = out.astype(bool) if dt.value == 9 else out
        return res

    def launches(self):
        return lib().q3tts_onnx_session_launches(self.h)


class OnnxDecoder:

    def __init__(self, path, device=0):
        L = lib()
        L.q3tts_onnx_decoder_open.argtypes = [C.c_char_p, C.c_int32, C.POINTER(C.c_void_p)]
        L.q3tts_onnx_decoder_close.argtypes = [C.c_void_p]
        L.q3tts_onnx_decoder_reset.argtypes = [C.c_void_p]
        L.q3tts_onnx_decoder_decode.argtypes = [C.c_void_p, C.c_void_p, C.c_int32, C.c_int32, C.c_void_p, C.c_int64, C.POINTER(C.c_int64)]
        h = C.c_void_p()
        _chk(L.q3tts_onnx_decoder_open(path.encode(), device, C.byref(h)))
        self.h = h.value

    def close(self):
        if self.h:
            lib().q3tts_onnx_decoder_close(self.h)
        self.h = None

    def reset(self):
        _chk(lib().q3tts_onnx_decoder_reset(self.h))

    def decode(self, codes, is_final=False, max_samples_per_frame=1920):
        codes = np.ascontiguousarray(codes, np.int64).reshape(-1, 16)
        out = np.zeros(max(codes.shape[0], 1) * max_samples_per_frame, np.float32)
        n = C.c_int64()
        rc = lib().q3tts_onnx_decoder_decode(self.h, codes.ctypes.data, codes.shape[0], 1 if is_final else 0, out.ctypes.data, out.size, C.byref(n))
        if rc == 2:
            out = np.zeros(n.value, np.float32)
            lib().q3tts_onnx_decoder_fetch.argtypes = [C.c_void_p, C.c_void_p, C.c_int64, C.POINTER(C.c_int64)]
            rc = lib().q3tts_onnx_decoder_fetch(self.h, out.ctypes.data, out.size, C.byref(n))
        _chk(rc)
        return out[: n.value].copy()


def op_gemv_kq(parts, k, xq, xd, lpr=0):
    L = lib()
    L.q3tts_op_gemv_kq.argtypes = [C.c_void_p, C.c_void_p, C.c_void_p, C.c_int32, C.c_int32, C.c_void_p, C.c_void_p, C.c_int32, C.c_void_p, C.c_int32]
    raws = [np.ascontiguousarray(p[0]) for p in parts]
    ptrs = (C.c_void_p * len(parts))(*[r.ctypes.data for r in raws])
    types = np.asarray([p[1] for p in parts], np.int32); rows = np.asarray([p[2] for p in parts], np.int32)
    xq = np.ascontiguousarray(xq, np.int8); xd = np.ascontiguousarray(xd, np.uint16)
    ntok = xq.shape[0]
    y = np.zeros((ntok, int(rows.sum())), np.float32)
    _chk(L.q3tts_op_gemv_kq(ptrs, types.ctypes.data, rows.ctypes.data, len(parts), k, xq.ctypes.data, xd.ctypes.data, ntok, y.ctypes.data, lpr))
    return y


def op_gateup_kq(gate_raw, up_raw, qtype, ff, k, xq, xd):
    L = lib()
    L.q3tts_op_gateup_kq.argtypes = [C.c_void_p, C.c_void_p, C.c_int32, C.c_int32, C.c_int32, C.c_void_p, C.c_void_p, C.c_int32, C.c_void_p, C.c_void_p]
    g = np.ascontiguousarray(gate_raw); u = np.ascontiguousarray(up_raw)
    xq = np.ascontiguousarray(xq, np.int8); xd = np.ascontiguousarray(xd, np.uint16)
    ntok = xq.shape[0]
    aq = np.zeros((ntok, ff), np.int8); ad = np.zeros((ntok, ff // 32), np.uint16)
    _chk(L.q3tts_op_gateup_kq(g.ctypes.data, u.ctypes.data, qtype, ff, k, xq.ctypes.data, xd.ctypes.data, ntok, aq.ctypes.data, ad.ctypes.data))
    return aq, ad


def text_nfc(text):
    L = lib()
    L.q3tts_text_nfc.restype = C.c_int64
    L.q3tts_text_nfc.argtypes = [C.c_char_p, C.c_char_p, C.c_int64]
    raw = text.encode("utf-8", "surrogatepass")
    n = L.q3tts_text_nfc(raw, None, 0)
    buf = C.create_string_buffer(int(n))
    L.q3tts_text_nfc(raw, buf, n)
    return buf.raw[: n - 1].decode("utf-8", "surrogatepass")


def onnx_op_executable(op_type):
    L = lib()
    L.q3tts_onnx_op_executable.argtypes = [C.c_char_p]
    return bool(L.q3tts_onnx_op_executable(op_type.encode()))


class OnnxModel:

    def __init__(self, path):
        L = lib()
        L.q3tts_onnx_open.argtypes = [C.c_char_p, C.POINTER(C.c_void_p)]
        L.q3tts_onnx_close.argtypes = [C.c_void_p]
        L.q3tts_onnx_counts.argtypes = [C.c_void_p] + [C.POINTER(C.c_int32)] * 4
        L.q3tts_onnx_summary.restype = C.c_int64
        L.q3tts_onnx_summary.argtypes = [C.c_void_p, C.c_char_p, C.c_int64]
        L.q3tts_onnx_node.argtypes = [C.c_void_p, C.c_int32, C.POINTER(C.c_char_p), C.POINTER(C.c_char_p)] + [C.POINTER(C.c_int32)] * 3
        L.q3tts_onnx_node_input.restype = C.c_char_p
        L.q3tts_onnx_node_input.argtypes = [C.c_void_p, C.c_int32, C.c_int32]
# ... 100 lines not shown
```

Measured before the change: 701.2.

## Route decode attention through fused kernel serving two q heads per kv head

Enables the fused QK-norm/RoPE/KV-append/attention kernel by default in the decode path, replacing the separate rope-append plus attention launches when the short kernel does not apply. The fused kernel gains a template option that processes both query heads sharing a kv head in one workgroup, so each K/V chunk is loaded once for two heads. It also uses scalar loads for routing metadata, packed FMAs, and a shared KV-chunk loader. A test C API and Python binding for the attention variants are added. The cost is more LDS and registers per workgroup and fewer workgroups when HPW=2.

```diff
diff --git a/include/q3tts.h b/include/q3tts.h
--- a/include/q3tts.h
+++ b/include/q3tts.h
@@ -288,6 +288,28 @@
 int q3tts_op_codec_gemm(q3tts_codec_gemm_desc* d);
 int q3tts_codec_gemm_plan(q3tts_codec_gemm_desc* d);
 
+enum { Q3TTS_ATTN_PAIR = 0,
+       Q3TTS_ATTN_FUSED1 = 1,
+       Q3TTS_ATTN_FUSED2 = 2,
+       Q3TTS_ATTN_SHORT1 = 3,
+       Q3TTS_ATTN_SHORT2 = 4 };
+typedef struct q3tts_decode_attn_desc {
+    int32_t kernel;
+    int32_t n_head, n_kv, ntok, n_ctx;
+    int32_t n_layer, layer, n_pages;
+    const float* qkv;
+    const float* q_norm; const float* k_norm; float eps;
+    const float* rope_cos; const float* rope_sin;
+    const int32_t* mrope_sec;
+    const int32_t* seq; const int32_t* slot; const int32_t* pos;
+    int32_t uniform_pos;
+    const int32_t* page_table; int32_t max_pages;
+    uint16_t* k_cache; uint16_t* v_cache;
+    int8_t* aq; uint16_t* ad;
+    float* att;
+} q3tts_decode_attn_desc;
+int q3tts_op_decode_attention(q3tts_decode_attn_desc* d);
+
 #ifdef __cplusplus
 }
 #endif
diff --git a/qwen3-tts-rust_amd/csrc/capi_ops.cpp b/qwen3-tts-rust_amd/csrc/capi_ops.cpp
--- a/qwen3-tts-rust_amd/csrc/capi_ops.cpp
+++ b/qwen3-tts-rust_amd/csrc/capi_ops.cpp
@@ -241,6 +241,67 @@
     Q3_API_END(Q3TTS_ERR)
 }
 
+int q3tts_op_decode_attention(q3tts_decode_attn_desc* d) {
+    Q3_API_BEGIN
+    require_gpu();
+    Q3_CHECK(d && d->qkv && d->q_norm && d->k_norm && d->rope_cos && d->rope_sin && d->mrope_sec && d->k_cache && d->v_cache && d->aq && d->ad,
+             "null argument");
+    const int nh = d->n_head, nkv = d->n_kv, ntok = d->ntok, kern = d->kernel;
+    Q3_CHECK(nh >= 1 && nkv >= 1 && nh % nkv == 0 && ntok >= 1 && d->n_ctx >= 1 && d->n_layer >= 1 && d->layer >= 0 && d->layer < d->n_layer &&
+             d->n_pages >= 1 && kern >= Q3TTS_ATTN_PAIR && kern <= Q3TTS_ATTN_SHORT2, "bad decode-attention shape");
+    Q3_CHECK(kern == Q3TTS_ATTN_PAIR || kern == Q3TTS_ATTN_FUSED1 || nh == 2 * nkv, "this kernel serves exactly two q heads per kv head");
+    Q3_CHECK(d->uniform_pos >= 0 || (d->seq && d->slot && d->pos), "per-token routing needs seq, slot and pos");
+    Q3_CHECK(!d->page_table || d->max_pages >= 1, "bad page table");
+    const int n_seq = d->uniform_pos >= 0 ? ntok : [&] { int m = 0; for (int t = 0; t < ntok; t++) m = std::max(m, d->seq[t] + 1); return m; }();
+    for (int t = 0; t < ntok; t++) {
+        const int seq = d->uniform_pos >= 0 ? t : d->seq[t], slot = d->uniform_pos >= 0 ? d->uniform_pos : d->slot[t];
+        Q3_CHECK(seq >= 0 && slot >= 0, "negative sequence or slot");
+        Q3_CHECK(kern < Q3TTS_ATTN_SHORT1 || slot < 64, "the single-wave kernel serves contexts of one page");
+        for (int lp = 0; lp <= slot >> 6; lp++) {
+            Q3_CHECK(!d->page_table || lp < d->max_pages, "slot beyond the page table row");
+            const int pg = d->page_table ? d->page_table[(size_t)seq * d->max_pages + lp] : seq;
+            Q3_CHECK(pg >= 0 && pg < d->n_pages, "page outside the cache");
+        }
+    }
+    const int dq = nh * 128, dqkv = (nh + 2 * nkv) * 128;
+    const size_t cache_halfs = (size_t)d->n_pages * d->n_layer * nkv * 8192;
+    DevBuf<float> dqkv_((size_t)ntok * dqkv), dqn(128), dkn(128), dcos((size_t)d->n_ctx * 64), dsin((size_t)d->n_ctx * 64), dqrot((size_t)ntok * dq);
+    DevBuf<int32_t> dsec(4), dseq(ntok), dslot(ntok), dpos((size_t)ntok * 4), dpt(d->page_table ? (size_t)n_seq * d->max_pages : 1);
+    DevBuf<uint16_t> dk(cache_halfs), dv(cache_halfs), dad((size_t)ntok * (dq / 32));
+    DevBuf<int8_t> daq((size_t)ntok * dq);
+    DevBuf<float> datt(d->att ? (size_t)ntok * dq : 1);
+    dqkv_.upload(d->qkv, dqkv_.n); dqn.upload(d->q_norm, 128); dkn.upload(d->k_norm, 128);
+    dcos.upload(d->rope_cos, dcos.n); dsin.upload(d->rope_sin, dsin.n); dsec.upload(d->mrope_sec, 4);
+    dk.upload(d->k_cache, cache_halfs); dv.upload(d->v_cache, cache_halfs);
+    TokMeta tm{};
+    tm.uniform_pos = d->uniform_pos >= 0 ? d->uniform_pos : -1;
+    if (tm.uniform_pos < 0) {
+        dseq.upload(d->seq, ntok); dslot.upload(d->slot, ntok); dpos.upload(d->pos, dpos.n);
+        tm.seq = dseq.p; tm.slot = dslot.p; tm.pos = dpos.p;
+    }
+    KvCache kv{};
+    kv.k = dk.p; kv.v = dv.p; kv.n_layer = d->n_layer; kv.n_kv = nkv; kv.max_pages = d->page_table ? d->max_pages : 1;
+    if (d->page_table) { dpt.upload(d->page_table, dpt.n); kv.page_table = dpt.p; }
+    float* att = d->att ? datt.p : nullptr;
+    if (kern == Q3TTS_ATTN_PAIR) {
+        launch_qk_rope_append(0, dqkv_.p, dqkv, nullptr, nh, nkv, dqn.p, dkn.p, d->eps, dcos.p, dsin.p, d->n_ctx, dsec.p, tm, kv, d->layer, dqrot.p, ntok);
+        launch_attention(0, dqrot.p, nh, nkv, tm, kv, d->layer, att, daq.p, dad.p, ntok);
+    } else if (kern == Q3TTS_ATTN_FUSED1 || kern == Q3TTS_ATTN_FUSED2) {
+        launch_attention_fused(0, dqkv_.p, dqkv, nh, nkv, dqn.p, dkn.p, d->eps, dcos.p, dsin.p, d->n_ctx, dsec.p, tm, kv, d->layer, daq.p, dad.p,
+                               ntok, kern == Q3TTS_ATTN_FUSED2 ? 2 : 1, att);
+    } else {
+        launch_attention_short(0, dqkv_.p, dqkv, nh, nkv, dqn.p, dkn.p, d->eps, dcos.p, dsin.p, d->n_ctx, dsec.p, tm, kv, d->layer, daq.p, dad.p,
+                               ntok, att, kern == Q3TTS_ATTN_SHORT2 ? 2 : 1);
+    }
+    Q3_LAUNCH_CHECK();
+    Q3_HIP(hipDeviceSynchronize());
+    dk.download(d->k_cache, cache_halfs); dv.download(d->v_cache, cache_halfs);
+    daq.download(d->aq, daq.n); dad.download(d->ad, dad.n);
+    if (d->att) datt.download(d->att, datt.n);
+    return Q3TTS_OK;
+    Q3_API_END(Q3TTS_ERR)
+}
+
 int q3tts_codec_gemm_plan(q3tts_codec_gemm_desc* d) {
     Q3_API_BEGIN
     codec_gemm_plan_only(d);
diff --git a/qwen3-tts-rust_amd/csrc/kernels.h b/qwen3-tts-rust_amd/csrc/kernels.h
--- a/qwen3-tts-rust_amd/csrc/kernels.h
+++ b/qwen3-tts-rust_amd/csrc/kernels.h
@@ -108,11 +108,12 @@
 void launch_attention_fused(hipStream_t st, const float* qkv, int qkv_stride, int n_head, int n_kv, const float* q_norm_w,
                             const float* k_norm_w, float eps, const float* rope_cos, const float* rope_sin, int n_ctx,
                             const int32_t* mrope_sec, const TokMeta& tm, const KvCache& kv, int layer, int8_t* aq, uint16_t* ad,
-                            int ntok);
+                            int ntok, int hpw = 1 ,
+                            float* att = nullptr );
 void launch_attention_short(hipStream_t st, const float* qkv, int qkv_stride, int n_head, int n_kv, const float* q_norm_w,
                             const float* k_norm_w, float eps, const float* rope_cos, const float* rope_sin, int n_ctx,
                             const int32_t* mrope_sec, const TokMeta& tm, const KvCache& kv, int layer, int8_t* aq, uint16_t* ad, int ntok,
-                            float* att = nullptr );
+                            float* att = nullptr , int hpw = 0 );
 void launch_project_blk(hipStream_t st, const float* x, int x_stride, const float* Wblk , const float* b,
                         int n_in, int n_out, float* out, int out_stride, int ntok);
 struct TextTrail {
diff --git a/qwen3-tts-rust_amd/csrc/kernels_fused.hip b/qwen3-tts-rust_amd/csrc/kernels_fused.hip
--- a/qwen3-tts-rust_amd/csrc/kernels_fused.hip
+++ b/qwen3-tts-rust_amd/csrc/kernels_fused.hip
@@ -312,79 +312,108 @@
 #undef Q3_GU
 }
 
+typedef __attribute__((address_space(4))) const int32_t q3_cint;
+__device__ __forceinline__ int sload(const int32_t* p, size_t i) { return ((q3_cint*)p)[i]; }
+struct TokRoute { int seq, slot, pos[4]; };
+__device__ __forceinline__ TokRoute tok_route(const TokMeta& tm, int tok) {
+    TokRoute r;
+    if (tm.uniform_pos >= 0) { r.seq = tok; r.slot = tm.uniform_pos; for (int i = 0; i < 4; i++) r.pos[i] = tm.uniform_pos; }
+    else {
+        r.seq = sload(tm.seq, tok); r.slot = sload(tm.slot, tok);
+        for (int i = 0; i < 4; i++) r.pos[i] = sload(tm.pos, (size_t)tok * 4 + i);
+    }
+    return r;
+}
+__device__ __forceinline__ int rope_row(const TokRoute& r, const int32_t* mrope_sec, int lane, int n_ctx) {
+    const int32_t sec[4] = { sload(mrope_sec, 0), sload(mrope_sec, 1), sload(mrope_sec, 2), sload(mrope_sec, 3) };
+    const int s = q3_mrope_stream(lane, sec);
+    int pp = s == 0 ? r.pos[0] : s == 1 ? r.pos[1] : s == 2 ? r.pos[2] : r.pos[3];
+    if (pp < 0) pp = 0;
+    if (pp > n_ctx - 1) pp = n_ctx - 1;
+    return pp;
+}
+__device__ __forceinline__ int page_at(const KvCache& kv, int seq, int logical) {
+    return kv.page_table ? sload(kv.page_table, (size_t)seq * kv.max_pages + logical) : seq;
+}
+__device__ __forceinline__ void load_kv_chunk(const KvCache& kv, size_t head_off, int seq, int lp0, int lpl, int cn, int wave, int lane,
+                                              uint4 (&kreg)[16], uint4 (&vreg)[16]) {
+    int pg[4];
+#pragma unroll
+    for (int i = 0; i < 4; i++) pg[i] = page_at(kv, seq, lp0 + i < lpl ? lp0 + i : lpl);
+    const int pw = wave == 0 ? pg[0] : wave == 1 ? pg[1] : wave == 2 ? pg[2] : pg[3];
+    const uint16_t* Kb = kv.k + (size_t)pw * kv.page_stride() + head_off;
+#pragma unroll
+    for (int d8 = 0; d8 < 16; d8++)
+        kreg[d8] = 64 * wave < cn ? *reinterpret_cast<const uint4*>(Kb + (d8 * 64 + lane) * 8) : make_uint4(0, 0, 0, 0);
+#pragma unroll
+    for (int u = 0; u < 16; u++) {
+        const int uc = 16 * u < cn ? u : (cn - 1) >> 4;
+        const uint16_t* Vb = kv.v + (size_t)pg[uc >> 2] * kv.page_stride() + head_off;
+        vreg[u] = *reinterpret_cast<const uint4*>(Vb + (16 * (uc & 3) + 4 * wave + (lane >> 4)) * 128 + (lane & 15) * 8);
+    }
+}
+typedef float q3_f2v __attribute__((ext_vector_type(2)));
+__device__ __forceinline__ q3_f2v pk_fma(float q0, float q1, float k, q3_f2v acc) { const q3_f2v qq = {q0, q1}, kk = {k, k}; return __builtin_elementwise_fma(qq, kk, acc); }
+template <int HPW>
 __global__ void __launch_bounds__(256) k_attention_fused(const float* __restrict__ qkv, int qkv_stride, int n_head, int n_kv,
                                                          const float* __restrict__ q_norm_w, const float* __restrict__ k_norm_w,
                                                          float eps, const float* __restrict__ rope_cos,
                                                          const float* __restrict__ rope_sin, int n_ctx,
                                                          const int32_t* __restrict__ mrope_sec, TokMeta tm, KvCache kv, int layer,
-                                                         int8_t* __restrict__ aq, uint16_t* __restrict__ ad) {
-    __shared__ __attribute__((aligned(16))) float q_s[128];
+                                                         int8_t* __restrict__ aq, uint16_t* __restrict__ ad, float* __restrict__ att) {
+    __shared__ __attribute__((aligned(16))) float q_s[128 * HPW];
     __shared__ __attribute__((aligned(16))) uint16_t kcur_s[128];
     __shared__ __attribute__((aligned(16))) uint16_t vcur_s[128];
-    __shared__ float p_s[256];
-    __shared__ float red_s[4][128];
-    __shared__ float wmax_s[4];
-    const int h = blockIdx.x, tok = blockIdx.y, tid = threadIdx.x, lane = tid & 63, wave = tid >> 6;
-    const int seq = tm.seq_of(tok), slot = tm.slot_of(tok), n = slot + 1;
-    const int grp = n_head / n_kv, kvh = h / grp;
+    __shared__ float p_s[HPW][256];
+    __shared__ float red_s[HPW][4][128];
+    __shared__ float wmax_s[HPW][4];
+    const int tok = blockIdx.y, tid = threadIdx.x, lane = tid & 63;
+    const int wave = __builtin_amdgcn_readfirstlane(tid >> 6);
+    const int grp = n_head / n_kv;
+    const int kvh = HPW == 2 ? blockIdx.x : blockIdx.x / grp, h0 = HPW == 2 ? 2 * blockIdx.x : blockIdx.x;
+    const bool writer = HPW == 2 || h0 % grp == 0;
+    const TokRoute r = tok_route(tm, tok);
+    const int seq = r.seq, slot = r.slot, n = slot + 1, lpl = slot >> 6;
     const size_t head_off = (size_t)layer * kv.layer_stride() + (size_t)kvh * 8192;
     const int jj = lane >> 4, dc = lane & 15;
+    const int role = wave < HPW ? 0 : wave == HPW ? 1 : 2;
+    const float* vec = qkv + (size_t)tok * qkv_stride + (role == 0 ? (size_t)(h0 + wave) * 128 : role == 1 ? (size_t)(n_head + kvh) * 128
+                                                                                                             : (size_t)(n_head + n_kv + kvh) * 128);
+    const float* wn = role == 0 ? q_norm_w : k_norm_w;
+    const int pp = rope_row(r, mrope_sec, lane, n_ctx);
+    const float x1 = vec[lane], x2 = vec[lane + 64];
+    const float w1 = wn[lane], w2 = wn[lane + 64];
+    const float cs = rope_cos[(size_t)pp * 64 + lane], sn = rope_sin[(size_t)pp * 64 + lane];
+    const int pslot = page_at(kv, seq, lpl), ps = slot & 63;
+    __builtin_amdgcn_sched_barrier(0);
     uint4 kreg[16], vreg[16];
-    {
-        const int jbase = wave * 64;
-        if (jbase < n) {
-            const int page = kv.page_of(seq, jbase >> 6);
-            const uint16_t* Kb = kv.k + (size_t)page * kv.page_stride() + head_off;
-#pragma unroll
-            for (int d8 = 0; d8 < 16; d8++) kreg[d8] = *reinterpret_cast<const uint4*>(Kb + (d8 * 64 + lane) * 8);
-        }
-#pragma unroll
-        for (int u = 0; u < 16; u++) {
-            const int jg = 16 * u + 4 * wave + jj;
-            vreg[u] = make_uint4(0, 0, 0, 0);
-            if (jg < n && jg != slot) {
-                const int page = kv.page_of(seq, jg >> 6);
-                vreg[u] = *reinterpret_cast<const uint4*>(kv.v + (size_t)page * kv.page_stride() + head_off + (jg & 63) * 128 + dc * 8);
-            }
-        }
-    }
-    if (wave < 3) {
-        const float* vec = qkv + (size_t)tok * qkv_stride + (wave == 0 ? (size_t)h * 128 : wave == 1 ? (size_t)(n_head + kvh) * 128 : (size_t)(n_head + n_kv + kvh) * 128);
-        const float x1 = vec[lane], x2 = vec[lane + 64];
-        const int page = kv.page_of(seq, slot >> 6), ps = slot & 63;
-        if (wave < 2) {
-            const float* wn = wave == 0 ? q_norm_w : k_norm_w;
-            const float w1 = wn[lane], w2 = wn[lane + 64];
-            int32_t sec[4] = { mrope_sec[0], mrope_sec[1], mrope_sec[2], mrope_sec[3] };
-            int pp = tm.pos_of(tok, q3_mrope_stream(lane, sec));
-            if (pp < 0) pp = 0;
-            if (pp > n_ctx - 1) pp = n_ctx - 1;
-            const float cs = rope_cos[(size_t)pp * 64 + lane], sn = rope_sin[(size_t)pp * 64 + lane];
-            float p = x1 * x1;
-            p = q3_fmaf(x2, x2, p);
-            const float ss = wave_sum_bfly(p);
-            const float mean = ss / 128.0f;
-            const float scale = 1.0f / q3_sqrtf(mean + eps);
-            const float y1 = (x1 * scale) * w1, y2 = (x2 * scale) * w2;
-            float o1, o2;
-            q3_rope_pair(y1, y2, cs, sn, &o1, &o2);
-            if (wave == 0) { q_s[lane] = o1; q_s[lane + 64] = o2; }
-            else {
-                const uint16_t k1 = f2h(o1), k2 = f2h(o2);
-                kcur_s[lane] = k1; kcur_s[lane + 64] = k2;
-                if (h % grp == 0) {
-                    uint16_t* Kb = kv.k + (size_t)page * kv.page_stride() + head_off;
-                    Kb[((lane >> 3) * 64 + ps) * 8 + (lane & 7)] = k1;
-                    Kb[(((lane + 64) >> 3) * 64 + ps) * 8 + (lane & 7)] = k2;
-                }
-            }
-        } else {
-            const uint16_t v1 = f2h(x1), v2 = f2h(x2);
-            vcur_s[lane] = v1; vcur_s[lane + 64] = v2;
-            if (h % grp == 0) {
-                uint16_t* Vb = kv.v + (size_t)page * kv.page_stride() + head_off;
-                Vb[ps * 128 + lane] = v1; Vb[ps * 128 + lane + 64] = v2;
-            }
+    load_kv_chunk(kv, head_off, seq, 0, lpl, n < 256 ? n : 256, wave, lane, kreg, vreg);
+    __builtin_amdgcn_sched_barrier(0);
+    if (role < 2) {
+        float p = x1 * x1;
+        p = q3_fmaf(x2, x2, p);
+        const float ss = wave_sum_bfly(p);
+        const float mean = ss / 128.0f;
+        const float scale = 1.0f / q3_sqrtf(mean + eps);
+        const float y1 = (x1 * scale) * w1, y2 = (x2 * scale) * w2;
+        float o1, o2;
+        q3_rope_pair(y1, y2, cs, sn, &o1, &o2);
+        if (role == 0) { q_s[HPW * lane + wave] = o1; q_s[HPW * (lane + 64) + wave] = o2; }
+        else {
+            const uint16_t k1 = f2h(o1), k2 = f2h(o2);
+            kcur_s[lane] = k1; kcur_s[lane + 64] = k2;
+            if (writer) {
+                uint16_t* Kb = kv.k + (size_t)pslot * kv.page_stride() + head_off;
+                Kb[((lane >> 3) * 64 + ps) * 8 + (lane & 7)] = k1;
+                Kb[(((lane + 64) >> 3) * 64 + ps) * 8 + (lane & 7)] = k2;
+            }
+        }
+    } else if (wave == HPW + 1) {
+        const uint16_t v1 = f2h(x1), v2 = f2h(x2);
+        vcur_s[lane] = v1; vcur_s[lane + 64] = v2;
+        if (writer) {
+            uint16_t* Vb = kv.v + (size_t)pslot * kv.page_stride() + head_off;
+            Vb[ps * 128 + lane] = v1; Vb[ps * 128 + lane + 64] = v2;
         }
     }
     wg_barrier_lds();
@@ -393,89 +422,115 @@
 #pragma unroll
     for (int i = 0; i < 8; i++) O[i] = 0.0f;
     for (int c0 = 0; c0 < n; c0 += 256) {
-        const int jbase = c0 + wave * 64;
-        const int jme = jbase + lane;
-        const bool valid = jme < n;
+        const int cn = (n - c0) < 256 ? (n - c0) : 256;
         if (c0 > 0) {
-            if (jbase < n) {
-                const int page = kv.page_of(seq, jbase >> 6);
-                const uint16_t* Kb = kv.k + (size_t)page * kv.page_stride() + head_off;
-#pragma unroll
-                for (int d8 = 0; d8 < 16; d8++) kreg[d8] = *reinterpret_cast<const uint4*>(Kb + (d8 * 64 + lane) * 8);
-            }
-#pragma unroll
-            for (int u = 0; u < 16; u++) {
-                const int jg = c0 + 16 * u + 4 * wave + jj;
-                vreg[u] = make_uint4(0, 0, 0, 0);
-                if (jg < n && jg != slot) {
-                    const int page = kv.page_of(seq, jg >> 6);
-                    vreg[u] = *reinterpret_cast<const uint4*>(kv.v + (size_t)page * kv.page_stride() + head_off + (jg & 63) * 128 + dc * 8);
-                }
-            }
-        }
-        float s = -INFINITY;
-        if (jbase < n) {
-            const bool cur = (jme == slot);
-            float acc = 0.0f;
+            load_kv_chunk(kv, head_off, seq, c0 >> 6, lpl, cn, wave, lane, kreg, vreg);
+            __builtin_amdgcn_sched_barrier(0);
+        }
+        const int jme = c0 + wave * 64 + lane;
+        const bool valid = jme < n, cur = jme == slot;
+        float acc[HPW];
+#pragma unroll
+        for (int hh = 0; hh < HPW; hh++) acc[hh] = 0.0f;
+        if (HPW == 2) {
 #pragma unroll
             for (int d8 = 0; d8 < 16; d8++) {
+                const uint4 kc = *reinterpret_cast<const uint4*>(&kcur_s[8 * d8]);
+                kreg[d8].x = cur ? kc.x : kreg[d8].x; kreg[d8].y = cur ? kc.y : kreg[d8].y; kreg[d8].z = cur ? kc.z : kreg[d8].z; kreg[d8].w = cur ? kc.w : kreg[d8].w;
+            }
+            q3_f2v a = {0.0f, 0.0f};
+#pragma unroll
+            for (int d8 = 0; d8 < 16; d8++) {
+                const uint4 kk = kreg[d8];
+                const float4* q4 = reinterpret_cast<const float4*>(&q_s[16 * d8]);
+                const float4 qa = q4[0], qb = q4[1], qc = q4[2], qd = q4[3];
+                a = pk_fma(qa.x, qa.y, h2f(kk.x & 0xFFFFu), a); a = pk_fma(qa.z, qa.w, h2f(kk.x >> 16), a);
+                a = pk_fma(qb.x, qb.y, h2f(kk.y & 0xFFFFu), a); a = pk_fma(qb.z, qb.w, h2f(kk.y >> 16), a);
+                a = pk_fma(qc.x, qc.y, h2f(kk.z & 0xFFFFu), a); a = pk_fma(qc.z, qc.w, h2f(kk.z >> 16), a);
+                a = pk_fma(qd.x, qd.y, h2f(kk.w & 0xFFFFu), a); a = pk_fma(qd.z, qd.w, h2f(kk.w >> 16), a);
+            }
+            acc[0] = a.x; acc[HPW - 1] = a.y;
+        } else {
+            float a = 0.0f;
+#pragma unroll
+            for (int d8 = 0; d8 < 16; d8++) {
+                const uint4 kc = *reinterpret_cast<const uint4*>(&kcur_s[8 * d8]);
                 uint4 kk = kreg[d8];
-                if (cur) kk = *reinterpret_cast<const uint4*>(&kcur_s[8 * d8]);
+                kk.x = cur ? kc.x : kk.x; kk.y = cur ? kc.y : kk.y; kk.z = cur ? kc.z : kk.z; kk.w = cur ? kc.w : kk.w;
                 const float4 qa = *reinterpret_cast<const float4*>(&q_s[8 * d8]);
                 const float4 qb = *reinterpret_cast<const float4*>(&q_s[8 * d8 + 4]);
-                acc = q3_fmaf(qa.x, h2f(kk.x & 0xFFFFu), acc); acc = q3_fmaf(qa.y, h2f(kk.x >> 16), acc);
-                acc = q3_fmaf(qa.z, h2f(kk.y & 0xFFFFu), acc); acc = q3_fmaf(qa.w, h2f(kk.y >> 16), acc);
-                acc = q3_fmaf(qb.x, h2f(kk.z & 0xFFFFu), acc); acc = q3_fmaf(qb.y, h2f(kk.z >> 16), acc);
-                acc = q3_fmaf(qb.z, h2f(kk.w & 0xFFFFu), acc); acc = q3_fmaf(qb.w, h2f(kk.w >> 16), acc);
-            }
-            if (valid) s = acc * scale;
-        }
-        const float wm = wave_max_bfly(s);
-        if (lane == 0) wmax_s[wave] = wm;
+                a = q3_fmaf(qa.x, h2f(kk.x & 0xFFFFu), a); a = q3_fmaf(qa.y, h2f(kk.x >> 16), a);
+                a = q3_fmaf(qa.z, h2f(kk.y & 0xFFFFu), a); a = q3_fmaf(qa.w, h2f(kk.y >> 16), a);
+                a = q3_fmaf(qb.x, h2f(kk.z & 0xFFFFu), a); a = q3_fmaf(qb.y, h2f(kk.z >> 16), a);
+                a = q3_fmaf(qb.z, h2f(kk.w & 0xFFFFu), a); a = q3_fmaf(qb.w, h2f(kk.w >> 16), a);
+            }
+            acc[0] = a;
+        }
+        float s[HPW];
+#pragma unroll
+        for (int hh = 0; hh < HPW; hh++) {
+            s[hh] = valid ? acc[hh] * scale : -INFINITY;
+            const float wm = wave_max_bfly(s[hh]);
+            if (lane == 0) wmax_s[hh][wave] = wm;
+        }
         wg_barrier_lds();
-        const float mc = fmaxf(fmaxf(wmax_s[0], wmax_s[1]), fmaxf(wmax_s[2], wmax_s[3]));
-        const float p = valid ? q3_expf(s - mc) : 0.0f;
-        p_s[wave * 64 + lane] = p;
+        float mc[HPW];
+#pragma unroll
+        for (int hh = 0; hh < HPW; hh++) {
+            mc[hh] = fmaxf(fmaxf(wmax_s[hh][0], wmax_s[hh][1]), fmaxf(wmax_s[hh][2], wmax_s[hh][3]));
+            p_s[hh][wave * 64 + lane] = valid ? q3_expf(s[hh] - mc[hh]) : 0.0f;
+        }
         wg_barrier_lds();
-        float S[8];
-#pragma unroll
-        for (int i = 0; i < 8; i++) S[i] = 0.0f;
-        const int cn = (n - c0) < 256 ? (n - c0) : 256;
+        float S[HPW][8];
+#pragma unroll
+        for (int hh = 0; hh < HPW; hh++)
+#pragma unroll
+            for (int i = 0; i < 8; i++) S[hh][i] = 0.0f;
+        const uint4 vc = *reinterpret_cast<const uint4*>(&vcur_s[dc * 8]);
 #pragma unroll
         for (int u = 0; u < 16; u++) {
             if (16 * u < cn) {
                 const int jl = 16 * u + 4 * wave + jj;
                 const int jg = c0 + jl;
-                const float pj = p_s[jl];
                 uint4 vv = vreg[u];
-                if (jg == slot) vv = *reinterpret_cast<const uint4*>(&vcur_s[dc * 8]);
-                S[0] = q3_fmaf(pj, h2f(vv.x & 0xFFFFu), S[0]); S[1] = q3_fmaf(pj, h2f(vv.x >> 16), S[1]);
-                S[2] = q3_fmaf(pj, h2f(vv.y & 0xFFFFu), S[2]); S[3] = q3_fmaf(pj, h2f(vv.y >> 16), S[3]);
-                S[4] = q3_fmaf(pj, h2f(vv.z & 0xFFFFu), S[4]); S[5] = q3_fmaf(pj, h2f(vv.z >> 16), S[5]);
-                S[6] = q3_fmaf(pj, h2f(vv.w & 0xFFFFu), S[6]); S[7] = q3_fmaf(pj, h2f(vv.w >> 16), S[7]);
-            }
-        }
-#pragma unroll
-        for (int i = 0; i < 8; i++) {
-            const float a2 = S[i] + xor_lane<16>(S[i]);
-            const float T = a2 + xor_lane<32>(a2);
-            if (jj == 0) red_s[wave][dc * 8 + i] = T;
-        }
+                const bool live = jg < n, now = jg == slot;
+                vv.x = now ? vc.x : live ? vv.x : 0u; vv.y = now ? vc.y : live ? vv.y : 0u;
+                vv.z = now ? vc.z : live ? vv.z : 0u; vv.w = now ? vc.w : live ? vv.w : 0u;
+#pragma unroll
+                for (int hh = 0; hh < HPW; hh++) {
+                    const float pj = p_s[hh][jl];
+                    S[hh][0] = q3_fmaf(pj, h2f(vv.x & 0xFFFFu), S[hh][0]); S[hh][1] = q3_fmaf(pj, h2f(vv.x >> 16), S[hh][1]);
+                    S[hh][2] = q3_fmaf(pj, h2f(vv.y & 0xFFFFu), S[hh][2]); S[hh][3] = q3_fmaf(pj, h2f(vv.y >> 16), S[hh][3]);
+                    S[hh][4] = q3_fmaf(pj, h2f(vv.z & 0xFFFFu), S[hh][4]); S[hh][5] = q3_fmaf(pj, h2f(vv.z >> 16), S[hh][5]);
+                    S[hh][6] = q3_fmaf(pj, h2f(vv.w & 0xFFFFu), S[hh][6]); S[hh][7] = q3_fmaf(pj, h2f(vv.w >> 16), S[hh][7]);
+                }
+            }
+        }
+#pragma unroll
+        for (int hh = 0; hh < HPW; hh++)
+#pragma unroll
+            for (int i = 0; i < 8; i++) {
+                const float a2 = S[hh][i] + xor_lane<16>(S[hh][i]);
+                const float T = a2 + xor_lane<32>(a2);
+                if (jj == 0) red_s[hh][wave][dc * 8 + i] = T;
+            }
         wg_barrier_lds();
-        if (wave == 0) {
-            float a2 = p_s[lane];
-            a2 = a2 + p_s[lane + 64]; a2 = a2 + p_s[lane + 128]; a2 = a2 + p_s[lane + 192];
+        if (wave < HPW) {
+            const int hh = wave;
+            float a2 = p_s[hh][lane];
+            a2 = a2 + p_s[hh][lane + 64]; a2 = a2 + p_s[hh][lane + 128]; a2 = a2 + p_s[hh][lane + 192];
             const float lc = wave_sum_bfly(a2);
+            const float mch = hh == 0 ? mc[0] : mc[HPW - 1];
             float oc[8];
 #pragma unroll
-            for (int i = 0; i < 8; i++) oc[i] = (red_s[0][dc * 8 + i] + red_s[1][dc * 8 + i]) + (red_s[2][dc * 8 + i] + red_s[3][dc * 8 + i]);
+            for (int i = 0; i < 8; i++) oc[i] = (red_s[hh][0][dc * 8 + i] + red_s[hh][1][dc * 8 + i]) + (red_s[hh][2][dc * 8 + i] + red_s[hh][3][dc * 8 + i]);
             if (c0 == 0) {
-                M = mc; L = lc;
+                M = mch; L = lc;
 #pragma unroll
                 for (int i = 0; i < 8; i++) O[i] = oc[i];
             } else {
-                const float mn = fmaxf(M, mc);
-                const float ea = q3_expf(M - mn), eb = q3_expf(mc - mn);
+                const float mn = fmaxf(M, mch);
+                const float ea = q3_expf(M - mn), eb = q3_expf(mch - mn);
                 const float t2 = lc * eb;
                 L = q3_fmaf(L, ea, t2);
 #pragma unroll
@@ -485,7 +540,7 @@
         }
         wg_barrier_lds();
     }
-    if (wave == 0) {
+    if (wave < HPW) {
         float y[8];
         float amax = 0.0f;
 #pragma unroll
@@ -495,7 +550,11 @@
         const float dd = amax / 127.0f;
         const float id = (dd != 0.0f) ? (1.0f / dd) : 0.0f;
         if (jj == 0) {
-            const size_t o = ((size_t)tok * n_head + h) * 128 + dc * 8;
+            const size_t o = ((size_t)tok * n_head + h0 + wave) * 128 + dc * 8;
+            if (att) {
+                *reinterpret_cast<float4*>(att + o) = make_float4(y[0], y[1], y[2], y[3]);
+                *reinterpret_cast<float4*>(att + o + 4) = make_float4(y[4], y[5], y[6], y[7]);
+            }
             uint32_t lo = 0, hi = 0;
 #pragma unroll
             for (int i = 0; i < 4; i++) {
@@ -510,9 +569,15 @@
 void launch_attention_fused(hipStream_t st, const float* qkv, int qkv_stride, int n_head, int n_kv, const float* q_norm_w,
                             const float* k_norm_w, float eps, const float* rope_cos, const float* rope_sin, int n_ctx,
                             const int32_t* mrope_sec, const TokMeta& tm, const KvCache& kv, int layer, int8_t* aq, uint16_t* ad,
-                            int ntok) {
-    hipLaunchKernelGGL(k_attention_fused, dim3(n_head, ntok), dim3(256), 0, st, qkv, qkv_stride, n_head, n_kv, q_norm_w, k_norm_w,
-                       eps, rope_cos, rope_sin, n_ctx, mrope_sec, tm, kv, layer, aq, ad);
+                            int ntok, int hpw, float* att) {
+    if (hpw == 2) {
+        Q3_CHECK(n_head == 2 * n_kv, "k_attention_fused<2> serves exactly two q heads per kv head");
+        hipLaunchKernelGGL(k_attention_fused<2>, dim3(n_kv, ntok), dim3(256), 0, st, qkv, qkv_stride, n_head, n_kv, q_norm_w, k_norm_w,
+                           eps, rope_cos, rope_sin, n_ctx, mrope_sec, tm, kv, layer, aq, ad, att);
+    } else {
+        hipLaunchKernelGGL(k_attention_fused<1>, dim3(n_head, ntok), dim3(256), 0, st, qkv, qkv_stride, n_head, n_kv, q_norm_w, k_norm_w,
+                           eps, rope_cos, rope_sin, n_ctx, mrope_sec, tm, kv, layer, aq, ad, att);
+    }
 }
 
 template <int HPW>
@@ -532,38 +597,41 @@
     const int tok = blockIdx.y, lane = threadIdx.x;
     const float scale = 0.08838834764831845f;
     const int jj = lane >> 4, dc = lane & 15;
-    const int seq = tm.seq_of(tok), slot = tm.slot_of(tok), n = slot + 1;
+    const TokRoute r = tok_route(tm, tok);
+    const int seq = r.seq, slot = r.slot, n = slot + 1;
     const size_t head_off = (size_t)layer * kv.layer_stride() + (size_t)kvh * 8192;
-    const int page = kv.page_of(seq, 0);
+    const int page = page_at(kv, seq, 0);
+    const int pp = rope_row(r, mrope_sec, lane, n_ctx);
+    const float* tv = qkv + (size_t)tok * qkv_stride;
+    float xr[HPW + 2][2];
+#pragma unroll
+    for (int which = 0; which < HPW + 2; which++) {
+        const float* vec = tv + (which < HPW ? (size_t)(h0 + which) * 128 : which == HPW ? (size_t)(n_head + kvh) * 128
+                                                                                         : (size_t)(n_head + n_kv + kvh) * 128);
+        xr[which][0] = vec[lane]; xr[which][1] = vec[lane + 64];
+    }
+    const float qw1 = q_norm_w[lane], qw2 = q_norm_w[lane + 64], kw1 = k_norm_w[lane], kw2 = k_norm_w[lane + 64];
+    const float cs = rope_cos[(size_t)pp * 64 + lane], sn = rope_sin[(size_t)pp * 64 + lane];
+    __builtin_amdgcn_sched_barrier(0);
     const uint16_t* Kb = kv.k + (size_t)page * kv.page_stride() + head_off;
     const uint16_t* Vb = kv.v + (size_t)page * kv.page_stride() + head_off;
     uint4 kreg[16], vreg[4][4];
 #pragma unroll
-    for (int d8 = 0; d8 < 16; d8++) kreg[d8] = (lane < slot) ? *reinterpret_cast<const uint4*>(Kb + (d8 * 64 + lane) * 8) : make_uint4(0, 0, 0, 0);
+    for (int d8 = 0; d8 < 16; d8++) kreg[d8] = *reinterpret_cast<const uint4*>(Kb + (d8 * 64 + lane) * 8);
 #pragma unroll
     for (int ww = 0; ww < 4; ww++)
 #pragma unroll
-        for (int u = 0; u < 4; u++) {
-            const int jl = 16 * u + 4 * ww + jj;
-            vreg[ww][u] = (jl < slot) ? *reinterpret_cast<const uint4*>(Vb + jl * 128 + dc * 8) : make_uint4(0, 0, 0, 0);
-        }
-    int32_t sec[4] = { mrope_sec[0], mrope_sec[1], mrope_sec[2], mrope_sec[3] };
-    int pp = tm.pos_of(tok, q3_mrope_stream(lane, sec));
-    if (pp < 0) pp = 0;
-    if (pp > n_ctx - 1) pp = n_ctx - 1;
-    const float cs = rope_cos[(size_t)pp * 64 + lane], sn = rope_sin[(size_t)pp * 64 + lane];
-    const float* tv = qkv + (size_t)tok * qkv_stride;
+        for (int u = 0; u < 4; u++) vreg[ww][u] = *reinterpret_cast<const uint4*>(Vb + (16 * u + 4 * ww + jj) * 128 + dc * 8);
+    __builtin_amdgcn_sched_barrier(0);
 #pragma unroll
     for (int which = 0; which < HPW + 1; which++) {
-        const float* vec = tv + (which < HPW ? (size_t)(h0 + which) * 128 : (size_t)(n_head + kvh) * 128);
-        const float* wn = which < HPW ? q_norm_w : k_norm_w;
-        const float x1 = vec[lane], x2 = vec[lane + 64];
+        const float x1 = xr[which][0], x2 = xr[which][1];
         float p = x1 * x1;
         p = q3_fmaf(x2, x2, p);
         const float ss = wave_sum_bfly(p);
         const float mean = ss / 128.0f;
         const float sc2 = 1.0f / q3_sqrtf(mean + eps);
-        const float y1 = (x1 * sc2) * wn[lane], y2 = (x2 * sc2) * wn[lane + 64];
+        const float y1 = (x1 * sc2) * (which < HPW ? qw1 : kw1), y2 = (x2 * sc2) * (which < HPW ? qw2 : kw2);
         float o1, o2;
         q3_rope_pair(y1, y2, cs, sn, &o1, &o2);
         if (which < HPW) { q_s[which][lane] = o1; q_s[which][lane + 64] = o2; }
@@ -578,8 +646,7 @@
         }
     }
     {
-        const float* vec = tv + (size_t)(n_head + n_kv + kvh) * 128;
-        const uint16_t v1 = f2h(vec[lane]), v2 = f2h(vec[lane + 64]);
+        const uint16_t v1 = f2h(xr[HPW + 1][0]), v2 = f2h(xr[HPW + 1][1]);
         vcur_s[lane] = v1; vcur_s[lane + 64] = v2;
         if (writer) {
             uint16_t* Vw = kv.v + (size_t)page * kv.page_stride() + head_off;
@@ -594,8 +661,9 @@
     for (int hh = 0; hh < HPW; hh++) a[hh] = 0.0f;
 #pragma unroll
     for (int d8 = 0; d8 < 16; d8++) {
+        const uint4 kc = *reinterpret_cast<const uint4*>(&kcur_s[8 * d8]);
         uint4 kk = kreg[d8];
-        if (cur) kk = *reinterpret_cast<const uint4*>(&kcur_s[8 * d8]);
+        kk.x = cur ? kc.x : kk.x; kk.y = cur ? kc.y : kk.y; kk.z = cur ? kc.z : kk.z; kk.w = cur ? kc.w : kk.w;
         const float kf[8] = { h2f(kk.x & 0xFFFFu), h2f(kk.x >> 16), h2f(kk.y & 0xFFFFu), h2f(kk.y >> 16),
                               h2f(kk.z & 0xFFFFu), h2f(kk.z >> 16), h2f(kk.w & 0xFFFFu), h2f(kk.w >> 16) };
 #pragma unroll
@@ -616,6 +684,7 @@
     wg_barrier_lds();
     Q3_STAMP(3);
     const int dq = n_head * 128;
+    const uint4 vc = *reinterpret_cast<const uint4*>(&vcur_s[dc * 8]);
 #pragma unroll
     for (int hh = 0; hh < HPW; hh++) {
         float s01[8], s23[8], y[8];
@@ -630,7 +699,9 @@
                     const int jl = 16 * u + 4 * ww + jj;
                     const float pj = p_s[hh][jl];
                     uint4 vv = vreg[ww][u];
-                    if (jl == slot) vv = *reinterpret_cast<const uint4*>(&vcur_s[dc * 8]);
+                    const bool live = jl < slot, now = jl == slot;
+                    vv.x = now ? vc.x : live ? vv.x : 0u; vv.y = now ? vc.y : live ? vv.y : 0u;
+                    vv.z = now ? vc.z : live ? vv.z : 0u; vv.w = now ? vc.w : live ? vv.w : 0u;
                     S[0] = q3_fmaf(pj, h2f(vv.x & 0xFFFFu), S[0]); S[1] = q3_fmaf(pj, h2f(vv.x >> 16), S[1]);
                     S[2] = q3_fmaf(pj, h2f(vv.y & 0xFFFFu), S[2]); S[3] = q3_fmaf(pj, h2f(vv.y >> 16), S[3]);
                     S[4] = q3_fmaf(pj, h2f(vv.z & 0xFFFFu), S[4]); S[5] = q3_fmaf(pj, h2f(vv.z >> 16), S[5]);
@@ -675,9 +746,11 @@
 }
 void launch_attention_short(hipStream_t st, const float* qkv, int qkv_stride, int n_head, int n_kv, const float* q_norm_w,
                             const float* k_norm_w, float eps, const float* rope_cos, const float* rope_sin, int n_ctx,
-                            const int32_t* mrope_sec, const TokMeta& tm, const KvCache& kv, int layer, int8_t* aq, uint16_t* ad, int ntok, float* att) {
+                            const int32_t* mrope_sec, const TokMeta& tm, const KvCache& kv, int layer, int8_t* aq, uint16_t* ad, int ntok, float* att,
+                            int hpw) {
     static const int hpw1_max = [] { const char* e = std::getenv("Q3_SHORT_ATTN_HPW1_MAX"); return e ? atoi(e) : 128; }();
-    if (ntok <= hpw1_max)
+    if (hpw == 0) hpw = ntok <= hpw1_max ? 1 : 2;
+    if (hpw == 1)
         hipLaunchKernelGGL(k_attention_short<1>, dim3(n_head, ntok), dim3(64), 0, st, qkv, qkv_stride, n_head, n_kv, q_norm_w, k_norm_w, eps, rope_cos,
                            rope_sin, n_ctx, mrope_sec, tm, kv, layer, aq, ad, att);
     else
diff --git a/qwen3-tts-rust_amd/csrc/transformer.cpp b/qwen3-tts-rust_amd/csrc/transformer.cpp
--- a/qwen3-tts-rust_amd/csrc/transformer.cpp
+++ b/qwen3-tts-rust_amd/csrc/transformer.cpp
@@ -271,7 +271,7 @@
 
 Transformer::Transformer(const std::string& path, int n_ctx, int max_tok) : n_ctx_(n_ctx), max_tok_(max_tok) {
     init_kernel_attributes();
-    if (const char* e = std::getenv("Q3_UNFUSED")) fused = !(e[0] == '1');
+    if (const char* e = std::getenv("Q3_UNFUSED")) fused = fused_attn = !(e[0] == '1');
     Gguf g(path);
     hp_.arch = g.kv_str("general.architecture", "qwen3");
     auto K = [&](const char* s) { return hp_.arch + "." + s; };
@@ -356,7 +356,7 @@
 }
 
 Transformer::Transformer(const Transformer& o, int max_tok)
-    : fused(o.fused), float_mode_(o.float_mode_), foutput_(o.foutput_), hp_(o.hp_), n_ctx_(o.n_ctx_), max_tok_(max_tok), layers_(o.layers_), output_(o.output_),
+    : fused(o.fused), fused_attn(o.fused_attn), float_mode_(o.float_mode_), foutput_(o.foutput_), hp_(o.hp_), n_ctx_(o.n_ctx_), max_tok_(max_tok), layers_(o.layers_), output_(o.output_),
       output_norm_(o.output_norm_), ws_(o.ws_), weight_bytes_(o.weight_bytes_), layer_weight_bytes_(o.layer_weight_bytes_), all_q8_(o.all_q8_),
       ggml_mode_(o.ggml_mode_), gg_layers_(o.gg_layers_), gg_output_(o.gg_output_) {
     alloc_workspace();
@@ -494,6 +494,9 @@
         if (short_attn_min_ > 0 && ntok >= short_attn_min_ && !same_seq_ && hp_.n_head == 2 * hp_.n_kv)
             launch_attention_short(st, qkv_.p, dq + 2 * dkv, hp_.n_head, hp_.n_kv, L.q_norm, L.k_norm, hp_.eps, rope_cos_.p, rope_sin_.p,
                                    n_ctx_, d_mrope_.p, tm, kv, l, aq_.p, ad_.p, ntok);
+        else if (fused_attn && !same_seq_)
+            launch_attention_fused(st, qkv_.p, dq + 2 * dkv, hp_.n_head, hp_.n_kv, L.q_norm, L.k_norm, hp_.eps, rope_cos_.p, rope_sin_.p,
+                                   n_ctx_, d_mrope_.p, tm, kv, l, aq_.p, ad_.p, ntok, hp_.n_head == 2 * hp_.n_kv ? 2 : 1);
         else {
             launch_qk_rope_append(st, qkv_.p, dq + 2 * dkv, nullptr, hp_.n_head, hp_.n_kv, L.q_norm, L.k_norm, hp_.eps, rope_cos_.p,
                                   rope_sin_.p, n_ctx_, d_mrope_.p, tm, kv, l, qrot_.p, ntok);
@@ -553,6 +556,9 @@
         if (short_attn_min_ > 0 && ntok >= short_attn_min_ && !same_seq_ && hp_.n_head == 2 * hp_.n_kv)
             launch_attention_short(st, qkv_.p, dq + 2 * dkv, hp_.n_head, hp_.n_kv, L.q_norm, L.k_norm, hp_.eps, rope_cos_.p, rope_sin_.p,
                                    n_ctx_, d_mrope_.p, tm, kv, l, aq_.p, ad_.p, ntok, attf_.p);
+        else if (fused_attn && !same_seq_)
+            launch_attention_fused(st, qkv_.p, dq + 2 * dkv, hp_.n_head, hp_.n_kv, L.q_norm, L.k_norm, hp_.eps, rope_cos_.p, rope_sin_.p,
+                                   n_ctx_, d_mrope_.p, tm, kv, l, aq_.p, ad_.p, ntok, hp_.n_head == 2 * hp_.n_kv ? 2 : 1, attf_.p);
         else {
             launch_qk_rope_append(st, qkv_.p, dq + 2 * dkv, nullptr, hp_.n_head, hp_.n_kv, L.q_norm, L.k_norm, hp_.eps, rope_cos_.p, rope_sin_.p,
                                   n_ctx_, d_mrope_.p, tm, kv, l, qrot_.p, ntok);
diff --git a/qwen3-tts-rust_amd/csrc/transformer.h b/qwen3-tts-rust_amd/csrc/transformer.h
--- a/qwen3-tts-rust_amd/csrc/transformer.h
+++ b/qwen3-tts-rust_amd/csrc/transformer.h
@@ -32,6 +32,7 @@
         const q3_u64* idx_keys = nullptr;
     };
     bool fused = true;
+    bool fused_attn = true;
     void forward(hipStream_t st, const Input& in, int ntok, const TokMeta& tm, const KvCache& kv, float* hidden_out);
     void head(hipStream_t st, int tok0, int tok_count, int row0, int nrows, float* logits, int logits_stride,
               const ArgmaxEpi* am = nullptr, int nrows_valid = -1, float* hidden_out = nullptr);
diff --git a/qwen3-tts-rust_amd/python/q3tts/__init__.py b/qwen3-tts-rust_amd/python/q3tts/__init__.py
--- a/qwen3-tts-rust_amd/python/q3tts/__init__.py
+++ b/qwen3-tts-rust_amd/python/q3tts/__init__.py
@@ -80,7 +80,7 @@
     "q3tts_gen_options_default", "q3tts_submit_ex", "q3tts_submit_text_ex", "q3tts_generate_batch_ex", "q3tts_group_submit_ex",
     "q3tts_group_submit_text_ex", "q3tts_op_sample_rows",
     "q3tts_prompt_build_streaming", "q3tts_submit_trailing", "q3tts_submit_text_streaming", "q3tts_generate_batch_trailing",
-    "q3tts_group_submit_text_streaming", "q3tts_op_codec_gemm", "q3tts_codec_gemm_plan",
+    "q3tts_group_submit_text_streaming", "q3tts_op_codec_gemm", "q3tts_codec_gemm_plan", "q3tts_op_decode_attention",
 ]
 
 
@@ -714,6 +714,49 @@
     return out, (GEMM_FORM_NAMES[d.form_ran], d.ksplit_ran, d.reducer_ran)
 
 
+ATTN_KERNELS = {"pair": 0, "fused1": 1, "fused2": 2, "short1": 3, "short2": 4}
+
+
+class DecodeAttnDesc(C.Structure):
+    _fields_ = [("kernel", C.c_int32), ("n_head", C.c_int32), ("n_kv", C.c_int32), ("ntok", C.c_int32), ("n_ctx", C.c_int32),
+                ("n_layer", C.c_int32), ("layer", C.c_int32), ("n_pages", C.c_int32),
+                ("qkv", C.c_void_p), ("q_norm", C.c_void_p), ("k_norm", C.c_void_p), ("eps", C.c_float),
+                ("rope_cos", C.c_void_p), ("rope_sin", C.c_void_p), ("mrope_sec", C.c_void_p),
+                ("seq", C.c_void_p), ("slot", C.c_void_p), ("pos", C.c_void_p), ("uniform_pos", C.c_int32),
+                ("page_table", C.c_void_p), ("max_pages", C.c_int32),
+                ("k_cache", C.c_void_p), ("v_cache", C.c_void_p), ("aq", C.c_void_p), ("ad", C.c_void_p), ("att", C.c_void_p)]
+
+
+def op_decode_attention(kernel, qkv, n_head, n_kv, q_norm, k_norm, eps, rope_cos, rope_sin, mrope_sec, k_cache, v_cache, n_layer, layer,
+                        seq=None, slot=None, pos=None, uniform_pos=-1, page_table=None, want_att=False):
+    qkv = np.ascontiguousarray(qkv, np.float32)
+    ntok = qkv.shape[0]
+    assert qkv.shape[1] == (n_head + 2 * n_kv) * 128
+    kc = np.array(k_cache, np.uint16, copy=True, order="C")
+    vc = np.array(v_cache, np.uint16, copy=True, order="C")
+    assert kc.shape == vc.shape and kc.shape[1:] == (n_layer, n_kv, 8192)
+    qn, kn = np.ascontiguousarray(q_norm, np.float32), np.ascontiguousarray(k_norm, np.float32)
+    cs, sn = np.ascontiguousarray(rope_cos, np.float32), np.ascontiguousarray(rope_sin, np.float32)
+    assert qn.size == 128 and kn.size == 128 and cs.shape == sn.shape and cs.shape[1] == 64
+    sec = np.ascontiguousarray(mrope_sec, np.int32)
+    assert sec.size == 4
+    arrs = [None if a is None else np.ascontiguousarray(a, np.int32) for a in (seq, slot, pos, page_table)]
+    aq = np.zeros((ntok, n_head * 128), np.int8)
+    ad = np.zeros((ntok, n_head * 4), np.uint16)
+    att = np.zeros((ntok, n_head * 128), np.float32) if want_att else None
+    d = DecodeAttnDesc()
+    d.kernel = ATTN_KERNELS[kernel] if isinstance(kernel, str) else kernel
+    d.n_head, d.n_kv, d.ntok, d.n_ctx, d.n_layer, d.layer, d.n_pages = n_head, n_kv, ntok, cs.shape[0], n_layer, layer, kc.shape[0]
+    d.qkv, d.q_norm, d.k_norm, d.eps, d.rope_cos, d.rope_sin, d.mrope_sec = _p(qkv), _p(qn), _p(kn), eps, _p(cs), _p(sn), _p(sec)
+    d.seq, d.slot, d.pos = (_p(a) for a in arrs[:3])
+    d.uniform_pos = uniform_pos
+    d.page_table, d.max_pages = _p(arrs[3]), 0 if arrs[3] is None else arrs[3].shape[1]
+    d.k_cache, d.v_cache, d.aq, d.ad, d.att = _p(kc), _p(vc), _p(aq), _p(ad), _p(att)
+    lib().q3tts_op_decode_attention.argtypes = [C.POINTER(DecodeAttnDesc)]
+    _chk(lib().q3tts_op_decode_attention(C.byref(d)))
+    return aq, ad, kc, vc, att
+
+
 def codec_gemm_plan(M, N, cin, taps=1, dil=1, lda=None, ldo=None, out_off=0, o_segT=0, o_skip=0, a_segT=0, a_skip=0, epi=EPI_NONE, ldr=0,
                     r_segT=0, r_skip=0, a_split=False, o_split=False, ws_floats=1 << 22):
     d = _codec_gemm_desc(M, N, cin, taps, dil, cin if lda is None else lda, 0, a_segT, a_skip, epi, ldr, 0, r_segT, r_skip,
```

Result: faster. 713.5, median of 6 (+1.8%).
